# jstrom2002/ImageCodecs

Hardware: AMD Instinct MI355X
Metric: megapixels/s JPEG decode, 4096x4096 RGB batch (higher is better)
Workload: dtype u8

## Files before the change

imagecodecs_amd/__init__.py:

```python
from __future__ import annotations

import ctypes as C
import os
import subprocess

import numpy as np

__all__ = ["ICXError", "Context", "Batch", "HdrBatch", "Image", "lib", "build", "LIB_PATH",
           "OK", "NO_JPEG", "UNSUPPORTED", "OUT_OF_MEM", "INTERNAL_ERR", "SYNTAX_ERROR",
           "HDR_OK", "HDR_NOT_RADIANCE", "HDR_BAD_HEADER", "HDR_MALFORMED", "HDR_TRUNCATED",
           "HDR_TOO_LARGE", "HDR_INTERNAL_ERR", "hdr_probe", "exr_probe", "EXR_SUCCESS", "EXR_INVALID_DATA", "Multi", "RECORD_DTYPE", "records_device",
           "checksum64", "multi_shard"]

OK, NO_JPEG, UNSUPPORTED, OUT_OF_MEM, INTERNAL_ERR, SYNTAX_ERROR = range(6)
RESULT_NAMES = ["NJ_OK", "NJ_NO_JPEG", "NJ_UNSUPPORTED", "NJ_OUT_OF_MEM", "NJ_INTERNAL_ERR", "NJ_SYNTAX_ERROR"]

_HERE = os.path.dirname(os.path.abspath(__file__))
_DEFAULT_LIB = os.path.join(_HERE, "lib", "libicx.so")
LIB_PATH = os.environ.get("ICX_LIB") or _DEFAULT_LIB
_LIB = None


class ICXError(RuntimeError):
    pass


def build() -> str:
    subprocess.run(["make", "-s", "-C", _HERE], check=True)
    return LIB_PATH


_vp, _i32, _i64, _u64, _sz = C.c_void_p, C.c_int, C.c_int64, C.c_uint64, C.c_size_t
_SIGS = {
    "icx_version": (C.c_char_p, []),
    "icx_last_error": (C.c_char_p, [_vp]),
    "icx_create": (_vp, [_i32]),
    "icx_destroy": (None, [_vp]),
    "icx_free": (None, [_vp]),
    "icx_jpeg_probe": (_i32, [_vp, _sz, C.POINTER(_i32), C.POINTER(_i32), C.POINTER(_i32)]),
    "icx_nj_init": (None, [_vp]),
    "icx_nj_done": (None, [_vp]),
    "icx_nj_decode": (_i32, [_vp, _vp, _i32]),
    "icx_nj_get_width": (_i32, [_vp]),
    "icx_nj_get_height": (_i32, [_vp]),
    "icx_nj_is_color": (_i32, [_vp]),
    "icx_nj_get_image": (_vp, [_vp]),
    "icx_nj_get_image_size": (_i32, [_vp]),
    "icx_jpeg_decode": (_i32, [_vp, _vp, _sz, C.POINTER(_vp), C.POINTER(_i32), C.POINTER(_i32), C.POINTER(_i32)]),
    "icx_batch_create": (_vp, [_vp, _i32, _i32, _i32, _i32]),
    "icx_batch_destroy": (None, [_vp]),
    "icx_jpeg_batch_decode": (_i32, [_vp, _i32, _vp, _vp, _vp, _vp, _u64, _vp, _vp, _vp]),
    "icx_jpeg_batch_decode_host": (_i32, [_vp, _i32, _vp, _vp, _vp, _u64, _vp, _vp]),
    "icx_batch_stage_times": (_i32, [_vp, _vp, _vp, _i32]),
    "icx_batch_group": (_i32, [_vp]),
    "icx_batch_groups": (_i32, [_vp, _i32]),
    "icx_batch_path_stats": (_i32, [_vp, C.POINTER(_i32), C.POINTER(_i32), C.POINTER(_i32)]),
    "icx_tje_encode_with_func": (_i32, [_vp, _vp, _vp, _i32, _i32, _i32, _i32, _vp]),
    "icx_tje_encode_to_file_at_quality": (_i32, [_vp, C.c_char_p, _i32, _i32, _i32, _i32, _vp]),
    "icx_tje_encode_to_file": (_i32, [_vp, C.c_char_p, _i32, _i32, _i32, _vp]),
    "icx_jpeg_encode_with_func": (_i32, [_vp, _vp, _vp, _i32, _i32, _i32, _i32, _i32, _vp]),
    "icx_encoder_create": (_vp, [_vp]),
    "icx_encoder_destroy": (None, [_vp]),
    "icx_encoder_stage_times": (_i32, [_vp, _vp, _vp, _i32]),
    "icx_png_encode_with_func": (_i32, [_vp, _vp, _vp, _vp, _i32, _i32, _i32]),
    "icx_png_save_to_file": (_i32, [_vp, C.c_char_p, _vp, _i32, _i32, _i32]),
    "icx_png_encoder_create": (_vp, [_vp]),
    "icx_png_encoder_destroy": (None, [_vp]),
    "icx_png_encode_device": (_i32, [_vp, _i32, _i32, _i32, _vp, _vp, _u64, C.POINTER(_u64), _vp]),
    "icx_png_encode_device_batch": (_i32, [_vp, _i32, _i32, _i32, _i32, _vp, _vp, _u64, _vp, _vp, _vp]),
    "icx_png_encoder_stage_times": (_i32, [_vp, C.POINTER(C.c_char_p), C.POINTER(C.c_float), _i32]),
    "icx_jpeg_encode_device": (_i32, [_vp, _i32, _i32, _i32, _i32, _i32, _vp, _vp, _u64, C.POINTER(_u64), _vp]),
    "icx_jpeg_encode_device_batch": (_i32, [_vp, _i32, _i32, _i32, _i32, _i32, _i32, _vp, _vp, _u64, _vp, _vp, _vp]),
    "icx_hdr_probe": (_i32, [_vp, _sz, C.POINTER(_i32), C.POINTER(_i32)]),
    "icx_hdr_decode": (_i32, [_vp, _vp, _sz, C.POINTER(_vp), C.POINTER(_i32), C.POINTER(_i32), C.POINTER(_i32)]),
    "icx_hdr_batch_create": (_vp, [_vp, _i32, _i32, _i32]),
    "icx_hdr_batch_destroy": (None, [_vp]),
    "icx_hdr_batch_decode": (_i32, [_vp, _i32, _vp, _vp, _vp, _vp, _u64, _vp, _vp, _vp]),
    "icx_hdr_batch_stage_times": (_i32, [_vp, _vp, _vp, _i32]),
    "icx_jpeg_records": (_i32, [_vp, _i32, _vp, _u64, _vp, _vp, _i32, _i32, _vp, _vp]),
    "icx_checksum64": (_u64, [_vp, _sz]),
    "icx_ctx_device": (_i32, [_vp]),
    "icx_ctx_stream": (_vp, [_vp]),
    "icx_multi_create": (_vp, [_vp, _i32, _i32, _i32]),
    "icx_multi_destroy": (None, [_vp]),
    "icx_multi_decode_host": (_i32, [_vp, _i32, _vp, _vp, _vp, _u64, _vp, _vp]),
    "icx_multi_last_error": (C.c_char_p, [_vp]),
    "icx_multi_gather": (C.c_char_p, [_vp]),
    "icx_multi_shard": (_i32, [_vp, _i32, _i32, _vp]),
    "icx_exr_probe": (_i32, [_vp, _sz, C.POINTER(_i32), C.POINTER(_i32)]),
    "icx_exr_decode": (_i32, [_vp, _vp, _sz, C.POINTER(_vp), C.POINTER(_i32), C.POINTER(_i32)]),
    "icx_exr_decode_device": (_i32, [_vp, _vp, _vp, _sz, _vp, _sz, C.POINTER(_i32), C.POINTER(_i32)]),
    "icx_exr_decode_device_batch": (_i32, [_vp, _i32, _vp, _vp, _vp, _vp, _vp, _vp, _vp, _vp]),
}

RECORD_DTYPE = np.dtype([("status", "<i4"), ("width", "<i4"), ("height", "<i4"), ("ncomp", "<i4"),
                         ("checksum", "<u8")])

HDR_OK, HDR_NOT_RADIANCE, HDR_BAD_HEADER, HDR_MALFORMED, HDR_TRUNCATED, HDR_TOO_LARGE = range(6)
HDR_INTERNAL_ERR = -1

EXR_SUCCESS, EXR_INVALID_MAGIC_NUMBER, EXR_INVALID_EXR_VERSION, EXR_INVALID_ARGUMENT, EXR_INVALID_DATA = 0, -1, -2, -3, -4
EXR_UNSUPPORTED_FORMAT, EXR_INVALID_HEADER, EXR_UNSUPPORTED_FEATURE, EXR_INTERNAL_ERR = -8, -9, -10, -100

WRITE_FUNC = C.CFUNCTYPE(None, C.c_void_p, C.c_void_p, C.c_int)


def _share_hip_runtime_with_torch() -> None:
    import importlib.util
    spec = importlib.util.find_spec("torch")
    if spec is None or not spec.submodule_search_locations:
        return
    tlib = os.path.join(list(spec.submodule_search_locations)[0], "lib")
    for name in ("libhsa-runtime64.so", "libamdhip64.so"):
        path = os.path.join(tlib, name)
        if os.path.exists(path):
            C.CDLL(path, mode=C.RTLD_GLOBAL)


def lib():
    global _LIB
    if _LIB is None:
        if not os.path.exists(LIB_PATH):
            raise ICXError(f"{LIB_PATH} not built: run `make -C imagecodecs_amd` (hipcc, gfx950)")
        _share_hip_runtime_with_torch()
        L = C.CDLL(LIB_PATH)
        for name, (res, args) in _SIGS.items():
            try:
                fn = getattr(L, name)
            except AttributeError:
                if LIB_PATH != _DEFAULT_LIB:
                    continue
                raise
            fn.restype = res
            fn.argtypes = args
        _LIB = L
    return _LIB


def _err(ctx_ptr) -> str:
    msg = lib().icx_last_error(ctx_ptr)
    return msg.decode() if msg else ""


class Context:

    def __init__(self, device: int = 0):
        self._p = lib().icx_create(device)
        if not self._p:
            raise ICXError("icx_create failed: " + _err(None))
        self.device = device

    def close(self):
        if getattr(self, "_p", None):
            lib().icx_destroy(self._p)
            self._p = None

    def __del__(self):
        self.close()

    def __enter__(self):
        return self

    def __exit__(self, *a):
        self.close()

    @property
    def ptr(self):
        return self._p

    def nj_init(self):
        lib().icx_nj_init(self._p)

    def nj_done(self):
        lib().icx_nj_done(self._p)

    def nj_decode(self, jpeg: bytes) -> int:
        buf = C.create_string_buffer(bytes(jpeg), max(1, len(jpeg)))
        return lib().icx_nj_decode(self._p, buf, len(jpeg))

    def nj_get_width(self) -> int:
        return lib().icx_nj_get_width(self._p)

    def nj_get_height(self) -> int:
        return lib().icx_nj_get_height(self._p)

    def nj_is_color(self) -> int:
        return lib().icx_nj_is_color(self._p)

    def nj_get_image_size(self) -> int:
        return lib().icx_nj_get_image_size(self._p)

    def nj_get_image(self) -> bytes:
        p = lib().icx_nj_get_image(self._p)
        return C.string_at(p, self.nj_get_image_size()) if p else b""

    def decode(self, jpeg: bytes):
        buf = C.create_string_buffer(bytes(jpeg), max(1, len(jpeg)))
        out = C.c_void_p()
        w, h, n = C.c_int(), C.c_int(), C.c_int()
        code = lib().icx_jpeg_decode(self._p, buf, len(jpeg), C.byref(out), C.byref(w), C.byref(h), C.byref(n))
        pix = b""
        if out.value:
            pix = C.string_at(out.value, w.value * h.value * n.value)
            lib().icx_free(out)
        if code == INTERNAL_ERR and _err(self._p):
            raise ICXError(_err(self._p))
        return code, w.value, h.value, n.value, pix

    def tje_encode(self, quality: int, width: int, height: int, comps: int, src: bytes):
        chunks = []

        @WRITE_FUNC
        def sink(_ctx, data, size):
            chunks.append(C.string_at(data, size))

        buf = C.create_string_buffer(bytes(src), max(1, len(src)))
        ok = lib().icx_tje_encode_with_func(self._p, sink, None, quality, width, height, comps, buf)
        return b"".join(chunks) if ok == 1 else None

    def hdr_decode(self, data: bytes):
        buf = C.create_string_buffer(bytes(data), max(1, len(data)))
        out = C.c_void_p()
        w, h, rows = C.c_int(), C.c_int(), C.c_int()
        code = lib().icx_hdr_decode(self._p, buf, len(data), C.byref(out), C.byref(w), C.byref(h), C.byref(rows))
        if code == HDR_INTERNAL_ERR:
            raise ICXError("icx_hdr_decode: " + _err(self._p))
        arr = None
        if out.value:
            n = w.value * h.value * 4
            arr = np.frombuffer(C.string_at(out.value, n * 4), np.float32).reshape(h.value, w.value, 4).copy()
            lib().icx_free(out)
        return code, w.value, h.value, rows.value, arr

    def exr_decode(self, data: bytes):
        buf = C.create_string_buffer(bytes(data), max(1, len(data)))
        out = C.c_void_p()
        w, h = C.c_int(), C.c_int()
        code = lib().icx_exr_decode(self._p, buf, len(data), C.byref(out), C.byref(w), C.byref(h))
        if code == EXR_INTERNAL_ERR:
            raise ICXError("icx_exr_decode: " + _err(self._p))
        arr = None
        if out.value:
            n = w.value * h.value * 4
            arr = np.frombuffer(C.string_at(out.value, n * 4), np.float32).reshape(h.value, w.value, 4).copy()
            lib().icx_free(out)
        return code, w.value, h.value, arr

    def exr_decode_device(self, data: bytes, d_data: int, d_out: int, out_floats: int):
        buf = C.create_string_buffer(bytes(data), max(1, len(data)))
        w, h = C.c_int(), C.c_int()
        code = lib().icx_exr_decode_device(self._p, buf, C.c_void_p(d_data), len(data), C.c_void_p(d_out), out_floats,
                                           C.byref(w), C.byref(h))
        if code == EXR_INTERNAL_ERR:
            raise ICXError("icx_exr_decode_device: " + _err(self._p))
        return code, w.value, h.value

    def exr_decode_device_batch(self, datas, d_ptrs, d_outs, out_floats):
        n = len(datas)
        bufs = [C.create_string_buffer(bytes(d), max(1, len(d))) for d in datas]
        hp = (C.c_void_p * n)(*[C.cast(b, C.c_void_p) for b in bufs])
        dp = (C.c_void_p * n)(*d_ptrs)
        sz = (C.c_size_t * n)(*[len(d) for d in datas])
        op = (C.c_void_p * n)(*d_outs)
        of = (C.c_size_t * n)(*out_floats)
        codes = np.zeros(n, np.int32)
        ws = np.zeros(n, np.int32)
        hs = np.zeros(n, np.int32)
        rc = lib().icx_exr_decode_device_batch(self._p, n, hp, dp, sz, op, of, codes.ctypes.data, ws.ctypes.data,
                                               hs.ctypes.data)
        if rc == EXR_INTERNAL_ERR:
            raise ICXError("icx_exr_decode_device_batch: " + _err(self._p))
        if rc != 0:
            raise ICXError(f"icx_exr_decode_device_batch: code {rc}")
        return codes, ws, hs

    def png_encode(self, width: int, height: int, d: int, src: bytes):
        chunks = []

        @WRITE_FUNC
        def sink(_ctx, data, size):
            chunks.append(C.string_at(data, size))

        buf = C.create_string_buffer(bytes(src), max(1, len(src)))
        ok = lib().icx_png_encode_with_func(self._p, sink, None, buf, width, height, d)
        return b"".join(chunks) if ok == 1 else None

    def jpeg_encode(self, quality: int, subsampling: int, width: int, height: int, comps: int, src: bytes):
        chunks = []

        @WRITE_FUNC
        def sink(_ctx, data, size):
            chunks.append(C.string_at(data, size))

        buf = C.create_string_buffer(bytes(src), max(1, len(src)))
        ok = lib().icx_jpeg_encode_with_func(self._p, sink, None, quality, subsampling, width, height, comps, buf)
        return b"".join(chunks) if ok == 1 else None


class PngEncoder:

    def __init__(self, ctx: Context):
        self.ctx = ctx
        self._p = lib().icx_png_encoder_create(ctx.ptr)
        if not self._p:
            raise ICXError("icx_png_encoder_create failed: " + _err(ctx.ptr))

    def close(self):
        if getattr(self, "_p", None):
            lib().icx_png_encoder_destroy(self._p)
            self._p = None

    def __del__(self):
        self.close()

    def encode_device(self, width, height, d, d_src, d_out, out_cap, stream=0):
        n = C.c_uint64()
        rc = lib().icx_png_encode_device(self._p, width, height, d, d_src, d_out, out_cap, C.byref(n), stream or None)
        if rc not in (OK, OUT_OF_MEM):
            raise ICXError(f"icx_png_encode_device -> {rc}: {_err(self.ctx.ptr)}")
        return rc, int(n.value)

    def encode_device_batch(self, width, height, d, d_srcs, d_out, out_stride, stream=0):
        n = len(d_srcs)
        srcs = (C.c_void_p * max(1, n))(*d_srcs)
        sizes = np.zeros(max(1, n), np.uint64)
        status = np.zeros(max(1, n), np.int32)
        rc = lib().icx_png_encode_device_batch(self._p, n, width, height, d, srcs, d_out, out_stride,
                                               sizes.ctypes.data, status.ctypes.data, stream or None)
        if rc != OK:
            raise ICXError(f"icx_png_encode_device_batch -> {rc}: {_err(self.ctx.ptr)}")
        return status[:n], sizes[:n].astype(np.int64)

    def stage_times(self) -> dict:
        names = (C.c_char_p * 8)()
        ms = (C.c_float * 8)()
        k = lib().icx_png_encoder_stage_times(self._p, names, ms, 8)
        return {names[i].decode(): float(ms[i]) for i in range(k)}


class Encoder:

    def __init__(self, ctx: Context):
        self.ctx = ctx
        self._p = lib().icx_encoder_create(ctx.ptr)
        if not self._p:
            raise ICXError("icx_encoder_create failed: " + _err(ctx.ptr))

    def close(self):
        if getattr(self, "_p", None):
            lib().icx_encoder_destroy(self._p)
            self._p = None

    def __del__(self):
        self.close()

    def encode_device(self, quality, subsampling, width, height, comps, d_src, d_out, out_cap, stream=0):
        n = C.c_uint64()
        rc = lib().icx_jpeg_encode_device(self._p, quality, subsampling, width, height, comps, d_src, d_out,
                                          out_cap, C.byref(n), stream or None)
        if rc not in (OK, OUT_OF_MEM):
            raise ICXError(f"icx_jpeg_encode_device -> {rc}: {_err(self.ctx.ptr)}")
        return rc, int(n.value)

    def encode_device_batch(self, quality, subsampling, width, height, comps, d_srcs, d_out, out_stride, stream=0):
        n = len(d_srcs)
        srcs = (C.c_void_p * max(1, n))(*d_srcs)
        sizes = np.zeros(max(1, n), np.uint64)
        status = np.zeros(max(1, n), np.int32)
        rc = lib().icx_jpeg_encode_device_batch(self._p, n, quality, subsampling, width, height, comps, srcs, d_out,
                                                out_stride, sizes.ctypes.data, status.ctypes.data, stream or None)
        if rc != OK:
            raise ICXError(f"icx_jpeg_encode_device_batch -> {rc}: {_err(self.ctx.ptr)}")
        return status[:n], sizes[:n].astype(np.int64)

    def stage_times(self) -> dict:
        names = (C.c_char_p * 8)()
        ms = (C.c_float * 8)()
        k = lib().icx_encoder_stage_times(self._p, names, ms, 8)
        return {names[i].decode(): float(ms[i]) for i in range(k)}


def probe(jpeg: bytes):
    w, h, n = C.c_int(), C.c_int(), C.c_int()
    buf = C.create_string_buffer(bytes(jpeg), max(1, len(jpeg)))
    code = lib().icx_jpeg_probe(buf, len(jpeg), C.byref(w), C.byref(h), C.byref(n))
    return code, w.value, h.value, n.value


def records_device(ctx: "Context", n, d_out, out_stride, d_status, d_dims, max_width, max_height, d_records,
                   stream=0):
    rc = lib().icx_jpeg_records(ctx.ptr, n, d_out, out_stride, d_status, d_dims, max_width, max_height, d_records,
                                stream or None)
    if rc != OK:
        raise ICXError(f"icx_jpeg_records -> {rc}: {_err(ctx.ptr)}")


def checksum64(data: bytes) -> int:
    buf = C.create_string_buffer(bytes(data), max(1, len(data)))
    return int(lib().icx_checksum64(buf, len(data)))


def multi_shard(sizes, ndev: int) -> np.ndarray:
    n = len(sizes)
    sz = (C.c_size_t * max(1, n))(*[int(x) for x in sizes])
    out = np.zeros(max(1, n), np.int32)
    if lib().icx_multi_shard(sz, n, ndev, out.ctypes.data) != OK:
        raise ICXError("icx_multi_shard failed")
    return out[:n]


class Multi:

    def __init__(self, devices, max_width: int, max_height: int):
        devs = (C.c_int * len(devices))(*devices)
        self._p = lib().icx_multi_create(devs, len(devices), max_width, max_height)
        if not self._p:
            raise ICXError("icx_multi_create failed: " + _err(None))
        self.devices = list(devices)
        self.max_width, self.max_height = max_width, max_height

    @property
    def gather(self) -> str:
        return lib().icx_multi_gather(self._p).decode()

    def close(self):
        if getattr(self, "_p", None):
            lib().icx_multi_destroy(self._p)
            self._p = None

    def __del__(self):
        self.close()

    def decode_host(self, jpegs, want_pixels: bool = True):
        n = len(jpegs)
        stride = self.max_width * self.max_height * 3
        bufs = [C.create_string_buffer(bytes(j), max(1, len(j))) for j in jpegs]
        ptrs = (C.c_void_p * max(1, n))(*[C.cast(b, C.c_void_p) for b in bufs])
        sizes = (C.c_size_t * max(1, n))(*[len(j) for j in jpegs])
        outs_np = [np.empty(stride, np.uint8) for _ in range(n)] if want_pixels else None
        outs = (C.c_void_p * max(1, n))(*[o.ctypes.data for o in outs_np]) if want_pixels else None
        rec = np.zeros(max(1, n), RECORD_DTYPE)
        shard_of = np.zeros(max(1, n), np.int32)
        rc = lib().icx_multi_decode_host(self._p, n, ptrs, sizes, outs, stride, rec.ctypes.data, shard_of.ctypes.data)
        if rc != OK:
            msg = lib().icx_multi_last_error(self._p)
            raise ICXError(f"icx_multi_decode_host -> {rc}: {msg.decode() if msg else ''}")
        pix = None
        if want_pixels:
            pix = []
            for i in range(n):
                r = rec[i]
                nb = int(r["width"]) * int(r["height"]) * int(r["ncomp"])
                pix.append(outs_np[i][:nb] if r["status"] == OK else None)
        return rec[:n], shard_of[:n], pix


class Batch:

    def __init__(self, ctx: Context, max_images: int, max_width: int, max_height: int, group: int = 0):
        self.ctx = ctx
        self._p = lib().icx_batch_create(ctx.ptr, max_images, max_width, max_height, group)
        if not self._p:
            raise ICXError("icx_batch_create failed: " + _err(ctx.ptr))
        self.max_images, self.max_width, self.max_height = max_images, max_width, max_height

    def close(self):
        if getattr(self, "_p", None):
            lib().icx_batch_destroy(self._p)
            self._p = None

    def __del__(self):
        self.close()

    def decode_device(self, n, d_data, d_offsets, d_sizes, d_out, out_stride, d_status, d_dims, stream=0):
        rc = lib().icx_jpeg_batch_decode(self._p, n, d_data, d_offsets, d_sizes, d_out, out_stride,
                                         d_status, d_dims, stream or None)
        if rc != OK:
            raise ICXError(f"icx_jpeg_batch_decode -> {rc}: {_err(self.ctx.ptr)}")

    def decode_host(self, jpegs, out_stride=None):
        n = len(jpegs)
        out_stride = out_stride or self.max_width * self.max_height * 3
        bufs = [C.create_string_buffer(bytes(j), max(1, len(j))) for j in jpegs]
        ptrs = (C.c_void_p * n)(*[C.cast(b, C.c_void_p) for b in bufs])
        sizes = (C.c_size_t * n)(*[len(j) for j in jpegs])
        outs_np = [np.empty(out_stride, np.uint8) for _ in range(n)]
        outs = (C.c_void_p * n)(*[o.ctypes.data for o in outs_np])
        status = np.zeros(n, np.int32)
        dims = np.zeros((n, 3), np.int32)
        rc = lib().icx_jpeg_batch_decode_host(self._p, n, ptrs, sizes, outs, out_stride,
                                              status.ctypes.data, dims.ctypes.data)
        if rc != OK:
            raise ICXError(f"icx_jpeg_batch_decode_host -> {rc}: {_err(self.ctx.ptr)}")
        res = []
        for i in range(n):
            w, h, c = (int(x) for x in dims[i])
            pix = outs_np[i][: w * h * c].reshape(h, w, c) if status[i] == OK else None
            res.append((int(status[i]), w, h, c, pix))
        return res

    def path_stats(self) -> dict:
        a, b, c = C.c_int(), C.c_int(), C.c_int()
        lib().icx_batch_path_stats(self._p, C.byref(a), C.byref(b), C.byref(c))
        return {"parallel": a.value, "fallback": b.value, "sequential": c.value}

    @property
    def group(self) -> int:
        return int(lib().icx_batch_group(self._p))

    def groups_per_call(self, n: int) -> int:
        return int(lib().icx_batch_groups(self._p, n))

    def stage_times(self) -> dict:
        names = (C.c_char_p * 16)()
        ms = (C.c_float * 16)()
        k = lib().icx_batch_stage_times(self._p, names, ms, 16)
        return {names[i].decode(): float(ms[i]) for i in range(k)}


def hdr_probe(data: bytes):
    w, h = C.c_int(), C.c_int()
    buf = C.create_string_buffer(bytes(data), max(1, len(data)))
    code = lib().icx_hdr_probe(buf, len(data), C.byref(w), C.byref(h))
    return code, w.value, h.value


def exr_probe(data: bytes):
    w, h = C.c_int(), C.c_int()
    buf = C.create_string_buffer(bytes(data), max(1, len(data)))
    code = lib().icx_exr_probe(buf, len(data), C.byref(w), C.byref(h))
    return code, w.value, h.value


class HdrBatch:

    def __init__(self, ctx: Context, max_images: int, max_width: int, max_height: int):
        self.ctx = ctx
        self._p = lib().icx_hdr_batch_create(ctx.ptr, max_images, max_width, max_height)
        if not self._p:
            raise ICXError("icx_hdr_batch_create failed: " + _err(ctx.ptr))
        self.max_images, self.max_width, self.max_height = max_images, max_width, max_height

    def close(self):
        if getattr(self, "_p", None):
            lib().icx_hdr_batch_destroy(self._p)
            self._p = None

    def __del__(self):
        self.close()

    def decode_device(self, n, d_data, d_offsets, d_sizes, d_out, out_stride, d_status, d_dims, stream=0):
        rc = lib().icx_hdr_batch_decode(self._p, n, d_data, d_offsets, d_sizes, d_out, out_stride,
                                        d_status, d_dims, stream or None)
        if rc != HDR_OK:
            raise ICXError(f"icx_hdr_batch_decode -> {rc}: {_err(self.ctx.ptr)}")

    def stage_times(self) -> dict:
        names = (C.c_char_p * 8)()
        ms = (C.c_float * 8)()
        k = lib().icx_hdr_batch_stage_times(self._p, names, ms, 8)
        return {names[i].decode(): float(ms[i]) for i in range(k)}


class Image:

    UBYTE, USHORT, FLOAT = range(3)
    _ctx = None

    def __init__(self):
        self.h_ = self.w_ = self.d_ = 0
        self.pixels_ = None
        self.type_ = Image.UBYTE

    @classmethod
    def context(cls):
        if cls._ctx is None:
            cls._ctx = Context(0)
        return cls._ctx

    def read(self, filepath: str):
        ext = os.path.splitext(filepath)[1].lower()
        if ext == ".hdr":
            self._read_hdr(filepath)
            return
        if ext == ".exr":
            self._read_exr(filepath)
            return
        if ext not in (".jpg", ".jpeg"):
            raise ValueError("Cannot parse filetype")
        data = open(filepath, "rb").read()
        code, w, h, n, pix = self.context().decode(data)
        if code != OK:
            raise RuntimeError("Error decoding the input file.\n")
        self.w_, self.h_, self.d_ = w, h, n
        self.pixels_ = np.frombuffer(pix, np.uint8).copy()
        self.type_ = Image.UBYTE

    def _read_hdr(self, filepath: str):
        data = open(filepath, "rb").read()
        code, w, h, rows, px = self.context().hdr_decode(data)
        if code not in (HDR_OK, HDR_TRUNCATED):
            raise RuntimeError("Invalid file format")
        self.w_, self.h_, self.d_ = w, h, 4
        self.pixels_ = px.reshape(-1).view(np.uint8).copy()
        self.type_ = Image.FLOAT

    def _read_exr(self, filepath: str):
        data = open(filepath, "rb").read()
        code, w, h, px = self.context().exr_decode(data + b"\xff")
        if code != EXR_SUCCESS:
            raise RuntimeError("Could not load .exr")
        self.w_, self.h_, self.d_ = w, h, 4
        self.pixels_ = px.reshape(-1).view(np.uint8).copy()
        self.type_ = Image.FLOAT

    def write(self, filepath: str):
        ext = os.path.splitext(filepath)[1].lower()
        if ext == ".png":
            out = self.context().png_encode(self.w_, self.h_, self.d_, self.pixels_.tobytes())
        elif ext in (".jpg", ".jpeg"):
            out = self.context().tje_encode(3, self.w_, self.h_, self.d_, self.pixels_.tobytes())
        else:
            raise ValueError("Cannot parse filetype")
        with open(filepath, "wb") as f:
            if out is not None:
                f.write(out)

    def load(self, pixels, w: int, h: int, channels: int):
        self.pixels_ = np.ascontiguousarray(pixels, np.uint8).reshape(-1)
        self.w_, self.h_, self.d_ = w, h, channels
        self.type_ = Image.UBYTE

    def rows(self):
        return self.h_

    def cols(self):
        return self.w_

    def channels(self):
        return self.d_

    def empty(self):
        return self.h_ == 0 or self.w_ == 0 or self.d_ == 0 or self.pixels_ is None

    def byteSize(self):
        return 4 if self.type_ == Image.FLOAT else 2 if self.type_ == Image.USHORT else 1

    def type(self):
        return self.type_

    def totalBytes(self):
        return self.w_ * self.h_ * self.d_ * self.byteSize()

    def data(self):
        return self.pixels_
```

imagecodecs_amd/csrc/icx_api.cpp:

```cpp
#include <hip/hip_runtime.h>
#include <rocprofiler-sdk-roctx/roctx.h>

#include <algorithm>
#include <cstdio>
#include <cstdlib>
#include <cstring>
#include <exception>
#include <memory>
#include <string>
#include <vector>

#include "../../include/icx.h"
#include "icx_internal.h"
#include "icx_step.h"

using namespace icx;

struct icx_ctx {
    int device = 0;
    hipStream_t stream = nullptr;
    std::string err;
    std::vector<uint8_t> nj_image;
    int nj_w = 0, nj_h = 0, nj_color = 0, nj_size = 0;
    icx_batch* single = nullptr;
    uint8_t* d_in = nullptr;
    size_t d_in_cap = 0;
    ExrWs* exr = nullptr;
};

struct EventHook;

#ifndef ICX_MAX_PIPES
#define ICX_MAX_PIPES 2
#endif
constexpr int kMaxPipes = ICX_MAX_PIPES;
struct icx_batch {
    icx_ctx* ctx = nullptr;
    int max_images = 0;
    int pipes = 1;
    GroupWs ws[kMaxPipes];
    hipStream_t pst[kMaxPipes] = {};
    hipEvent_t fork = nullptr, join[kMaxPipes] = {};
    std::vector<hipEvent_t> front_done;
    int min_groups = 1;
    bool stagger = false;
    uint8_t* d_hin = nullptr;
    size_t d_hin_cap = 0;
    hipEvent_t done = nullptr;
    bool decoded = false;
    std::unique_ptr<EventHook> hook;
};

static std::string g_create_err;

static thread_local char g_msg[512];

#define ICX_HIP(ctx, call, ret)                                                             \
    do {                                                                                    \
        hipError_t e_ = (call);                                                             \
        if (e_ != hipSuccess) {                                                             \
            (void)hipGetLastError();  \
            std::snprintf(g_msg, sizeof g_msg, "%s failed: %s", #call, hipGetErrorString(e_)); \
            if (ctx) (ctx)->err = g_msg;                                                    \
            return ret;                                                                     \
        }                                                                                   \
    } while (0)

struct RoctxRange {
    explicit RoctxRange(const char* m) { (void)roctxRangePushA(m); }
    ~RoctxRange() { (void)roctxRangePop(); }
};
static const char* const kRangeNames[kStCount] = {"icx:parse", "icx:unstuff", "icx:entropy", "icx:write",
                                                  "icx:idct", "icx:upsample", "icx:convert"};
struct EventHook : StageHook {
    struct Rec { Stage s; hipEvent_t a, b; };
    std::vector<Rec> recs;
    std::vector<hipEvent_t> pool;
    size_t used = 0;
    hipEvent_t get() {
        if (used == pool.size()) {
            hipEvent_t e;
            if (hipEventCreate(&e) != hipSuccess) return nullptr;
            pool.push_back(e);
        }
        return pool[used++];
    }
    void reset() { recs.clear(); used = 0; }
    void begin(Stage s, hipStream_t st) override {
        (void)roctxRangePushA(kRangeNames[s]);
        hipEvent_t a = get(), b = get();
        if (!a || !b) return;
        (void)hipEventRecord(a, st);
        recs.push_back({s, a, b});
    }
    void end(Stage s, hipStream_t st) override {
        (void)roctxRangePop();
        for (auto it = recs.rbegin(); it != recs.rend(); ++it)
            if (it->s == s) { (void)hipEventRecord(it->b, st); return; }
    }
    ~EventHook() override {
        for (auto e : pool) (void)hipEventDestroy(e);
    }
};

extern "C" {

const char* icx_version(void) { return "icx 0.1.0 gfx950"; }

const char* icx_last_error(const icx_ctx* ctx) { return ctx ? ctx->err.c_str() : g_create_err.c_str(); }

icx_ctx* icx_create(int device) {
    int n = 0;
    if (hipGetDeviceCount(&n) != hipSuccess || n <= 0) {
        g_create_err = "no HIP device available (libicx has no CPU decode path)";
        return nullptr;
    }
    if (device < 0 || device >= n) {
        g_create_err = "device ordinal out of range";
        return nullptr;
    }
    if (hipSetDevice(device) != hipSuccess) {
        g_create_err = "hipSetDevice failed";
        return nullptr;
    }
    auto* c = new icx_ctx();
    c->device = device;
    if (hipStreamCreateWithFlags(&c->stream, hipStreamNonBlocking) != hipSuccess) {
        g_create_err = "hipStreamCreate failed";
        delete c;
        return nullptr;
    }
    return c;
}

void icx_batch_destroy(icx_batch* b);

void icx_destroy(icx_ctx* c) {
    if (!c) return;
    (void)hipSetDevice(c->device);
    if (c->single) icx_batch_destroy(c->single);
    if (c->d_in) (void)hipFree(c->d_in);
    if (c->exr) exr_ws_destroy(c->exr);
    if (c->stream) (void)hipStreamDestroy(c->stream);
    delete c;
}

void icx_free(void* p) { std::free(p); }
int icx_ctx_device(const icx_ctx* c) { return c ? c->device : -1; }
void* icx_ctx_stream(const icx_ctx* c) { return c ? (void*)c->stream : nullptr; }

int icx_jpeg_probe(const uint8_t* jpeg, size_t size, int* w, int* h, int* ncomp) {
    if (w) *w = 0;
    if (h) *h = 0;
    if (ncomp) *ncomp = 0;
    if (!jpeg) return ICX_NO_JPEG;
    auto d = std::make_unique<Desc>();
    int st = parse_headers(jpeg, (int64_t)std::min<size_t>(size, 0x7FFFFFFF), *d);
    if (st != kPending) return st;
    if (w) *w = d->W;
    if (h) *h = d->H;
    if (ncomp) *ncomp = d->nc == 1 ? 1 : 3;
    return ICX_OK;
}

static int64_t ws_per_slot(GroupWs& ws, int max_w, int max_h) {
    ws.max_w = max_w;
    ws.max_h = max_h;
    ws.coef_cap = ws_coef_cap(max_w, max_h);
    ws.plane_cap = ws_plane_cap(max_w, max_h);
    ws.tmp_cap = ws_tmp_cap(max_w, max_h);
    const int bpp = std::getenv("ICX_UPOOL_BPP") ? std::max(1, std::min(16, std::atoi(std::getenv("ICX_UPOOL_BPP")))) : 2;
    ws.ucap = ((int64_t)max_w * max_h * bpp + 4095) / 4096 * 4096;
    ws.rst_cap = ((int64_t)max_w / 8 + 1) * ((int64_t)max_h / 8 + 1);
    const int64_t tiles_per_slot = ws.ucap / kTileBytes + 2;
    const int64_t lanes_per_slot = ((ws.ucap + kSubBytesSmall - 1) / kSubBytesSmall + kLanes - 1) / kLanes * kLanes + kLanes;
    return ws.coef_cap * kPoolPerSlotX4 / 4 * (64 * 2 + 4 + 8) + ws.plane_cap + (int64_t)sizeof(Desc) + ws.ucap +
           (int64_t)sizeof(StepSet) +
           tiles_per_slot * 28 + ws.rst_cap * 8 +
           lanes_per_slot * (8 + 8 + 20 + 24 + 4 + 16 + (int64_t)sizeof(RecState) * kRec + (int64_t)sizeof(GwOut) +
                             (int64_t)sizeof(GcRec) + 8) + kMaxRepair * 4;
}

static void ws_free(GroupWs& ws) {
    if (ws.tmp_own && ws.tmp) (void)hipFree(ws.tmp);
    for (void* p : {(void*)ws.desc, (void*)ws.ac, (void*)ws.dc, (void*)ws.planes, (void*)ws.spec,
                    (void*)ws.tilepre, (void*)ws.wgpre, (void*)ws.wg2pre, (void*)ws.totals, (void*)ws.tiles,
                    (void*)ws.tile_obase, (void*)ws.U, (void*)ws.X, (void*)ws.sub, (void*)ws.rst, (void*)ws.tile_rbase,
                    (void*)ws.ent, (void*)ws.stats, (void*)ws.Y, (void*)ws.rec, (void*)ws.nrec, (void*)ws.guess_cnt,
                    (void*)ws.repair, (void*)ws.steps, (void*)ws.map, (void*)ws.chunk_next, (void*)ws.pool_next,
                    (void*)ws.gw, (void*)ws.crec, (void*)ws.clist})
        if (p) (void)hipFree(p);
    if (ws.h_defer) (void)hipHostFree(ws.h_defer);
    if (ws.h_layout) (void)hipHostFree(ws.h_layout);
    if (ws.ev_defer) (void)hipEventDestroy(ws.ev_defer);
    ws = GroupWs{};
}

static bool ws_alloc_all(icx_ctx* ctx, GroupWs& ws, int group, int max_w, int max_h);
static bool ws_alloc(icx_ctx* ctx, GroupWs& ws, int group, int max_w, int max_h) {
    if (ws_alloc_all(ctx, ws, group, max_w, max_h)) return true;
    ws_free(ws);
    return false;
}

static bool ws_alloc_all(icx_ctx* ctx, GroupWs& ws, int group, int max_w, int max_h) {
    (void)ws_per_slot(ws, max_w, max_h);
    const int64_t tiles_per_slot = ws.ucap / kTileBytes + 2;
    const int64_t lanes_per_slot = ((ws.ucap + kSubBytesSmall - 1) / kSubBytesSmall + kLanes - 1) / kLanes * kLanes + kLanes;
    ws.slots = group;
    ws.upool = (int64_t)(group + 2) * ws.ucap;
    ICX_HIP(ctx, hipMalloc(&ws.desc, sizeof(Desc) * group), false);
    ws.pool_cap = (int64_t)(group + 2) * ws.coef_cap * kPoolPerSlotX4 / 4;
    ICX_HIP(ctx, hipMalloc(&ws.ac, (size_t)(ws.pool_cap + kGwChunk) * 64 * 2), false);
    ICX_HIP(ctx, hipMalloc(&ws.dc, (size_t)(ws.pool_cap + kGwChunk) * 4), false);
    ICX_HIP(ctx, hipMalloc(&ws.map, (size_t)ws.pool_cap * sizeof(uint2)), false);
    ICX_HIP(ctx, hipMalloc(&ws.chunk_next, (size_t)(ws.pool_cap / kGwChunk + 2) * 4), false);
    ICX_HIP(ctx, hipMalloc(&ws.pool_next, sizeof(unsigned long long)), false);
    ICX_HIP(ctx, hipMalloc(&ws.planes, (size_t)ws.plane_cap * group), false);
    if ((int64_t)(ws.pool_cap + kGwChunk) * 64 * 2 >= ws.tmp_cap * 6 * group) {
        ws.tmp = reinterpret_cast<uint8_t*>(ws.ac);
    } else {
        ICX_HIP(ctx, hipMalloc(&ws.tmp, (size_t)ws.tmp_cap * 6 * group), false);
        ws.tmp_own = true;
    }
    ws.tiles_cap = tiles_per_slot * (group + 2);
    ws.lanes_cap = lanes_per_slot * (group + 2);
    ICX_HIP(ctx, hipMalloc(&ws.spec, sizeof(SpecImg) * group), false);
    ICX_HIP(ctx, hipMalloc(&ws.tilepre, sizeof(int32_t) * (group + 1)), false);
    ICX_HIP(ctx, hipMalloc(&ws.wgpre, sizeof(int32_t) * (group + 1)), false);
    ICX_HIP(ctx, hipMalloc(&ws.wg2pre, sizeof(int32_t) * (group + 1)), false);
    ICX_HIP(ctx, hipMalloc(&ws.totals, sizeof(int32_t) * 4), false);
    ICX_HIP(ctx, hipMalloc(&ws.tiles, sizeof(TileRec) * ws.tiles_cap), false);
    ICX_HIP(ctx, hipMalloc(&ws.tile_obase, sizeof(int32_t) * ws.tiles_cap), false);
    ICX_HIP(ctx, hipMalloc(&ws.U, (size_t)ws.upool + 256), false);
    ICX_HIP(ctx, hipMalloc(&ws.X, sizeof(uint64_t) * ws.lanes_cap), false);
    ICX_HIP(ctx, hipMalloc(&ws.sub, sizeof(SubRec) * ws.lanes_cap), false);
    ICX_HIP(ctx, hipMalloc(&ws.rst, sizeof(int64_t) * ws.rst_cap * group), false);
    ICX_HIP(ctx, hipMalloc(&ws.tile_rbase, sizeof(int32_t) * ws.tiles_cap), false);
    ICX_HIP(ctx, hipMalloc(&ws.ent, sizeof(LaneEntry) * ws.lanes_cap), false);
    ICX_HIP(ctx, hipMalloc(&ws.stats, sizeof(int32_t) * 4), false);
    ICX_HIP(ctx, hipMalloc(&ws.Y, sizeof(uint64_t) * ws.lanes_cap), false);
    ICX_HIP(ctx, hipMalloc(&ws.rec, sizeof(RecState) * kRec * ws.lanes_cap), false);
    ICX_HIP(ctx, hipMalloc(&ws.nrec, sizeof(int32_t) * ws.lanes_cap), false);
    ICX_HIP(ctx, hipMalloc(&ws.guess_cnt, sizeof(int32_t) * 4 * ws.lanes_cap), false);
    ICX_HIP(ctx, hipMalloc(&ws.repair, sizeof(int32_t) * kMaxRepair * group), false);
    ICX_HIP(ctx, hipMalloc(&ws.steps, sizeof(StepSet) * group), false);
    ICX_HIP(ctx, hipMalloc(&ws.gw, sizeof(GwOut) * ws.lanes_cap), false);
    ICX_HIP(ctx, hipMalloc(&ws.crec, sizeof(GcRec) * ws.lanes_cap), false);
    ICX_HIP(ctx, hipMalloc(&ws.clist, sizeof(int2) * ws.lanes_cap), false);
    ICX_HIP(ctx, hipHostMalloc(&ws.h_defer, 3 * sizeof(int32_t), hipHostMallocDefault), false);
    ws.h_defer[0] = ws.h_defer[1] = ws.h_defer[2] = 0;
    ICX_HIP(ctx, hipHostMalloc(&ws.h_layout, sizeof(int32_t), hipHostMallocDefault), false);
    *ws.h_layout = 1;
    ICX_HIP(ctx, hipEventCreateWithFlags(&ws.ev_defer, hipEventDisableTiming), false);
    return true;
}

icx_batch* icx_batch_create(icx_ctx* ctx, int max_images, int max_w, int max_h, int group) {
    if (!ctx || max_images <= 0 || max_w <= 0 || max_h <= 0 || max_w > 65535 || max_h > 65535) {
        if (ctx) ctx->err = "icx_batch_create: bad arguments";
        return nullptr;
    }
    ICX_HIP(ctx, hipSetDevice(ctx->device), nullptr);
    std::unique_ptr<icx_batch, void (*)(icx_batch*)> b(new icx_batch(), icx_batch_destroy);
    b->ctx = ctx;
    b->max_images = max_images;
    int pipes = kMaxPipes;
    if (const char* e = std::getenv("ICX_PIPES")) pipes = std::max(1, std::min(kMaxPipes, std::atoi(e)));
    if (max_images < 2) pipes = 1;
    GroupWs probe;
    const int64_t per_slot = ws_per_slot(probe, max_w, max_h);
    if (group <= 0) {
        size_t free_b = 0, total_b = 0;
        ICX_HIP(ctx, hipMemGetInfo(&free_b, &total_b), nullptr);
        const int64_t budget = (int64_t)(0.8 * (double)free_b);
        group = (int)std::max<int64_t>(1, std::min<int64_t>(max_images, budget / per_slot));
    }
    group = std::min(group, max_images);
    if (group < 2) pipes = 1;
    b->pipes = pipes;
    if (const char* e = std::getenv("ICX_GROUPS")) b->min_groups = std::max(1, std::atoi(e));
    if (const char* e = std::getenv("ICX_STAGGER")) b->stagger = std::atoi(e) != 0;
    for (int p = 0; p < pipes; ++p) {
        const int slots = (group + pipes - 1) / pipes;
        if (!ws_alloc(ctx, b->ws[p], slots, max_w, max_h)) return nullptr;
        if (p > 0) ICX_HIP(ctx, hipStreamCreateWithFlags(&b->pst[p], hipStreamNonBlocking), nullptr);
        ICX_HIP(ctx, hipEventCreateWithFlags(&b->join[p], hipEventDisableTiming), nullptr);
    }
    ICX_HIP(ctx, hipEventCreateWithFlags(&b->fork, hipEventDisableTiming), nullptr);
    ICX_HIP(ctx, hipEventCreateWithFlags(&b->done, hipEventDisableTiming), nullptr);
    b->hook = std::make_unique<EventHook>();
    return b.release();
}

void icx_batch_destroy(icx_batch* b) {
    if (!b) return;
    (void)hipSetDevice(b->ctx->device);
    for (int p = 0; p < kMaxPipes; ++p) {
        ws_free(b->ws[p]);
        if (b->pst[p]) (void)hipStreamDestroy(b->pst[p]);
        if (b->join[p]) (void)hipEventDestroy(b->join[p]);
    }
    if (b->fork) (void)hipEventDestroy(b->fork);
    if (b->done) (void)hipEventDestroy(b->done);
    for (auto e : b->front_done) (void)hipEventDestroy(e);
    if (b->d_hin) (void)hipFree(b->d_hin);
    delete b;
}

static int batch_split(const icx_batch* b, int n, int* per_out) {
    const int slots = b->ws[0].slots;
    const int want = std::min(n, std::max((n + slots - 1) / slots, b->min_groups));
    int per = (n + want - 1) / want;
    int ng = (n + per - 1) / per;
    if (b->pipes > 1 && ng > 1 && ng % b->pipes) {
        const int up = (ng + b->pipes - 1) / b->pipes * b->pipes;
        if (up <= n) {
            const int per2 = (n + up - 1) / up;
            const int ng2 = (n + per2 - 1) / per2;
            if (ng2 % b->pipes == 0) {
                per = per2;
                ng = ng2;
            }
        }
    }
    *per_out = per;
    return ng;
}

int icx_batch_groups(const icx_batch* b, int n) {
    int per = 0;
    return b && n > 0 ? batch_split(b, n, &per) : 0;
}

int icx_jpeg_batch_decode(icx_batch* b, int n, const uint8_t* d_data, const uint64_t* d_off, const uint64_t* d_size,
                          uint8_t* d_out, uint64_t out_stride, int32_t* d_status, int32_t* d_dims, void* stream) {
    if (!b) return ICX_INTERNAL_ERR;
    icx_ctx* ctx = b->ctx;
    if (n < 0 || n > b->max_images) { ctx->err = "icx_jpeg_batch_decode: n exceeds batch capacity"; return ICX_INTERNAL_ERR; }
    if (n == 0) return ICX_OK;
    if (!d_data || !d_off || !d_size || !d_out || !d_status || !d_dims) { ctx->err = "null pointer"; return ICX_INTERNAL_ERR; }
    ICX_HIP(ctx, hipSetDevice(ctx->device), ICX_INTERNAL_ERR);
    hipStream_t st = stream ? (hipStream_t)stream : ctx->stream;
    const RoctxRange range("icx_jpeg_batch_decode");
    b->hook->reset();
    for (int p = 0; p < b->pipes; ++p)
        ICX_HIP(ctx, hipMemsetAsync(b->ws[p].stats, 0, sizeof(int32_t) * 4, st), ICX_INTERNAL_ERR);
    int per = 0;
    const int ng = batch_split(b, n, &per);
    const int used = std::min(b->pipes, ng);
    if (used > 1) {
        ICX_HIP(ctx, hipEventRecord(b->fork, st), ICX_INTERNAL_ERR);
        for (int p = 1; p < used; ++p) ICX_HIP(ctx, hipStreamWaitEvent(b->pst[p], b->fork, 0), ICX_INTERNAL_ERR);
    }
    const bool stagger = b->stagger && used > 1;
    hipStreamCaptureStatus cap = hipStreamCaptureStatusNone;
    ICX_HIP(ctx, hipStreamIsCapturing(st, &cap), ICX_INTERNAL_ERR);
    const char* hw = std::getenv("ICX_HOST_WAIT");
    const bool no_wait_env = hw && std::atoi(hw) == 0;
    const bool host_wait = !stagger && cap == hipStreamCaptureStatusNone && !no_wait_env;
    while (stagger && (int)b->front_done.size() < ng) {
        hipEvent_t e;
        ICX_HIP(ctx, hipEventCreateWithFlags(&e, hipEventDisableTiming), ICX_INTERNAL_ERR);
        b->front_done.push_back(e);
    }
    auto front0 = [&](int g) {
        const int g0 = g * per, p = g % used;
        launch_decode_front(b->ws[p], std::min(per, n - g0), d_data, d_off + g0, d_size + g0, out_stride,
                            p == 0 ? st : b->pst[p], b->hook.get(), host_wait ? kFrontFirst : kFrontAll);
    };
    for (int g = 0; g < std::min(used, ng); ++g) {
        if (stagger && g > 0) ICX_HIP(ctx, hipStreamWaitEvent(b->pst[g % used], b->front_done[g - 1], 0), ICX_INTERNAL_ERR);
        front0(g);
        if (stagger) ICX_HIP(ctx, hipEventRecord(b->front_done[g], g % used == 0 ? st : b->pst[g % used]), ICX_INTERNAL_ERR);
    }
    for (int g = 0; g < ng; ++g) {
        const int g0 = g * per, gn = std::min(per, n - g0), p = g % used;
        hipStream_t ps = p == 0 ? st : b->pst[p];
        if (host_wait) launch_decode_front(b->ws[p], gn, d_data, d_off + g0, d_size + g0, out_stride, ps, b->hook.get(),
                                           kFrontRest);
        launch_decode_back(b->ws[p], gn, d_out + (uint64_t)g0 * out_stride, out_stride, d_status + g0, d_dims + 3 * g0,
                           ps, b->hook.get(), host_wait);
        const int gnext = g + used;
        if (gnext < ng) {
            hipStream_t pn = gnext % used == 0 ? st : b->pst[gnext % used];
            if (stagger) ICX_HIP(ctx, hipStreamWaitEvent(pn, b->front_done[gnext - 1], 0), ICX_INTERNAL_ERR);
            front0(gnext);
            if (stagger) ICX_HIP(ctx, hipEventRecord(b->front_done[gnext], pn), ICX_INTERNAL_ERR);
        }
    }
    for (int p = 1; p < used; ++p) {
        ICX_HIP(ctx, hipEventRecord(b->join[p], b->pst[p]), ICX_INTERNAL_ERR);
        ICX_HIP(ctx, hipStreamWaitEvent(st, b->join[p], 0), ICX_INTERNAL_ERR);
    }
    ICX_HIP(ctx, hipEventRecord(b->done, st), ICX_INTERNAL_ERR);
    b->decoded = true;
    ICX_HIP(ctx, hipGetLastError(), ICX_INTERNAL_ERR);
    return ICX_OK;
}

int icx_batch_path_stats(const icx_batch* b, int32_t* parallel, int32_t* fallback, int32_t* sequential) {
    if (!b) return ICX_INTERNAL_ERR;
    int32_t h[4] = {0, 0, 0, 0};
    ICX_HIP(b->ctx, hipSetDevice(b->ctx->device), ICX_INTERNAL_ERR);
    if (b->decoded) ICX_HIP(b->ctx, hipEventSynchronize(b->done), ICX_INTERNAL_ERR);
    for (int p = 0; p < b->pipes; ++p) {
        int32_t q[4];
        ICX_HIP(b->ctx, hipMemcpy(q, b->ws[p].stats, sizeof q, hipMemcpyDeviceToHost), ICX_INTERNAL_ERR);
        for (int k = 0; k < 4; ++k) h[k] += q[k];
    }
    if (parallel) *parallel = h[0];
    if (fallback) *fallback = h[1];
    if (sequential) *sequential = h[2];
    return ICX_OK;
}

int icx_batch_group(const icx_batch* b) { return b ? b->ws[0].slots : 0; }

int icx_batch_stage_times(const icx_batch* b, const char** names, float* ms, int cap) {
    if (!b) return 0;
    float acc[kStCount] = {0};
    for (auto& r : b->hook->recs) {
        float t = 0;
        if (hipEventSynchronize(r.b) == hipSuccess && hipEventElapsedTime(&t, r.a, r.b) == hipSuccess) acc[r.s] += t;
        else (void)hipGetLastError();
    }
    int k = 0;
    for (int s = 0; s < kStCount && k < cap; ++s, ++k) {
        if (names) names[k] = kStageNames[s];
        if (ms) ms[k] = acc[s];
    }
    return kStCount;
}

int icx_jpeg_batch_decode_host(icx_batch* b, int n, const uint8_t* const* jpegs, const size_t* sizes,
                               uint8_t* const* outs, uint64_t out_stride, int32_t* status, int32_t* dims) {
    if (!b) return ICX_INTERNAL_ERR;
    icx_ctx* ctx = b->ctx;
    if (n <= 0) return n == 0 ? ICX_OK : ICX_INTERNAL_ERR;
    ICX_HIP(ctx, hipSetDevice(ctx->device), ICX_INTERNAL_ERR);
    std::vector<uint64_t> off(n), sz(n);
    uint64_t total = 0;
    for (int i = 0; i < n; ++i) { off[i] = total; sz[i] = sizes[i]; total += (sizes[i] + 15) & ~uint64_t(15); }
    const size_t meta = (size_t)n * (8 + 8 + 4 + 12);
    const size_t need = total + meta + (size_t)n * out_stride + 256;
    if (need > b->d_hin_cap) {
        if (b->d_hin) (void)hipFree(b->d_hin);
        b->d_hin = nullptr;
        b->d_hin_cap = 0;
        ICX_HIP(ctx, hipMalloc(&b->d_hin, need), ICX_OUT_OF_MEM);
        b->d_hin_cap = need;
    }
    uint8_t* base = b->d_hin;
    uint8_t* d_data = base;
    uint64_t* d_off = reinterpret_cast<uint64_t*>(base + ((total + 15) & ~uint64_t(15)));
    uint64_t* d_sz = d_off + n;
    int32_t* d_st = reinterpret_cast<int32_t*>(d_sz + n);
    int32_t* d_dm = d_st + n;
    uint8_t* d_out = reinterpret_cast<uint8_t*>(((uintptr_t)(d_dm + 3 * n) + 255) & ~uintptr_t(255));
    hipStream_t st = ctx->stream;
    for (int i = 0; i < n; ++i)
        if (sz[i]) ICX_HIP(ctx, hipMemcpyAsync(d_data + off[i], jpegs[i], sz[i], hipMemcpyHostToDevice, st), ICX_INTERNAL_ERR);
    ICX_HIP(ctx, hipMemcpyAsync(d_off, off.data(), 8 * n, hipMemcpyHostToDevice, st), ICX_INTERNAL_ERR);
    ICX_HIP(ctx, hipMemcpyAsync(d_sz, sz.data(), 8 * n, hipMemcpyHostToDevice, st), ICX_INTERNAL_ERR);
    int rc = icx_jpeg_batch_decode(b, n, d_data, d_off, d_sz, d_out, out_stride, d_st, d_dm, st);
    if (rc) return rc;
    ICX_HIP(ctx, hipMemcpyAsync(status, d_st, 4 * n, hipMemcpyDeviceToHost, st), ICX_INTERNAL_ERR);
    ICX_HIP(ctx, hipMemcpyAsync(dims, d_dm, 12 * n, hipMemcpyDeviceToHost, st), ICX_INTERNAL_ERR);
    ICX_HIP(ctx, hipStreamSynchronize(st), ICX_INTERNAL_ERR);
    for (int i = 0; i < n; ++i) {
        const size_t bytes = (size_t)dims[3 * i] * dims[3 * i + 1] * dims[3 * i + 2];
        if (status[i] == ICX_OK && bytes)
            ICX_HIP(ctx, hipMemcpyAsync(outs[i], d_out + (uint64_t)i * out_stride, bytes, hipMemcpyDeviceToHost, st),
                    ICX_INTERNAL_ERR);
    }
    ICX_HIP(ctx, hipStreamSynchronize(st), ICX_INTERNAL_ERR);
    return ICX_OK;
}

static int decode_one(icx_ctx* ctx, const uint8_t* jpeg, size_t size, std::vector<uint8_t>& out, int& w, int& h,
                      int& color) {
    w = h = color = 0;
    out.clear();
    if (!ctx) return ICX_INTERNAL_ERR;
    int pw = 0, ph = 0, pc = 0;
    const int probe = icx_jpeg_probe(jpeg, size, &pw, &ph, &pc);
    if (probe != ICX_OK) return probe;
    if (!ctx->single || ctx->single->ws[0].max_w < pw || ctx->single->ws[0].max_h < ph) {
        if (ctx->single) icx_batch_destroy(ctx->single);
        ctx->single = icx_batch_create(ctx, 1, std::max(pw, 1), std::max(ph, 1), 1);
        if (!ctx->single) return ICX_OUT_OF_MEM;
    }
    const uint8_t* in[1] = {jpeg};
    size_t sizes[1] = {std::min<size_t>(size, 0x7FFFFFFF)};
    out.resize(std::max<size_t>((size_t)pw * ph * 3, 1));
    uint8_t* outs[1] = {out.data()};
    int32_t st = 0, dims[3] = {0, 0, 0};
    int rc = icx_jpeg_batch_decode_host(ctx->single, 1, in, sizes, outs, out.size(), &st, dims);
    if (rc) return rc;
    if (st != ICX_OK) { out.clear(); return st; }
    w = dims[0];
    h = dims[1];
    color = dims[2] == 3;
    out.resize((size_t)w * h * dims[2]);
    return ICX_OK;
}

int icx_jpeg_decode(icx_ctx* ctx, const uint8_t* jpeg, size_t size, uint8_t** out, int* w, int* h, int* ncomp) {
    if (out) *out = nullptr;
    std::vector<uint8_t> buf;
    int W = 0, H = 0, color = 0;
    int rc = decode_one(ctx, jpeg, size, buf, W, H, color);
    if (w) *w = W;
    if (h) *h = H;
    if (ncomp) *ncomp = rc == ICX_OK ? (color ? 3 : 1) : 0;
    if (rc == ICX_OK && out && !buf.empty()) {
        *out = static_cast<uint8_t*>(std::malloc(buf.size()));
        if (!*out) return ICX_OUT_OF_MEM;
        std::memcpy(*out, buf.data(), buf.size());
    }
    return rc;
}

void icx_nj_init(icx_ctx* ctx) {
    if (!ctx) return;
    ctx->nj_image.clear();
    ctx->nj_w = ctx->nj_h = ctx->nj_color = ctx->nj_size = 0;
}
void icx_nj_done(icx_ctx* ctx) { icx_nj_init(ctx); }

int icx_nj_decode(icx_ctx* ctx, const void* jpeg, int size) {
    if (!ctx) return ICX_INTERNAL_ERR;
    icx_nj_init(ctx);
    int W = 0, H = 0, color = 0;
    int rc = decode_one(ctx, static_cast<const uint8_t*>(jpeg), (size_t)(size & 0x7FFFFFFF), ctx->nj_image, W, H, color);
    if (rc == ICX_OK) {
        ctx->nj_w = W;
        ctx->nj_h = H;
        ctx->nj_color = color;
        ctx->nj_size = (int)ctx->nj_image.size();
    }
    return rc;
}
int icx_nj_get_width(const icx_ctx* ctx) { return ctx ? ctx->nj_w : 0; }
int icx_nj_get_height(const icx_ctx* ctx) { return ctx ? ctx->nj_h : 0; }
int icx_nj_is_color(const icx_ctx* ctx) { return ctx ? ctx->nj_color : 0; }
unsigned char* icx_nj_get_image(icx_ctx* ctx) {
    return (ctx && !ctx->nj_image.empty()) ? ctx->nj_image.data() : nullptr;
}
int icx_nj_get_image_size(const icx_ctx* ctx) { return ctx ? ctx->nj_size : 0; }

int icx_tje_encode_with_func(icx_ctx* ctx, icx_write_func* func, void* context, int quality, int width, int height,
                             int num_components, const unsigned char* src) {
    if (!ctx || !func) return 0;
    if (quality < 1 || quality > 3) { ctx->err = "quality must be 1, 2 or 3"; return 0; }
    if (num_components != 3 && num_components != 4) { ctx->err = "num_components must be 3 or 4"; return 0; }
    if (width > 0xFFFF || height > 0xFFFF || width < 0 || height < 0) { ctx->err = "image too large"; return 0; }
    if ((int64_t)width * height > 0 && !src) { ctx->err = "null source"; return 0; }
    ICX_HIP(ctx, hipSetDevice(ctx->device), 0);
    std::vector<uint8_t> file;
    if (!tje_encode_gpu(ctx->stream, quality, width, height, num_components, src, file)) {
        ctx->err = "HIP failure in tje_encode_gpu";
        return 0;
    }
    for (size_t o = 0; o < file.size(); o += 1023)
        func(context, file.data() + o, (int)std::min<size_t>(1023, file.size() - o));
    return 1;
}

static void file_sink(void* ctx, void* data, int size) { std::fwrite(data, (size_t)size, 1, (FILE*)ctx); }

int icx_tje_encode_to_file_at_quality(icx_ctx* ctx, const char* dest_path, int quality, int width, int height,
                                      int num_components, const unsigned char* src) {
    FILE* fd = std::fopen(dest_path, "wb");
    if (!fd) { if (ctx) ctx->err = "could not open file for writing"; return 0; }
    int result = icx_tje_encode_with_func(ctx, file_sink, fd, quality, width, height, num_components, src);
    result |= 0 == std::fclose(fd);
    return result;
}

int icx_tje_encode_to_file(icx_ctx* ctx, const char* dest_path, int width, int height, int num_components,
                           const unsigned char* src) {
    return icx_tje_encode_to_file_at_quality(ctx, dest_path, 3, width, height, num_components, src);
}

static const char* enc_args_bad(int quality, int subsampling, int width, int height, int comps) {
    if (quality < 1 || quality > 100) return "quality must be 1..100";
    if (subsampling != 444 && subsampling != 420) return "subsampling must be 444 or 420";
    if (comps != 3 && comps != 4) return "num_components must be 3 or 4";
    if (width > 0xFFFF || height > 0xFFFF || width < 0 || height < 0) return "image too large";
    return nullptr;
}

int icx_jpeg_encode_with_func(icx_ctx* ctx, icx_write_func* func, void* context, int quality, int subsampling,
                              int width, int height, int num_components, const unsigned char* src) {
    if (!ctx || !func) return 0;
    if (const char* e = enc_args_bad(quality, subsampling, width, height, num_components)) { ctx->err = e; return 0; }
    if ((int64_t)width * height > 0 && !src) { ctx->err = "null source"; return 0; }
    ICX_HIP(ctx, hipSetDevice(ctx->device), 0);
    std::vector<uint8_t> file;
    if (!jpeg_encode_gpu(ctx->stream, quality, subsampling, width, height, num_components, src, file)) {
        ctx->err = "HIP failure in jpeg_encode_gpu";
        return 0;
    }
    for (size_t o = 0; o < file.size(); o += 1023)
        func(context, file.data() + o, (int)std::min<size_t>(1023, file.size() - o));
    return 1;
}

struct icx_encoder {
    icx_ctx* ctx = nullptr;
    EncWs* ws = nullptr;
};

icx_encoder* icx_encoder_create(icx_ctx* ctx) {
    if (!ctx) return nullptr;
    icx_encoder* e = new icx_encoder();
    e->ctx = ctx;
    e->ws = enc_ws_create();
    return e;
}

void icx_encoder_destroy(icx_encoder* enc) {
    if (!enc) return;
    (void)hipSetDevice(enc->ctx->device);
    enc_ws_destroy(enc->ws);
    delete enc;
}

int icx_encoder_stage_times(icx_encoder* enc, const char** names, float* ms, int cap) {
    if (!enc || cap <= 0) return 0;
    return enc_ws_stage_times(enc->ws, names, ms, cap);
}

int icx_jpeg_encode_device(icx_encoder* enc, int quality, int subsampling, int width, int height,
                           int num_components, const uint8_t* d_src, uint8_t* d_out, uint64_t out_cap,
                           uint64_t* out_size, void* hip_stream) {
    if (!enc || !out_size) return ICX_UNSUPPORTED;
    icx_ctx* ctx = enc->ctx;
    if (const char* e = enc_args_bad(quality, subsampling, width, height, num_components)) {
        ctx->err = e;
        return ICX_UNSUPPORTED;
    }
    if (((int64_t)width * height > 0 && !d_src) || (out_cap && !d_out)) { ctx->err = "null buffer"; return ICX_UNSUPPORTED; }
    ICX_HIP(ctx, hipSetDevice(ctx->device), ICX_INTERNAL_ERR);
    hipStream_t st = hip_stream ? (hipStream_t)hip_stream : ctx->stream;
    const int rc = jpeg_encode_device(st, enc->ws, quality, subsampling, width, height, num_components, d_src, d_out,
                                      out_cap, out_size);
    if (rc < 0) { ctx->err = "HIP failure in jpeg_encode_device"; return ICX_INTERNAL_ERR; }
    return rc == 0 ? ICX_OK : ICX_OUT_OF_MEM;
}

int icx_jpeg_encode_device_batch(icx_encoder* enc, int n, int quality, int subsampling, int width, int height,
                                 int num_components, const uint8_t* const* d_srcs, uint8_t* d_out, uint64_t out_stride,
                                 uint64_t* out_sizes, int32_t* status, void* hip_stream) {
    if (!enc || n < 0 || (n > 0 && (!d_srcs || !out_sizes || !status))) return ICX_UNSUPPORTED;
    icx_ctx* ctx = enc->ctx;
    if (const char* e = enc_args_bad(quality, subsampling, width, height, num_components)) {
        ctx->err = e;
        return ICX_UNSUPPORTED;
    }
    for (int i = 0; i < n; ++i)
        if ((int64_t)width * height > 0 && !d_srcs[i]) { ctx->err = "null buffer"; return ICX_UNSUPPORTED; }
    if (n > 0 && out_stride && !d_out) { ctx->err = "null buffer"; return ICX_UNSUPPORTED; }
    ICX_HIP(ctx, hipSetDevice(ctx->device), ICX_INTERNAL_ERR);
    hipStream_t st = hip_stream ? (hipStream_t)hip_stream : ctx->stream;
    std::vector<int32_t> rc(n > 0 ? n : 1);
    if (jpeg_encode_device_batch(st, enc->ws, n, quality, subsampling, width, height, num_components, d_srcs, d_out,
                                 out_stride, out_sizes, rc.data()) < 0) {
        ctx->err = "HIP failure in jpeg_encode_device_batch";
        return ICX_INTERNAL_ERR;
    }
    for (int i = 0; i < n; ++i) status[i] = rc[i] == 0 ? ICX_OK : ICX_OUT_OF_MEM;
    return ICX_OK;
}

static const char* png_args_bad(int w, int h, int d) {
    if (d != 3 && d != 4) return "d must be 3 or 4";
    if (w <= 0 || h <= 0) return "empty image";
    if ((int64_t)w * h > (int64_t)1 << 31) return "image too large";
    return nullptr;
}

int icx_png_encode_with_func(icx_ctx* ctx, icx_write_func* func, void* context, const unsigned char* pixels, int width,
                             int height, int d) {
    if (!ctx || !func) return 0;
    if (const char* e = png_args_bad(width, height, d)) { ctx->err = e; return 0; }
    if (!pixels) { ctx->err = "null source"; return 0; }
    ICX_HIP(ctx, hipSetDevice(ctx->device), 0);
    std::vector<uint8_t> file;
    if (!png_encode_gpu(ctx->stream, width, height, d, pixels, file)) {
        ctx->err = "HIP failure in png_encode_gpu";
        return 0;
    }
    for (size_t o = 0; o < file.size(); o += 1023)
        func(context, file.data() + o, (int)std::min<size_t>(1023, file.size() - o));
    return 1;
}

int icx_png_save_to_file(icx_ctx* ctx, const char* path, const unsigned char* pixels, int width, int height, int d) {
    if (!ctx || !path) return ICX_UNSUPPORTED;
    FILE* fd = std::fopen(path, "wb");
    if (!fd) { ctx->err = "could not open file for writing"; return ICX_INTERNAL_ERR; }
    const int ok = icx_png_encode_with_func(ctx, file_sink, fd, pixels, width, height, d);
    const bool closed = std::fclose(fd) == 0;
    if (!ok) return png_args_bad(width, height, d) || !pixels ? ICX_UNSUPPORTED : ICX_INTERNAL_ERR;
    return closed ? ICX_OK : ICX_INTERNAL_ERR;
}

constexpr int kPngInflightMax = 8;
struct icx_png_encoder {
    icx_ctx* ctx = nullptr;
    PngWs* ws = nullptr;
    PngWs* wsx[kPngInflightMax] = {};
    hipStream_t stx[kPngInflightMax] = {};
    hipEvent_t fork = nullptr;
// ... 313 lines not shown
```

imagecodecs_amd/csrc/icx_decode.hip:

```cpp
#include <hip/hip_runtime.h>

#include <algorithm>
#include <cstdlib>

#include "icx_internal.h"

namespace icx {

const char* const kStageNames[kStCount] = {"parse", "unstuff", "entropy", "write", "idct", "upsample", "convert"};

int64_t ws_coef_cap(int w, int h) {
    int64_t wp = ((int64_t)w + 63) / 64 * 64, hp = ((int64_t)h + 63) / 64 * 64;
    return 3 * (wp / 8) * (hp / 8);
}
int64_t ws_plane_cap(int w, int h) { return ws_coef_cap(w, h) * 64; }
int64_t ws_tmp_cap(int w, int h) { return ((int64_t)w + 8) * ((int64_t)h + 8); }

__device__ __forceinline__ bool fused420_shape(const Desc& d);
__global__ __launch_bounds__(64) void k_parse(int n, const uint8_t* __restrict__ data, const uint64_t* __restrict__ off,
                                              const uint64_t* __restrict__ size, Desc* __restrict__ desc, int max_w,
                                              int max_h, uint64_t out_stride, int32_t* __restrict__ layout) {
    const int i = blockIdx.x;
    if (i >= n) return;
    Desc& d = desc[i];
// ... 1187 lines not shown
    hi = max(hi, R[0][0]);
    lo = min(lo, R[0][0]);
    const bool fast = __all(hi < (1 << 14) && lo > -(1 << 14));
    if (fast) {
#pragma unroll
        for (int i = 0; i < 4; ++i) idct_row_full(R[i]);
    } else {
#pragma unroll
        for (int i = 0; i < 4; ++i) idct_row<false>(R[i]);
    }
    int32_t C[8][4];
#pragma unroll
    for (int i = 0; i < 4; ++i) {
#pragma unroll
        for (int jj = 0; jj < 4; ++jj) {
            const int32_t keep = h ? R[i][4 + jj] : R[i][jj];
            const int32_t got = pair_swap(h ? R[i][jj] : R[i][4 + jj]);
            C[i][jj] = h ? got : keep;
            C[4 + i][jj] = h ? keep : got;
        }
    }
    if (fast) {
        int32_t o[4][8];
#pragma unroll
        for (int jj = 0; jj < 4; ++jj) {
            int32_t col[8];
#pragma unroll
            for (int r = 0; r < 8; ++r) col[r] = C[r][jj];
            idct_col_raw(col, o[jj]);
        }
#pragma unroll
        for (int r = 0; r < 8; ++r) rowd[r] = sat4<14>(o[0][r], o[1][r], o[2][r], o[3][r]);
        return;
    }
#pragma unroll
    for (int r = 0; r < 8; ++r) rowd[r] = 0;
#pragma unroll
    for (int jj = 0; jj < 4; ++jj) {
        int32_t col[8];
#pragma unroll
        for (int r = 0; r < 8; ++r) col[r] = C[r][jj];
        uint8_t o[8];
        idct_col<false>(col, o);
#pragma unroll
        for (int r = 0; r < 8; ++r) rowd[r] |= (uint32_t)o[r] << (8 * jj);
    }
}
__device__ __forceinline__ void load_qw_g(const uint8_t* q, uint32_t (&qw)[16]) {
    const uint32_t* p = reinterpret_cast<const uint32_t*>(q);
#pragma unroll
    for (int k = 0; k < 16; ++k) qw[k] = p[k];
}
__device__ __forceinline__ void load_qw(const uint8_t* qz, uint32_t (&qw)[16]) {
    const uint4* qs = reinterpret_cast<const uint4*>(qz);
#pragma unroll
    for (int k = 0; k < 4; ++k) {
        const uint4 w = qs[k];
        qw[4 * k] = w.x; qw[4 * k + 1] = w.y; qw[4 * k + 2] = w.z; qw[4 * k + 3] = w.w;
    }
}
__device__ __forceinline__ void load_block(const int16_t* ac, int64_t blk, int h, int4 (&c)[8]) {
    const int4* src = reinterpret_cast<const int4*>(ac + blk * 64);
    c[0] = nt_ld(src + (h ? 4 : 0));
    c[1] = nt_ld(src + 1);
    c[2] = nt_ld(src + 2);
    c[3] = nt_ld(src + (h ? 7 : 3));
    c[5] = nt_ld(src + 5);
    c[6] = nt_ld(src + 6);
    c[4] = c[0];
    c[7] = c[3];
}

template <class PendF, class UnitF>
__device__ __forceinline__ void idct_units(const int16_t* ac, const Desc& d, int h, uint32_t wid, uint32_t nw,
                                           uint32_t nunits, PendF pendf, UnitF unit) {
    if (wid >= nunits) return;
    auto at = [&](uint32_t u) { return pendf(min(u, nunits - 1)); };
    int4 ca[8], cb[8];
    BlkLoc la = blk_resolve(d, at(wid)), lb;
    load_block(ac, la.blk, h, ca);
    BlkPend pa, pb = at(wid + nw);
    auto step = [&](uint32_t u, const int4 (&D)[8], const BlkLoc& lD, int4 (&Dn)[8], BlkLoc& lDn, const BlkPend& Pn,
                    BlkPend& Pa) {
        lDn = blk_resolve(d, Pn);
        load_block(ac, lDn.blk, h, Dn);
        Pa = at(u + 2 * nw);
        unit(u, D, lD);
    };
    for (uint32_t u = wid;;) {
        step(u, ca, la, cb, lb, pb, pa);
        if ((u += nw) >= nunits) break;
        step(u, cb, lb, ca, la, pa, pb);
        if ((u += nw) >= nunits) break;
    }
}

#ifndef ICX_IDCT_Y_MINW
#define ICX_IDCT_Y_MINW 4
#endif
#ifndef ICX_IDCT_C_MINW
#define ICX_IDCT_C_MINW 1
#endif

__global__ __launch_bounds__(256, ICX_IDCT_C_MINW) void k_idct420c(const Desc* __restrict__ desc, const int16_t* __restrict__ ac,
                                                  const int32_t* __restrict__ dcv, const uint2* __restrict__ map,
                                                  uint8_t* __restrict__ planes, int64_t plane_cap) {
    const int img = blockIdx.y;
    const Desc& d = desc[img];
    if (!fused420(d)) return;
    const int t = threadIdx.x;
    const int wave = __builtin_amdgcn_readfirstlane(t >> 6), lane = t & 63, q = lane >> 1, h = lane & 1, cc = q >> 4, mq = q & 15;
    uint32_t qw[16], qb[16];
    load_qw_g(d.q[d.c[1].tq], qw);
    load_qw_g(d.q[d.c[2].tq], qb);
#pragma unroll
    for (int k = 0; k < 16; ++k) qw[k] = cc ? qb[k] : qw[k];
    const int mbw = d.mbw, stride = d.c[1].stride;
    uint8_t* Pc = planes + (int64_t)img * plane_cap + comp_plane_off(d, 1);
    const uint32_t ccoff = cc ? (uint32_t)(comp_plane_off(d, 2) - comp_plane_off(d, 1)) : 0u;
    const uint32_t ucols = (uint32_t)((mbw + 15) >> 4), nunits = ucols * (uint32_t)d.mbh;
    const uint32_t chunk0 = (gridDim.x & 7) ? blockIdx.x : (blockIdx.x & 7) * (gridDim.x >> 3) + (blockIdx.x >> 3);
    const uint32_t wid = chunk0 * 4 + wave, nw = gridDim.x * 4;
    auto pendf = [&](uint32_t u) {
        const uint32_t mby = u / ucols;
        const int mx = (int)((u - mby * ucols) << 4) + mq;
        return blk_pend(d, map, ((int64_t)mby * mbw + min(mx, mbw - 1)) * 6 + 4 + cc);
    };
    auto unit = [&](uint32_t u, const int4 (&c)[8], const BlkLoc& l) {
        const uint32_t mby = u / ucols;
        const int mx = min((int)((u - mby * ucols) << 4) + mq, mbw - 1);
        uint32_t rowd[8];
        pair_idct(c, qw, h, dcv, l, rowd);
        uint8_t* const rowp = Pc + (int64_t)mby * 8 * stride;
        const uint32_t lo = ccoff + (uint32_t)(mx * 8 + 4 * h);
#pragma unroll
        for (int r = 0; r < 8; ++r) nt_st(rowd[r], reinterpret_cast<uint32_t*>(rowp + (lo + (uint32_t)(r * stride))));
    };
    idct_units(ac, d, h, wid, nw, nunits, pendf, unit);
}

__global__ __launch_bounds__(256, ICX_IDCT_Y_MINW) void k_idct420y(const Desc* __restrict__ desc, const int16_t* __restrict__ ac,
                                                  const int32_t* __restrict__ dcv, const uint2* __restrict__ map,
                                                  uint8_t* __restrict__ planes, int64_t plane_cap) {
    const int img = blockIdx.y;
    const Desc& d = desc[img];
    if (!fused420(d)) return;
    const int t = threadIdx.x;
    const int wave = __builtin_amdgcn_readfirstlane(t >> 6), lane = t & 63, q = lane >> 1, h = lane & 1, mq = q >> 2, k = q & 3;
    int sbx, sby;
    (void)mcu_block_comp(d, k, sbx, sby);
    uint32_t qw[16];
    load_qw_g(d.q[d.c[0].tq], qw);
    const int mbw = d.mbw, stride = d.c[0].stride;
    uint8_t* Py = planes + (int64_t)img * plane_cap;
    const uint32_t ucols = (uint32_t)((mbw + 7) >> 3), nunits = ucols * (uint32_t)d.mbh;
    const uint32_t chunk0 = (gridDim.x & 7) ? blockIdx.x : (blockIdx.x & 7) * (gridDim.x >> 3) + (blockIdx.x >> 3);
    const uint32_t wid = chunk0 * 4 + wave, nw = gridDim.x * 4;
    auto pendf = [&](uint32_t u) {
        const uint32_t mby = u / ucols;
        const int mx = (int)((u - mby * ucols) << 3) + mq;
        return blk_pend(d, map, ((int64_t)mby * mbw + min(mx, mbw - 1)) * 6 + k);
    };
    auto unit = [&](uint32_t u, const int4 (&c)[8], const BlkLoc& l) {
        const uint32_t mby = u / ucols;
        const int mx = min((int)((u - mby * ucols) << 3) + mq, mbw - 1);
        uint32_t rowd[8];
        pair_idct(c, qw, h, dcv, l, rowd);
        uint8_t* const rowp = Py + (int64_t)mby * 16 * stride;
        const uint32_t lo = (uint32_t)(sby * 8 * stride + mx * 16 + sbx * 8 + 4 * h);
#pragma unroll
        for (int r = 0; r < 8; ++r) nt_st(rowd[r], reinterpret_cast<uint32_t*>(rowp + (lo + (uint32_t)(r * stride))));
    };
    idct_units(ac, d, h, wid, nw, nunits, pendf, unit);
}

#ifndef ICX_IDCT1_MINW
#define ICX_IDCT1_MINW 4
#endif
#ifndef ICX_IDCT1_PF
#define ICX_IDCT1_PF 0
#endif
__device__ __forceinline__ void load_block8(const int16_t* ac, int64_t blk, int4 (&c)[8]) {
    const int4* src = reinterpret_cast<const int4*>(ac + blk * 64);
#pragma unroll
    for (int k = 0; k < 8; ++k) c[k] = nt_ld(src + k);
}
__device__ __forceinline__ void block_dequant(const int4 (&c)[8], const uint32_t (&qw)[16], const int32_t* dcv,
                                              const BlkLoc& loc, int32_t (&R)[8][8], int32_t& hi, int32_t& lo) {
    auto qt = [&](int z) { return (int32_t)((qw[z >> 2] >> (8 * (z & 3))) & 0xFFu); };
    auto coef = [&](int z) {
        const int4& w = c[z >> 3];
        const int e = z & 7;
        const uint32_t d32 = (uint32_t)(e < 2 ? w.x : e < 4 ? w.y : e < 6 ? w.z : w.w);
        return (int32_t)(int16_t)(d32 >> (16 * (e & 1)));
    };
    hi = 0;
    lo = 0;
#pragma unroll
    for (int n = 1; n < 64; ++n) {
        const int z = kZigOfNatC[n];
        R[n >> 3][n & 7] = m24(coef(z), qt(z));
        hi = max(hi, R[n >> 3][n & 7]);
        lo = min(lo, R[n >> 3][n & 7]);
    }
    R[0][0] = wmul(blk_dc((int16_t)c[0].x, dcv, loc), qt(0));
    hi = max(hi, R[0][0]);
    lo = min(lo, R[0][0]);
}
__device__ __forceinline__ void block_transform(int32_t (&R)[8][8], int32_t hi, int32_t lo, uint32_t (&rowd)[16]) {
    if (hi < (1 << 14) && lo > -(1 << 14)) {
#pragma unroll
        for (int i = 0; i < 8; ++i) idct_row_full(R[i]);
#pragma unroll
        for (int half = 0; half < 2; ++half) {
            int32_t o[4][8];
#pragma unroll
            for (int jj = 0; jj < 4; ++jj) {
                int32_t col[8];
#pragma unroll
                for (int r = 0; r < 8; ++r) col[r] = R[r][4 * half + jj];
                idct_col_raw(col, o[jj]);
            }
#pragma unroll
            for (int r = 0; r < 8; ++r) rowd[2 * r + half] = sat4<14>(o[0][r], o[1][r], o[2][r], o[3][r]);
        }
    } else {
#pragma unroll
        for (int i = 0; i < 8; ++i) idct_row<false>(R[i]);
#pragma unroll
        for (int r = 0; r < 16; ++r) rowd[r] = 0;
#pragma unroll
        for (int j = 0; j < 8; ++j) {
            int32_t col[8];
#pragma unroll
            for (int r = 0; r < 8; ++r) col[r] = R[r][j];
            uint8_t ob[8];
            idct_col<false>(col, ob);
#pragma unroll
            for (int r = 0; r < 8; ++r) rowd[2 * r + (j >> 2)] |= (uint32_t)ob[r] << (8 * (j & 3));
        }
    }
}
__device__ __forceinline__ void block_idct(const int4 (&c)[8], const uint32_t (&qw)[16], const int32_t* dcv,
                                           const BlkLoc& loc, uint32_t (&rowd)[16]) {
    int32_t R[8][8], hi, lo;
    block_dequant(c, qw, dcv, loc, R, hi, lo);
    block_transform(R, hi, lo, rowd);
}
template <class BlkN>
__device__ __forceinline__ void plane_units(const Desc& d, const int16_t* ac, const int32_t* dcv, const uint2* map,
                                            const uint32_t (&qw)[16], uint8_t* P, int stride, uint32_t nbx,
                                            uint32_t nby, uint32_t wid, uint32_t nw, BlkN blkn) {
    const uint32_t lane = threadIdx.x & 63;
    const uint32_t ucols = (nbx + 63) >> 6, nunits = ucols * nby;
    if (wid >= nunits) return;
    auto pend = [&](uint32_t u) {
        u = min(u, nunits - 1);
        const uint32_t by = u / ucols;
        const uint32_t bx = min(((u - by * ucols) << 6) + lane, nbx - 1);
        return blk_pend(d, map, blkn(bx, by));
    };
    auto unit = [&](uint32_t u, const int4 (&c)[8], const BlkLoc& l) {
        const uint32_t by = u / ucols, bx0 = (u - by * ucols) << 6;
        const uint32_t bx = min(bx0 + lane, nbx - 1);
        uint32_t rowd[16];
        block_idct(c, qw, dcv, l, rowd);
        uint8_t* const rowp = P + (int64_t)by * 8 * stride + (int64_t)bx0 * 8;
        const uint32_t lo = (bx - bx0) * 8;
#pragma unroll
        for (int r = 0; r < 8; ++r) {
            const uint2 v = make_uint2(rowd[2 * r], rowd[2 * r + 1]);
            nt_st(v, reinterpret_cast<uint2*>(rowp + (lo + (uint32_t)(r * stride))));
        }
    };
#if ICX_IDCT1_PF
    int4 ca[8], cb[8];
    BlkLoc la = blk_resolve(d, pend(wid)), lb;
    load_block8(ac, la.blk, ca);
    BlkPend pa, pb = pend(wid + nw);
    auto step = [&](uint32_t u, const int4 (&D)[8], const BlkLoc& lD, int4 (&Dn)[8], BlkLoc& lDn, const BlkPend& Pn,
                    BlkPend& Pa) {
        lDn = blk_resolve(d, Pn);
        load_block8(ac, lDn.blk, Dn);
        Pa = pend(u + 2 * nw);
        unit(u, D, lD);
    };
    for (uint32_t u = wid;;) {
        step(u, ca, la, cb, lb, pb, pa);
        if ((u += nw) >= nunits) break;
        step(u, cb, lb, ca, la, pa, pb);
        if ((u += nw) >= nunits) break;
    }
#else
    BlkPend p = pend(wid);
    for (uint32_t u = wid; u < nunits; u += nw) {
        const BlkLoc l = blk_resolve(d, p);
        int4 c[8];
        load_block8(ac, l.blk, c);
        p = pend(u + nw);
        unit(u, c, l);
    }
#endif
}
__global__ __launch_bounds__(256, ICX_IDCT1_MINW) void k_idct420s(const Desc* __restrict__ desc, const int16_t* __restrict__ ac,
                                                                   const int32_t* __restrict__ dcv, const uint2* __restrict__ map,
                                                                   uint8_t* __restrict__ planes, int64_t plane_cap, int luma) {
    const int img = blockIdx.y;
    const Desc& d = desc[img];
    if (!fused420(d)) return;
    const uint32_t wave = (uint32_t)wave_index();
    const uint32_t chunk0 = (gridDim.x & 7) ? blockIdx.x : (blockIdx.x & 7) * (gridDim.x >> 3) + (blockIdx.x >> 3);
    const uint32_t wid = chunk0 * 4 + wave, nw = gridDim.x * 4;
    const uint32_t mbw = (uint32_t)d.mbw, mbh = (uint32_t)d.mbh;
    uint8_t* const slot = planes + (int64_t)img * plane_cap;
    const uint32_t ynbx = 2 * mbw, yunits = luma ? ((ynbx + 63) >> 6) * (2 * mbh) : 0u;
    const uint32_t cnbx = mbw, cunits = ((cnbx + 63) >> 6) * mbh;
    auto first = [&](uint32_t base) { return wid >= base ? wid - base : (base - wid + nw - 1) / nw * nw + wid - base; };
    uint32_t qw[16];
    auto uniform_q = [&]() {
#pragma unroll
        for (int k = 0; k < 16; ++k) qw[k] = __builtin_amdgcn_readfirstlane(qw[k]);
    };
    if (wid < yunits) {
        load_qw_g(d.q[d.c[0].tq], qw);
        uniform_q();
        plane_units(d, ac, dcv, map, qw, slot, d.c[0].stride, ynbx, 2 * mbh, wid, nw, [&](uint32_t bx, uint32_t by) {
            return (int64_t)(((by >> 1) * mbw + (bx >> 1)) * 6 + ((by & 1) << 1) + (bx & 1));
        });
    }
#pragma unroll
    for (uint32_t cc = 0; cc < 2; ++cc) {
        const uint32_t f = first(yunits + cc * cunits);
        if (f >= cunits) continue;
        load_qw_g(d.q[d.c[1 + cc].tq], qw);
        uniform_q();
        plane_units(d, ac, dcv, map, qw, slot + comp_plane_off(d, 1 + cc), d.c[1 + cc].stride, cnbx, mbh, f, nw,
                    [&](uint32_t bx, uint32_t by) { return (int64_t)((by * mbw + bx) * 6 + 4 + cc); });
    }
}

__device__ __forceinline__ void lds_barrier() { asm volatile("s_waitcnt lgkmcnt(0)\n\ts_barrier" ::: "memory"); }

constexpr int kFB = 4;
__global__ __launch_bounds__(256) void k_fused420(const Desc* __restrict__ desc, const int16_t* __restrict__ ac,
                                                  const int32_t* __restrict__ dcv, const uint2* __restrict__ map,
                                                  const uint8_t* __restrict__ planes, int64_t plane_cap, uint8_t* __restrict__ out,
                                                  uint64_t out_stride) {
    const int img = blockIdx.y;
    const Desc& d = desc[img];
    if (!fused420(d)) return;
    __shared__ uint32_t Yl_all[4][16][64];
    __shared__ __attribute__((aligned(16))) uint8_t qz[64];
    const int t = threadIdx.x;
    if (t < 64) qz[t] = d.q[d.c[0].tq][t];
    __syncthreads();
    const int wave = __builtin_amdgcn_readfirstlane(t >> 6), lane = t & 63, h = lane & 1, k = (lane >> 1) & 3;
    uint32_t (*Yl)[64] = Yl_all[wave];
    int sbx, sby;
    (void)mcu_block_comp(d, k, sbx, sby);
    uint32_t qw[16];
    load_qw(qz, qw);
    const int W = d.W, H = d.H, mbw = d.mbw, mbh = d.mbh;
    const uint8_t* pslot = planes + (int64_t)img * plane_cap;
    const CPl c1{pslot + comp_plane_off(d, 1), d.c[1].w, d.c[1].h, d.c[1].stride};
    const CPl c2{pslot + comp_plane_off(d, 2), d.c[2].w, d.c[2].h, d.c[2].stride};
    uint8_t* o = out + (int64_t)img * out_stride;
    const StreamOut so{o, W, ((reinterpret_cast<uintptr_t>(o) & 3) == 0) && (W & 3) == 0};
    const int nsx = (mbw + 15) >> 4, nsy = (mbh + kFB - 1) / kFB, nstrip = nsx * nsy;
    for (int strip = blockIdx.x * 4 + wave; strip < nstrip; strip += gridDim.x * 4) {
        const int sy = strip / nsx, sx = strip - sy * nsx;
        const int mx0 = sx << 4, mb0 = sy * kFB, mb1 = min(mbh, mb0 + kFB);
        const int x0 = 256 * sx + 4 * lane, M = x0 >> 2;
        const bool xl = x0 < W;
        const int nb = min(4, W - x0) * 3;
        const bool f1 = M >= 1 && x0 + 3 <= 2 * c1.w - 4 && 2 * M + 5 < c1.s;
        const bool f2 = M >= 1 && x0 + 3 <= 2 * c2.w - 4 && 2 * M + 5 < c2.s;
        KvWin w;
        kv_init<true>(w, c1, c2, M, f1, f2, 8 * mb0);
        for (int mby = mb0; mby < mb1; ++mby) {
#pragma unroll
            for (int r2 = 0; r2 < 2; ++r2) {
                const int mq = (lane >> 3) + 8 * r2, mx = mx0 + mq;
                const bool live = mx < mbw;
                const int64_t n = ((int64_t)mby * mbw + (live ? mx : mbw - 1)) * 6 + k;
                int4 c[8];
                const BlkLoc l = blk_loc(d, map, n);
                load_block(ac, l.blk, h, c);
                uint32_t rowd[8];
                pair_idct(c, qw, h, dcv, l, rowd);
                if (live) {
                    const int lc = mq * 4 + sbx * 2 + h;
#pragma unroll
                    for (int r = 0; r < 8; ++r) Yl[sby * 8 + r][lc] = rowd[r];
                }
            }
            asm volatile("" ::: "memory");
            const int Y0 = 16 * mby, Y1 = min(H, Y0 + 16);
            if (xl) {
                auto luma = [&](int y) { return Yl[y - Y0][lane]; };
                auto emit = [&](int y, uint32_t yv, uint32_t cb, uint32_t cr) {
                    uint32_t w[3];
                    ycc4_to_rgb(yv, cb, cr, w);
                    so.put3(y, x0, w, nb);
                };
                kv_rows<true>(w, c1, c2, M, f1, f2, Y0, Y1, luma, emit);
            }
            asm volatile("" ::: "memory");
        }
    }
}

#ifndef ICX_FB5
#define ICX_FB5 4
#endif
#ifndef ICX_FUSED5_MINW
#define ICX_FUSED5_MINW 3
#endif
#ifndef ICX_F5_CARRY
#define ICX_F5_CARRY 1
#endif
#ifndef ICX_F5_PF
#define ICX_F5_PF 1
#endif
#ifndef ICX_F5_QV
#define ICX_F5_QV 0
#endif
#ifndef ICX_F5_QL
#define ICX_F5_QL 1
#endif
constexpr int kFB5 = ICX_FB5;
__global__ __launch_bounds__(256, ICX_FUSED5_MINW) void k_fused420s(const Desc* __restrict__ desc, const int16_t* __restrict__ ac,
                                                   const int32_t* __restrict__ dcv, const uint2* __restrict__ map,
                                                   const uint8_t* __restrict__ planes, int64_t plane_cap,
                                                   uint8_t* __restrict__ out, uint64_t out_stride) {
    const int img = blockIdx.y;
    const Desc& d = desc[img];
    if (!fused420(d)) return;
    __shared__ __attribute__((aligned(16))) uint32_t Yl_all[4][16][64];
    const int wave = wave_index(), lane = threadIdx.x & 63, mq = lane >> 2, k = lane & 3, sbx = k & 1, sby = k >> 1;
    uint32_t (*Yl)[64] = Yl_all[wave];
    uint32_t qw[16];
#if ICX_F5_QL
    __shared__ __attribute__((aligned(16))) uint32_t qlds[16];
    if (threadIdx.x < 16) qlds[threadIdx.x] = reinterpret_cast<const uint32_t*>(d.q[d.c[0].tq])[threadIdx.x];
    __syncthreads();
#endif
    load_qw_g(d.q[d.c[0].tq], qw);
#if ICX_F5_QV
#pragma unroll
    for (int k2 = 0; k2 < 16; ++k2) asm volatile("" : "+v"(qw[k2]));
#elif ICX_F5_QL
#else
#pragma unroll
    for (int k2 = 0; k2 < 16; ++k2) qw[k2] = __builtin_amdgcn_readfirstlane(qw[k2]);
#endif
    const int W = d.W, H = d.H, mbw = d.mbw, mbh = d.mbh;
    const uint8_t* pslot = planes + (int64_t)img * plane_cap;
    const CPl c1{pslot + comp_plane_off(d, 1), d.c[1].w, d.c[1].h, d.c[1].stride};
    const CPl c2{pslot + comp_plane_off(d, 2), d.c[2].w, d.c[2].h, d.c[2].stride};
    uint8_t* o = out + (int64_t)img * out_stride;
    const StreamOut so{o, W, ((reinterpret_cast<uintptr_t>(o) & 3) == 0) && (W & 3) == 0};
    const int nsx = (mbw + 15) >> 4, nsy = (mbh + kFB5 - 1) / kFB5, nstrip = nsx * nsy;
    uint8_t* const P0 = const_cast<uint8_t*>(pslot);
    const int s0 = d.c[0].stride;
    const int ef = edge_from(c1, c2, W);
    const bool conv = ef > 1;
    const uint32_t chunk0 = (gridDim.x & 7) ? blockIdx.x : (blockIdx.x & 7) * (gridDim.x >> 3) + (blockIdx.x >> 3);
    for (int strip = chunk0 * 4 + wave; strip < nstrip; strip += gridDim.x * 4) {
        const int sy = strip / nsx, sx = strip - sy * nsx;
        const int mx0 = sx << 4, mb0 = sy * kFB5, mb1 = min(mbh, mb0 + kFB5);
        const int M = 64 * sx + lane, x0 = 4 * M;
        const bool live = M >= 1 && M < ef;
        const bool border = x0 < W && !live;
        const int Mc = min(max(M, 1), max(ef - 1, 1));
        const int nb = live ? min(4, W - x0) * 3 : 0;
        const int mxl = min(mx0 + mq, mbw - 1);
        auto nblk = [&](int mby) { return ((int64_t)min(mby, mb1 - 1) * mbw + mxl) * 6 + k; };
        BlkPend p = blk_pend(d, map, nblk(mb0));
#if ICX_F5_CARRY
        KvWin w;
        if (conv) kv_init<true>(w, c1, c2, Mc, true, true, 8 * mb0);
#endif
#if ICX_F5_PF
        BlkLoc l = blk_resolve(d, p);
        int4 c[8];
        load_block8(ac, l.blk, c);
        p = blk_pend(d, map, nblk(mb0 + 1));
#endif
        for (int mby = mb0; mby < mb1; ++mby) {
            {
#if !ICX_F5_PF
                const BlkLoc l = blk_resolve(d, p);
                int4 c[8];
                load_block8(ac, l.blk, c);
                p = blk_pend(d, map, nblk(mby + 1));
#endif
                uint32_t rowd[16];
#if ICX_F5_QL
                {
                    asm volatile("" ::: "memory");
                    uint32_t qv[16];
#pragma unroll
                    for (int q4 = 0; q4 < 4; ++q4) {
                        const uint4 t4 = reinterpret_cast<const uint4*>(qlds)[q4];
                        qv[4 * q4] = t4.x;
                        qv[4 * q4 + 1] = t4.y;
                        qv[4 * q4 + 2] = t4.z;
                        qv[4 * q4 + 3] = t4.w;
                    }
                    block_idct(c, qv, dcv, l, rowd);
                }
#else
                block_idct(c, qw, dcv, l, rowd);
#endif
                uint2* dst = reinterpret_cast<uint2*>(&Yl[sby * 8][mq * 4 + sbx * 2]);
#pragma unroll
                for (int r = 0; r < 8; ++r) dst[r * 32] = make_uint2(rowd[2 * r], rowd[2 * r + 1]);
            }
#if ICX_F5_PF
            l = blk_resolve(d, p);
            load_block8(ac, l.blk, c);
            p = blk_pend(d, map, nblk(mby + 2));
#endif
            asm volatile("" ::: "memory");
            const int Y0 = 16 * mby, Y1 = min(H, Y0 + 16);
            if (border) {
                for (int y = Y0; y < Y1; ++y)
                    *reinterpret_cast<uint32_t*>(P0 + (int64_t)y * s0 + x0) = Yl[y - Y0][lane];
            }
            if (conv) {
                auto luma = [&](int y) { return Yl[y - Y0][lane]; };
                auto emit = [&](int y, uint32_t yv, uint32_t cb, uint32_t cr) {
                    uint32_t wo[3];
                    ycc4_to_rgb(yv, cb, cr, wo);
                    so.put3(y, 4 * Mc, wo, nb);
                };
#if !ICX_F5_CARRY
                KvWin w;
                kv_init<true>(w, c1, c2, Mc, true, true, Y0 >> 1);
#endif
                kv_rows<true>(w, c1, c2, Mc, true, true, Y0, Y1, luma, emit);
            }
            asm volatile("" ::: "memory");
        }
    }
}

#ifndef ICX_BACK_PP
#define ICX_BACK_PP 0
#endif
#ifndef ICX_BACK_MINW
#define ICX_BACK_MINW 4
#endif
constexpr int kBW = 16;
constexpr int kBRaw = 36;
struct BackLds {
    uint32_t y[3][16][64];
    uint32_t raw[2][2][8][kBRaw];
    uint32_t dbl[4][2][8][64];
    uint32_t q[3][16];
};
__global__ __launch_bounds__(256, ICX_BACK_MINW) void k_back420(const Desc* __restrict__ desc, const int16_t* __restrict__ ac,
                                                 const int32_t* __restrict__ dcv, const uint2* __restrict__ map,
                                                 uint8_t* __restrict__ out, uint64_t out_stride, int seg) {
    const int img = blockIdx.y;
    const Desc& d = desc[img];
    if (!fused420(d)) return;
    __shared__ __attribute__((aligned(16))) BackLds L;
    const int t = threadIdx.x;
    const int wave = __builtin_amdgcn_readfirstlane(t >> 6), lane = t & 63, p = t >> 1, h = t & 1;
    const int W = d.W, H = d.H, mbw = d.mbw, mbh = d.mbh;
    const int cw = d.c[1].w, chh = d.c[1].h, cs = d.c[1].stride;
    if (t < 48) L.q[t >> 4][t & 15] = reinterpret_cast<const uint32_t*>(d.q[d.c[t >> 4].tq])[t & 15];
    const int kb = p < 64 ? (p & 3) : (p < 96 ? 4 + ((p - 64) >> 4) : 4 + (p & 1));
    const int dmx = p < 64 ? (p >> 2) : (p < 96 ? (p & 15) : (p < 98 ? -1 : kBW));
    int sbx = 0, sby = 0;
    if (kb < 4) (void)mcu_block_comp(d, kb, sbx, sby);
    const uint8_t* qz = reinterpret_cast<const uint8_t*>(L.q[kb < 4 ? 0 : kb - 3]);
    uint8_t* o = out + (int64_t)img * out_stride;
    const StreamOut so{o, W, ((reinterpret_cast<uintptr_t>(o) & 3) == 0) && (W & 3) == 0};
    const int nsx = (mbw + kBW - 1) / kBW, nseg = (mbh + seg - 1) / seg, items = nsx * nseg;
    for (int it = blockIdx.x; it < items; it += gridDim.x) {
        const int sg = it / nsx, sx = it - sg * nsx;
        const int mx0 = sx * kBW, r0 = sg * seg, r1 = min(mbh, r0 + seg);
        const int lo = max(r0 - 1, 0), hi = min(r1, mbh - 1);
        const int M = 64 * sx + lane, x0 = 4 * M;
#ifdef ICX_EXP_BACK_NOSTORE
        uint32_t sink = 0;
#endif
        auto live_at = [&](int tr) {
            const int row = kb < 4 ? tr + 1 : tr + 2, mx = mx0 + dmx;
            return (kb < 4 ? row >= r0 && row < r1 : row >= lo && row <= hi) && p < 100 && mx >= 0 && mx < mbw;
        };
        auto pend_at = [&](int tr) {
            const int row = kb < 4 ? tr + 1 : tr + 2;
            const int mxc = min(max(mx0 + dmx, 0), mbw - 1), rowc = min(max(row, 0), mbh - 1);
#ifdef ICX_EXP_BACK_NOMAP
            return BlkPend{make_uint2(0, 0), d.acbase + ((int64_t)rowc * mbw + mxc) * 6 + kb};
#else
            return blk_pend(d, map, ((int64_t)rowc * mbw + mxc) * 6 + kb);
#endif
        };
        auto step = [&](int tr, const int4 (&D)[8], const BlkLoc& lD, int4 (&Dn)[8], BlkLoc& lDn, const BlkPend& Pn,
                        BlkPend& Pa) {
            const int ry = tr + 1, rc = tr + 2;
            const bool live = live_at(tr);
            if (__any(live)) {
                uint32_t qw[16];
                load_qw(qz, qw);
                uint32_t rowd[8];
                pair_idct(D, qw, h, dcv, lD, rowd);
                if (live) {
                    if (kb < 4) {
                        uint32_t* dst = &L.y[ry % 3][sby * 8][dmx * 4 + sbx * 2 + h];
#pragma unroll
                        for (int r = 0; r < 8; ++r) dst[r * 64] = rowd[r];
                    } else {
                        uint32_t* dst = &L.raw[rc & 1][kb - 4][0][(dmx + 1) * 2 + h];
#pragma unroll
                        for (int r = 0; r < 8; ++r) dst[r * kBRaw] = rowd[r];
                    }
                }
            }
            lDn = blk_resolve(d, Pn);
#ifndef ICX_EXP_BACK_NOLOAD
            load_block(ac, lDn.blk, h, Dn);
#endif
            Pa = pend_at(tr + 2);
            const int rd = tr + 1;
            if (rd >= lo && rd <= hi) {
                const bool interior = M >= 1 && x0 + 3 <= 2 * cw - 4;
#pragma unroll
                for (int j = 0; j < 4; ++j) {
                    const int task = wave * 4 + j, cc = task >> 3, r = task & 7;
                    const uint32_t* rw = L.raw[rd & 1][cc][r];
                    uint32_t v;
                    if (interior) {
                        const int b0 = ((2 * lane + 6) >> 2);
                        const uint64_t w = ((uint64_t)rw[b0] | ((uint64_t)rw[b0 + 1] << 32)) ^ 0x8080808080808080ull;
                        const uint64_t b = w >> ((lane & 1) ? 0 : 16);
                        const uint32_t w0 = (uint32_t)b, w1 = (uint32_t)(b >> 8), w2 = (uint32_t)(b >> 16);
                        v = pack4(dtap(w0, kTapRev), dtap(w1, kTapFwd), dtap(w1, kTapRev), dtap(w2, kTapFwd));
                    } else {
                        const uint8_t* rb = reinterpret_cast<const uint8_t*>(rw);
                        const int sh = 8 * mx0 - 8;
                        auto at = [&](int g) { return (int)rb[min(max(g - sh, 0), 4 * kBRaw - 1)]; };
                        v = pmap([&](int i) {
                            const int x = x0 + i;
                            if (x >= 2 * cw) return 0;
                            return (int)double_tap(x, cw, at, [&](int jj) { return at(cs - jj); });
                        });
                    }
                    L.dbl[rd & 3][cc][r][lane] = v;
                }
            }
#ifndef ICX_EXP_BACK_NOBAR
            lds_barrier();
#endif
            const int y0 = 16 * tr + 4 * wave;
            if (tr >= r0 && y0 < H) {
                const int k0 = y0 >> 1;
                const int nb = x0 < W ? min(4, W - x0) * 3 : 0;
                uint32_t A[2][6];
#pragma unroll
                for (int cc = 0; cc < 2; ++cc)
#pragma unroll
                    for (int i = 0; i < 6; ++i) {
                        const int r = min(max(k0 - 2 + i, 0), chh - 1);
                        A[cc][i] = L.dbl[(r >> 3) & 3][cc][r & 7][lane];
                    }
#pragma unroll
                for (int u = 0; u < 2; ++u) {
                    const int k = k0 + u, y = 2 * k;
                    if (y >= H) break;
                    uint32_t ev[2], od[2];
#pragma unroll
                    for (int cc = 0; cc < 2; ++cc) {
                        const uint32_t w0 = A[cc][u], w1 = A[cc][u + 1], w2 = A[cc][u + 2], w3 = A[cc][u + 3],
                                       w4 = A[cc][u + 4];
                        if (k >= 2 && k <= chh - 3) {
                            uint32_t e[4], f[4];
#pragma unroll
                            for (int i = 0; i < 4; ++i) {
                                e[i] = dtap(kv_column(w0, w1, w2, w3, i) ^ kBias8, kTapRev);
                                f[i] = dtap(kv_column(w1, w2, w3, w4, i) ^ kBias8, kTapFwd);
                            }
                            ev[cc] = pack4(e[0], e[1], e[2], e[3]);
                            od[cc] = pack4(f[0], f[1], f[2], f[3]);
                        } else {
                            ev[cc] = vtap_even(k, chh, w0, w1, w2, w3);
                            od[cc] = vtap_odd(k, chh, w1, w2, w3, w4);
                        }
                    }
                    const uint32_t(*Y)[64] = L.y[tr % 3];
                    uint32_t wv[3];
                    ycc4_to_rgb(Y[y - 16 * tr][lane], ev[0], ev[1], wv);
#ifdef ICX_EXP_BACK_NOSTORE
                    sink ^= wv[0] ^ wv[1] ^ wv[2];
#else
                    so.put3(y, x0, wv, nb);
#endif
                    if (y + 1 < H) {
                        ycc4_to_rgb(Y[y + 1 - 16 * tr][lane], od[0], od[1], wv);
#ifdef ICX_EXP_BACK_NOSTORE
                        sink ^= wv[0] ^ wv[1] ^ wv[2];
#else
                        so.put3(y + 1, x0, wv, nb);
#endif
                    }
                }
            }
        };
        lds_barrier();
#if ICX_BACK_PP
        int4 ca[8], cb[8];
        BlkLoc la = blk_resolve(d, pend_at(lo - 2)), lb;
        BlkPend pa, pb = pend_at(lo - 1);
        load_block(ac, la.blk, h, ca);
        for (int tr = lo - 2;;) {
            step(tr, ca, la, cb, lb, pb, pa);
            if (++tr >= r1) break;
            step(tr, cb, lb, ca, la, pa, pb);
            if (++tr >= r1) break;
        }
#else
        int4 ca[8];
        BlkLoc la = blk_resolve(d, pend_at(lo - 2));
        BlkPend pa = pend_at(lo - 1);
        load_block(ac, la.blk, h, ca);
        for (int tr = lo - 2; tr < r1; ++tr) step(tr, ca, la, ca, la, pa, pa);
#endif
#ifdef ICX_EXP_BACK_NOSTORE
        if (sink == 0x12345678u) o[lane] = 1;
#endif
    }
}

__global__ void k_finalize(int n, const Desc* __restrict__ desc, int32_t* __restrict__ status,
                           int32_t* __restrict__ dims) {
    const int i = blockIdx.x * blockDim.x + threadIdx.x;
    if (i >= n) return;
    const Desc& d = desc[i];
    const int st = d.status == kPending ? kInternalErr : d.status;
    status[i] = st;
    dims[3 * i + 0] = st == kOk ? d.W : 0;
    dims[3 * i + 1] = st == kOk ? d.H : 0;
    dims[3 * i + 2] = st == kOk ? (d.nc == 1 ? 1 : 3) : 0;
}

void launch_decode_front(const GroupWs& ws, int n, const uint8_t* d_data, const uint64_t* d_off,
                         const uint64_t* d_size, uint64_t out_stride, hipStream_t st, StageHook* hook, int part) {
    if (n <= 0) return;
    auto B = [&](Stage s) { if (hook) hook->begin(s, st); };
    auto E = [&](Stage s) { if (hook) hook->end(s, st); };
    if (part != kFrontRest) {
        B(kStParse);
        *ws.h_layout = 0;
        hipLaunchKernelGGL(k_parse, dim3(n), dim3(64), 0, st, n, d_data, d_off, d_size, ws.desc, ws.max_w, ws.max_h,
                           out_stride, ws.h_layout);
        E(kStParse);
    }
    launch_spec_entropy(ws, n, d_data, d_off, st, hook, part);
    if (part == kFrontFirst) return;
    B(kStEntropy);
    hipLaunchKernelGGL(k_entropy_seq, dim3(n), dim3(64), 0, st, n, d_data, d_off, ws.desc, ws.ac, ws.dc);
    E(kStEntropy);
}

void launch_decode_back(const GroupWs& ws, int n, uint8_t* d_out, uint64_t out_stride, int32_t* d_status,
                        int32_t* d_dims, hipStream_t st, StageHook* hook, bool known_layout) {
    if (n <= 0) return;
    const bool other = !known_layout || hipEventSynchronize(ws.ev_defer) != hipSuccess || *ws.h_layout != 0;
    auto B = [&](Stage s) { if (hook) hook->begin(s, st); };
    auto E = [&](Stage s) { if (hook) hook->end(s, st); };
    const int tb = 64, nb = (n + tb - 1) / tb;
    B(kStIdct);
    const int64_t maxblk = ws.coef_cap;
    static const int gwg = std::getenv("ICX_GENERIC_WG") ? std::max(8, std::atoi(std::getenv("ICX_GENERIC_WG"))) : kGenericWG;
    int gx = (int)std::max<int64_t>(1, std::min<int64_t>((maxblk + 32 * kIdctU - 1) / (32 * kIdctU), gwg / n));
    if (gx >= 8) gx &= ~7;
    const int fuse = [] {
        const int v = std::getenv("ICX_FUSE420") ? std::atoi(std::getenv("ICX_FUSE420")) : 5;
        return (v >= 0 && v <= 5) ? v : 5;
    }();
    if (other || fuse == 0) {
        hipLaunchKernelGGL(k_idct, dim3(gx, n), dim3(256), 0, st, ws.desc, ws.ac, ws.dc, ws.map, ws.planes, ws.plane_cap,
                           fuse);
        hipLaunchKernelGGL(k_idct_any, dim3(gx, n), dim3(256), 0, st, ws.desc, ws.ac, ws.dc, ws.map, ws.planes,
                           ws.plane_cap);
    }
    if (fuse == 4 || fuse == 5) {
        static const int upw = std::getenv("ICX_IDCT1_UPW") ? std::max(1, std::atoi(std::getenv("ICX_IDCT1_UPW"))) : 1;
        const int64_t units = (maxblk / 6) * (fuse == 4 ? 6 : 2) / 64 + 3;
        const int sgx = (int)std::max<int64_t>(1, std::min<int64_t>((units + 4 * upw - 1) / (4 * upw), 16384 / n)) & ~7;
        hipLaunchKernelGGL(k_idct420s, dim3(std::max(sgx, 8), n), dim3(256), 0, st, ws.desc, ws.ac, ws.dc, ws.map,
                           ws.planes, ws.plane_cap, fuse == 4 ? 1 : 0);
    }
    if (fuse == 1 || fuse == 2) {
        const int cgx = (int)std::max<int64_t>(1, std::min<int64_t>((maxblk / 6 / 16 + 31) / 32, 16384 / n)) & ~7;
        hipLaunchKernelGGL(k_idct420c, dim3(std::max(cgx, 8), n), dim3(256), 0, st, ws.desc, ws.ac, ws.dc, ws.map,
                           ws.planes, ws.plane_cap);
        if (fuse == 2) {
            const int ygx = (int)std::max<int64_t>(1, std::min<int64_t>((maxblk / 6 / 8 + 31) / 32, 16384 / n)) & ~7;
            hipLaunchKernelGGL(k_idct420y, dim3(std::max(ygx, 8), n), dim3(256), 0, st, ws.desc, ws.ac, ws.dc, ws.map,
                               ws.planes, ws.plane_cap);
        }
    }
    E(kStIdct);
    B(kStConvert);
    const int fgx = (int)std::max<int64_t>(1, std::min<int64_t>((((int64_t)(ws.max_w + 255) / 256) *
                                                                  ((ws.max_h + 16 * kFB - 1) / (16 * kFB)) + 3) / 4,
                                                                 16384 / n));
    if (fuse == 3) {
        const int seg = std::getenv("ICX_BSEG")
             ? std::max(1, std::atoi(std::getenv("ICX_BSEG"))) : 32;
        const int64_t items = (int64_t)((ws.max_w + 16 * kBW - 1) / (16 * kBW)) * (((ws.max_h + 15) / 16 + seg - 1) / seg);
        const int bgx = (int)std::max<int64_t>(1, std::min<int64_t>(items, 16384 / n));
        hipLaunchKernelGGL(k_back420, dim3(bgx, n), dim3(256), 0, st, ws.desc, ws.ac, ws.dc, ws.map, d_out, out_stride,
                           seg);
    }
    if (fuse == 1)
        hipLaunchKernelGGL(k_fused420, dim3(fgx, n), dim3(256), 0, st, ws.desc, ws.ac, ws.dc, ws.map, ws.planes,
                           ws.plane_cap, d_out, out_stride);
    if (fuse == 5) {
        const int64_t fs = ((int64_t)(ws.max_w + 255) / 256) * ((ws.max_h + 16 * kFB5 - 1) / (16 * kFB5));
        static const int spw = std::getenv("ICX_F5_SPW") ? std::max(1, std::atoi(std::getenv("ICX_F5_SPW"))) : 1;
        int f5 = (int)std::max<int64_t>(1, std::min<int64_t>((fs + 4 * spw - 1) / (4 * spw), 16384 / n));
        if (f5 >= 8) f5 &= ~7;
        hipLaunchKernelGGL(k_fused420s, dim3(f5, n), dim3(256), 0, st, ws.desc, ws.ac, ws.dc, ws.map, ws.planes,
                           ws.plane_cap, d_out, out_stride);
    }
    E(kStConvert);
    B(kStUpsample);
    const int ux = (int)std::max<int64_t>(1, std::min<int64_t>((ws.tmp_cap + 255) / 256, gwg / (3 * n)));
    for (int p = 0; p < 6 && other; ++p)
        hipLaunchKernelGGL(k_upsample, dim3(ux, n * 3), dim3(256), 0, st, ws.desc, ws.planes, ws.tmp, ws.plane_cap,
                           ws.tmp_cap, p);
    E(kStUpsample);
    B(kStConvert);
    const int cx = (int)std::max<int64_t>(1, std::min<int64_t>(((int64_t)ws.max_w * ws.max_h + 255) / 256, gwg / n));
    const int64_t sxw = ((int64_t)(ws.max_w + 255) / 256) * ((ws.max_h + kSH - 1) / kSH) / 4 + 1;
    const int sxg = (int)std::max<int64_t>(1, std::min<int64_t>(sxw, 16384 / n));
    const int sxo = (int)std::max<int64_t>(1, std::min<int64_t>(sxw, gwg / n));
    hipLaunchKernelGGL(k_convert_stream<3>, dim3(sxg, n), dim3(256), 0, st, ws.desc, ws.planes, ws.plane_cap, d_out,
                       out_stride, fuse);
    if (other) {
        hipLaunchKernelGGL(k_convert_stream<0>, dim3(sxo, n), dim3(256), 0, st, ws.desc, ws.planes, ws.plane_cap, d_out,
                           out_stride, fuse);
        hipLaunchKernelGGL(k_convert_stream<1>, dim3(sxo, n), dim3(256), 0, st, ws.desc, ws.planes, ws.plane_cap, d_out,
                           out_stride, fuse);
        hipLaunchKernelGGL(k_convert_stream<2>, dim3(sxo, n), dim3(256), 0, st, ws.desc, ws.planes, ws.plane_cap, d_out,
                           out_stride, fuse);
        hipLaunchKernelGGL(k_convert_stream<4>, dim3(sxo, n), dim3(256), 0, st, ws.desc, ws.planes, ws.plane_cap, d_out,
                           out_stride, fuse);
    }
    const int64_t egw = (4 * ((ws.max_h + kSHE - 1) / kSHE) + 255) / 256;
    const int egx = (int)std::max<int64_t>(1, std::min<int64_t>(egw, 16384 / n));
    const int ego = (int)std::max<int64_t>(1, std::min<int64_t>(egw, gwg / n));
    hipLaunchKernelGGL(k_convert_edge<3>, dim3(egx, n), dim3(256), 0, st, ws.desc, ws.planes, ws.plane_cap, d_out,
                       out_stride, fuse);
    if (other) {
        hipLaunchKernelGGL(k_convert_edge<1>, dim3(ego, n), dim3(256), 0, st, ws.desc, ws.planes, ws.plane_cap, d_out,
                           out_stride, fuse);
        hipLaunchKernelGGL(k_convert_fused, dim3(cx, n), dim3(256), 0, st, ws.desc, ws.planes, ws.plane_cap, d_out,
                           out_stride);
        hipLaunchKernelGGL(k_convert, dim3(cx, n), dim3(256), 0, st, ws.desc, ws.planes, ws.tmp, ws.plane_cap,
                           ws.tmp_cap, d_out, out_stride);
    }
    hipLaunchKernelGGL(k_finalize, dim3(nb), dim3(tb), 0, st, n, ws.desc, d_status, d_dims);
    E(kStConvert);
}

void launch_decode_group(const GroupWs& ws, int n, const uint8_t* d_data, const uint64_t* d_off,
                         const uint64_t* d_size, uint8_t* d_out, uint64_t out_stride, int32_t* d_status,
                         int32_t* d_dims, hipStream_t st, StageHook* hook) {
    launch_decode_front(ws, n, d_data, d_off, d_size, out_stride, st, hook);
    launch_decode_back(ws, n, d_out, out_stride, d_status, d_dims, st, hook, false);
}

}
```

imagecodecs_amd/csrc/icx_internal.h:

```cpp
#pragma once
#include <hip/hip_runtime.h>
#include <stdint.h>

#include <string>
#include <vector>

#include "icx_jpeg.h"

namespace icx {

constexpr int kTileBytes = 4096;
constexpr int kSubBytes = 2560;
constexpr int kMaxRounds = 8;
constexpr int kPoolPerSlotX4 = 10;
constexpr int kSubBytesSmall = 512;
constexpr int kRec = 16;
constexpr int kGenericWG = 4096;
constexpr int kGuessLead = 4096;
constexpr int kMaxRepair = 1024;
constexpr int kLanes = 256;
constexpr int kWriteLanesBig = 512;
constexpr int kSpecMaxBpm = 16;
enum : int32_t { kSpecSyntax = 1, kSpecGiveUp = 2 };

struct SpecImg {
    int32_t mode;
    int32_t err;
    int32_t ntiles, tile_base;
    int32_t nwg, wg_base;
    int32_t nsub, nrepair;
    int32_t nint, nrst;
    int32_t sub_bytes;
    int32_t gw_S;
    int64_t scan_len;
    int64_t ulen;
    int64_t errpos;
    int64_t total_blocks;
    int64_t uoff;
    int32_t ncount;
    int32_t dri_first;
    int64_t tail_G, tail_n;
    int32_t tail_p[3];
    int32_t kint;
};
struct TileRec { int32_t kept, end_err; int64_t end_at; int32_t nrst, pad_; };
struct SubRec { int32_t cnt, ds0, ds1, ds2; int32_t mism; };
struct RecState { uint32_t rel; int32_t b, cnt; int32_t ds[3]; };
struct LaneEntry { int64_t G; int32_t p0, p1, p2, pad; };

constexpr int kGwChunk = 32;
constexpr int kRecGw = kRec;
constexpr int64_t kGwMinPixels = 2048 * 2048;
constexpr int kGwMaxWalk = 64;
constexpr int kDriGwMin = 4096;
struct GwOut {
    uint64_t g0;
    int32_t k;
    int32_t ds[3];
    int32_t err;
    int32_t chunk0;
    int32_t nrec;
    int32_t over;
};
struct GcRec {
    int32_t chunk0;
    int32_t pad_;
    int32_t c;
    int32_t m;
    int32_t cds[3];
    int32_t err;
};

constexpr int16_t kDcEscape = INT16_MIN;
__host__ __device__ inline int16_t dc_cell(int32_t dc) {
    return (dc > -32768 && dc <= 32767) ? (int16_t)dc : kDcEscape;
}

struct GroupWs {
    int slots = 0;
    int max_w = 0, max_h = 0;
    int64_t coef_cap = 0;
    int64_t plane_cap = 0;
    int64_t tmp_cap = 0;
    Desc* desc = nullptr;
    int16_t* ac = nullptr;
    int32_t* dc = nullptr;
    uint8_t* planes = nullptr;
    uint8_t* tmp = nullptr;
    bool tmp_own = false;
    int64_t ucap = 0;
    int64_t upool = 0;
    int64_t tiles_cap = 0;
    int64_t lanes_cap = 0;
    SpecImg* spec = nullptr;
    int32_t* tilepre = nullptr;
    int32_t* wgpre = nullptr;
    int32_t* wg2pre = nullptr;
    int32_t* totals = nullptr;
    TileRec* tiles = nullptr;
    int32_t* tile_obase = nullptr;
    uint8_t* U = nullptr;
    uint64_t* X = nullptr;
    uint64_t* Y = nullptr;
    RecState* rec = nullptr;
    int32_t* nrec = nullptr;
    int32_t* guess_cnt = nullptr;
    int32_t* repair = nullptr;
    SubRec* sub = nullptr;
    int64_t rst_cap = 0;
    int64_t* rst = nullptr;
    int32_t* tile_rbase = nullptr;
    LaneEntry* ent = nullptr;
    struct StepSet* steps = nullptr;
    int32_t* stats = nullptr;
    int64_t pool_cap = 0;
    uint2* map = nullptr;
    int32_t* chunk_next = nullptr;
    unsigned long long* pool_next = nullptr;
    GwOut* gw = nullptr;
    GcRec* crec = nullptr;
    int2* clist = nullptr;
    int32_t* h_defer = nullptr;
    int32_t* h_layout = nullptr;
    hipEvent_t ev_defer = nullptr;
};

struct BlkLoc {
    int64_t blk;
    int32_t dcoff;
};
__device__ __forceinline__ BlkLoc blk_loc(const Desc& d, const uint2* map, int64_t n) {
    if (!d.mapped) return BlkLoc{d.acbase + n, 0};
    const uint2 e = map[d.acbase + n];
    return BlkLoc{(int64_t)e.x, (int32_t)e.y};
}
__device__ __forceinline__ int32_t blk_dc(int16_t cell, const int32_t* dcv, const BlkLoc& l) {
    int32_t v = cell;
    if (__any(cell == kDcEscape)) {
        const int32_t e = dcv[l.blk];
        v = cell == kDcEscape ? e : v;
    }
    return wadd(v, l.dcoff);
}
struct BlkPend {
    uint2 e;
    int64_t n;
};
__device__ __forceinline__ BlkPend blk_pend(const Desc& d, const uint2* map, int64_t n) {
    return BlkPend{map[d.acbase + n], d.acbase + n};
}
__device__ __forceinline__ BlkLoc blk_resolve(const Desc& d, const BlkPend& q) {
#ifdef ICX_EXP_BACK_NOMAP
    return BlkLoc{q.n, 0};
#else
    return d.mapped ? BlkLoc{(int64_t)q.e.x, (int32_t)q.e.y} : BlkLoc{q.n, 0};
#endif
}


int64_t ws_coef_cap(int w, int h);
int64_t ws_plane_cap(int w, int h);
int64_t ws_tmp_cap(int w, int h);

enum Stage { kStParse = 0, kStUnstuff, kStEntropy, kStWrite, kStIdct, kStUpsample, kStConvert, kStCount };
extern const char* const kStageNames[kStCount];
struct StageHook {
    virtual void begin(Stage s, hipStream_t st) = 0;
    virtual void end(Stage s, hipStream_t st) = 0;
    virtual ~StageHook() = default;
};

void launch_decode_group(const GroupWs& ws, int n, const uint8_t* d_data, const uint64_t* d_off,
                         const uint64_t* d_size, uint8_t* d_out, uint64_t out_stride, int32_t* d_status,
                         int32_t* d_dims, hipStream_t st, StageHook* hook);
enum { kFrontAll = 0, kFrontFirst = 1, kFrontRest = 2 };
void launch_decode_front(const GroupWs& ws, int n, const uint8_t* d_data, const uint64_t* d_off,
                         const uint64_t* d_size, uint64_t out_stride, hipStream_t st, StageHook* hook,
                         int part = kFrontAll);
void launch_decode_back(const GroupWs& ws, int n, uint8_t* d_out, uint64_t out_stride, int32_t* d_status,
                        int32_t* d_dims, hipStream_t st, StageHook* hook, bool known_layout = false);
void launch_spec_entropy(const GroupWs& ws, int n, const uint8_t* d_data, const uint64_t* d_off, hipStream_t st,
                         StageHook* hook, int part = kFrontAll);
enum { kRoundAll = 0, kRoundHead = 1, kRoundTail = 2, kRoundTailNoDri = 3, kRoundTailGw = 4 };
void launch_spec_round(const GroupWs& ws, int n, const uint8_t* d_data, const uint64_t* d_off, hipStream_t st,
                       StageHook* hook, int round, int last, int piece = kRoundAll);

struct Record {
    int32_t status, w, h, c;
    uint64_t checksum;
};
static_assert(sizeof(Record) == 24, "icx_record layout");
void launch_records(int n, const uint8_t* d_out, uint64_t out_stride, const int32_t* d_status, const int32_t* d_dims,
                    Record* d_rec, int max_w, int max_h, hipStream_t st);

bool tje_encode_gpu(hipStream_t st, int quality, int w, int h, int comps, const uint8_t* src,
                    std::vector<uint8_t>& out);
struct EncWs;
EncWs* enc_ws_create();
void enc_ws_destroy(EncWs* ws);
int enc_ws_stage_times(EncWs* ws, const char** names, float* ms, int cap);
bool jpeg_encode_gpu(hipStream_t st, int quality, int subsampling, int w, int h, int comps, const uint8_t* src,
                     std::vector<uint8_t>& out);
int jpeg_encode_device(hipStream_t st, EncWs* ws, int quality, int subsampling, int w, int h, int comps,
                       const uint8_t* d_src, uint8_t* d_out, uint64_t cap, uint64_t* size);
int jpeg_encode_device_batch(hipStream_t st, EncWs* ws, int n, int quality, int subsampling, int w, int h, int comps,
                             const uint8_t* const* d_srcs, uint8_t* d_out, uint64_t stride, uint64_t* sizes,
                             int32_t* status);

struct PngWs;
PngWs* png_ws_create();
void png_ws_destroy(PngWs* ws);
int png_ws_stage_times(PngWs* ws, const char** names, float* ms, int cap);
int png_encode_device_batch(int k, hipStream_t* sts, PngWs** wss, int n, int w, int h, int d,
                            const uint8_t* const* d_srcs, uint8_t* d_out, uint64_t stride, uint64_t* sizes,
                            int32_t* status);
int png_encode_device(hipStream_t st, PngWs* ws, int w, int h, int d, const uint8_t* d_src, uint8_t* d_out,
                      uint64_t cap, uint64_t* size);
bool png_encode_gpu(hipStream_t st, int w, int h, int d, const uint8_t* src, std::vector<uint8_t>& out);

enum : int32_t {
    kHdrOk = 0, kHdrNotRadiance = 1, kHdrBadHeader = 2, kHdrMalformed = 3, kHdrTruncated = 4, kHdrTooLarge = 5,
    kHdrPending = 6
};
struct HdrDesc {
    int32_t status, w, h, rows;
    int64_t ds, size;
    int32_t has_marker;
    int32_t not_flat;
    int32_t ncand, new_ok;
    int32_t mode;
    int32_t pad_;
};
struct HdrWs {
    int max_images = 0, max_w = 0, max_h = 0;
    HdrDesc* desc = nullptr;
    int32_t* cq = nullptr;
    int32_t* ce = nullptr;
    int64_t* start = nullptr;
    uint8_t* kind = nullptr;
    uint8_t* planes = nullptr;
};
int hdr_probe(const uint8_t* data, int64_t size, int* w, int* h);
int64_t hdr_ws_bytes(int max_images, int max_w, int max_h);
bool hdr_ws_alloc(HdrWs& ws, int max_images, int max_w, int max_h);
void hdr_ws_free(HdrWs& ws);
void launch_hdr_decode(const HdrWs& ws, int n, const uint8_t* d_data, const uint64_t* d_off, const uint64_t* d_size,
                       float* d_out, uint64_t out_stride, int32_t* d_status, int32_t* d_dims, hipStream_t st,
                       StageHook* hook);

struct ExrWs;
ExrWs* exr_ws_create();
void exr_ws_destroy(ExrWs* w);
int exr_decode(hipStream_t st, ExrWs& ws, const uint8_t* data, size_t size, const uint8_t* d_file, float* d_out,
               size_t out_floats, float** out_rgba, int* width, int* height, std::string& err);
int exr_decode_batch(hipStream_t st, ExrWs& ws, int n, const uint8_t* const* data, const uint8_t* const* d_data,
                     const size_t* sizes, float* const* d_out, const size_t* out_floats, int32_t* codes, int32_t* widths,
                     int32_t* heights, std::string& err);
int exr_probe(const uint8_t* data, size_t size, int* width, int* height);

}
```

imagecodecs_amd/csrc/icx_spec.hip:

```cpp
#include <hip/hip_runtime.h>
#include <rocprim/warp/warp_scan.hpp>

#include <algorithm>
#include <cstdlib>
#include <type_traits>

#include "icx_spec_core.h"

namespace icx {

__device__ int block_exclusive_scan(int v, int* sh) {
    const int t = threadIdx.x;
    sh[t] = v;
    __syncthreads();
    for (int o = 1; o < (int)blockDim.x; o <<= 1) {
        const int x = t >= o ? sh[t - o] : 0;
        __syncthreads();
        sh[t] += x;
        __syncthreads();
    }
    const int incl = sh[t];
    __syncthreads();
    return incl - v;
}

__global__ __launch_bounds__(1024) void k_spec_plan(int n, const uint8_t* __restrict__ data, const uint64_t* __restrict__ off,
                                                    Desc* __restrict__ desc, SpecImg* __restrict__ spec,
                                                    int32_t* __restrict__ tilepre, int32_t* __restrict__ wgpre,
                                                    int32_t* __restrict__ wg2pre, int32_t* __restrict__ totals,
                                                    int64_t upool, int64_t lanes_cap, int sub_bytes, int64_t pool_cap,
                                                    unsigned long long* __restrict__ pool_next, int gw, int round,
                                                    int last_round, int32_t* __restrict__ defer_out, int dri_min) {
    __shared__ int sh[1024];
    __shared__ int last[7];
    if (round > 0) {
        int any = 0;
        for (int i = threadIdx.x; i < n; i += blockDim.x) any |= spec[i].mode == 4;
        if (!__syncthreads_or(any)) {
            if (threadIdx.x == 0) {
                totals[0] = totals[1] = totals[2] = 0;
                tilepre[n] = wgpre[n] = wg2pre[n] = 0;
                if (defer_out) defer_out[0] = defer_out[1] = defer_out[2] = 0;
            }
            return;
        }
    }
    int carry_t = 0, carry_w = 0, carry_w2 = 0, carry_u = 0, carry_c = 0, carry_r = 0, carry_a = 0, carry_d = 0, carry_i = 0, carry_k = 0;
    const int64_t pool_units = upool >> 12, wg_cap = lanes_cap / kLanes;
    for (int i0 = 0; i0 < n; i0 += blockDim.x) {
        const int i = i0 + threadIdx.x;
        const int64_t scan_len = i < n ? desc[i].size - desc[i].scan_off : 0;
        const bool mine = i < n && (round == 0 || spec[i].mode == 4);
        const bool cand = mine && desc[i].status == kPending && desc[i].nc >= 1 && desc[i].bpm <= kSpecMaxBpm &&
                          scan_len > 0 && scan_len < ((int64_t)1 << 40);
        int nt = 0, nw = 0, nw2 = 0, nu = 0, kint = 0;
        int64_t sb = kSubBytes, nsub = 0, nlanes = 0;
        if (cand) {
            const Desc& d = desc[i];
            nu = (int)min<int64_t>((scan_len + 64 + 4095) >> 12, INT32_MAX / 4);
            nt = (int)ustf_ntiles(scan_len, ustf_align(data + off[i] + d.scan_off));
            const int64_t nmcu = (int64_t)d.mbw * d.mbh;
            sb = sub_bytes;
            if (sb <= 0) {
                const int64_t smax = sub_bytes < 0 ? -(int64_t)sub_bytes : kSubBytes;
                const int64_t full = (int64_t)kWriteLanesBig * smax;
                const int64_t nwg = (scan_len + full - 1) / full;
                sb = (scan_len + nwg * kWriteLanesBig - 1) / (nwg * kWriteLanesBig);
                sb = min<int64_t>(smax, max<int64_t>(kSubBytesSmall, (sb + 15) & ~15));
            }
            nsub = d.restart == 0 ? (scan_len + sb - 1) / sb : (nmcu + d.restart - 1) / d.restart;
            if (d.restart != 0 && gw && dri_min > 0 && scan_len / nsub >= dri_min && min_mcu_bits(d) >= 8) {
                const int64_t avg = scan_len / nsub;
                kint = (int)min<int64_t>(64, max<int64_t>(2, (avg + kSubBytes - 1) / kSubBytes));
                sb = (avg + kint - 1) / kint;
            }
            nlanes = kint ? nsub * kint : nsub;
            nw = (int)min<int64_t>((nlanes + kLanes - 1) / kLanes, INT32_MAX / 4);
            nw2 = (int)((nlanes + kWriteLanesBig - 1) / kWriteLanesBig);
        }
        const int nwc = cand && (desc[i].restart == 0 || kint) ? nw : 0;
        const int eu = block_exclusive_scan(nu, sh);
        const int ec = block_exclusive_scan(nwc, sh);
        const bool ok = cand && (int64_t)carry_u + eu + nu <= pool_units && (int64_t)carry_c + ec + nwc <= wg_cap;
        if (threadIdx.x == blockDim.x - 1) { last[3] = eu + nu; last[4] = ec + nwc; }
        if (!ok) nt = nw = nw2 = 0;
        const int nwr = ok ? nwc : 0;
        const int er = block_exclusive_scan(nwr, sh);
        if (threadIdx.x == blockDim.x - 1) last[5] = er + nwr;
        const int64_t tb = i < n && desc[i].status == kPending ? (int64_t)desc[i].mbw * desc[i].mbh * desc[i].bpm : 0;
        const bool gwr = gw && cand && (desc[i].restart == 0 || kint), gwi = gwr && ok;
        const int32_t gS = gwr ? (int32_t)((tb * 11 / 10 + nlanes - 1) / nlanes + 1) : 0;
        const int64_t region = gwr ? nlanes * gS : tb;
        const int na = round ? 0 : (int)min<int64_t>((region + kGwChunk - 1) / kGwChunk, INT32_MAX / 4);
        const int ea = block_exclusive_scan(na, sh);
        if (threadIdx.x == blockDim.x - 1) last[6] = ea + na;
        if (mine) {
            const Desc& d = desc[i];
            SpecImg& s = spec[i];
            s.mode = ok ? (d.restart == 0 || kint ? 1 : 3) : (cand && !last_round ? 4 : 0);
            s.err = 0;
            s.nrepair = 0;
            s.ncount = 0;
            s.dri_first = INT32_MAX;
            s.nrst = 0;
            s.sub_bytes = ok ? (int32_t)sb : kSubBytes;
            s.uoff = ((int64_t)carry_u + eu) << 12;
            s.ulen = 0;
            s.scan_len = ok ? scan_len : 0;
            s.total_blocks = ok ? (int64_t)d.mbw * d.mbh * d.bpm : 0;
            s.nint = ok && (s.mode == 3 || kint) ? (int32_t)nsub : 0;
            s.kint = ok ? kint : 0;
            s.ntiles = nt;
            s.nwg = nw;
            s.gw_S = gS;
            Desc& dd = desc[i];
            if (round == 0) dd.acbase = ((int64_t)carry_a + ea) * kGwChunk;
            dd.mapped = gwi;
            if (round == 0 && dd.acbase + region > pool_cap && dd.status == kPending) {
                dd.status = kOutOfMem;
                s.mode = 0;
                dd.mapped = 0;
            }
        }
        carry_d += __syncthreads_count(mine && !ok && cand && !last_round);
        carry_i += __syncthreads_count(ok && desc[i].restart != 0 && !kint);
        carry_k += __syncthreads_count(ok && kint);
        const int et = block_exclusive_scan(nt, sh);
        const int ew = block_exclusive_scan(nw, sh);
        const int ew2 = block_exclusive_scan(nw2, sh);
        if (i < n) {
            tilepre[i] = carry_t + et;
            wgpre[i] = carry_w + ew;
            wg2pre[i] = carry_w2 + ew2;
            spec[i].tile_base = carry_t + et;
            spec[i].wg_base = carry_r + er;
        }
        if (threadIdx.x == blockDim.x - 1) { last[0] = et + nt; last[1] = ew + nw; last[2] = ew2 + nw2; }
        __syncthreads();
        carry_t += last[0];
        carry_w += last[1];
        carry_w2 += last[2];
        carry_u = min(carry_u + last[3], INT32_MAX / 4);
        carry_c = min(carry_c + last[4], INT32_MAX / 4);
        carry_r += last[5];
        carry_a = min(carry_a + last[6], INT32_MAX / 4);
        __syncthreads();
    }
    if (threadIdx.x == 0) {
        tilepre[n] = carry_t;
        wgpre[n] = carry_w;
        wg2pre[n] = carry_w2;
        totals[0] = carry_t;
        totals[1] = carry_w;
        totals[2] = carry_w2;
        if (round == 0) *pool_next = (unsigned long long)carry_a * kGwChunk;
        if (defer_out) {
            defer_out[0] = carry_d;
            defer_out[1] = carry_i;
            defer_out[2] = carry_k;
        }
    }
}

__device__ __forceinline__ int find_image(const int32_t* pre, int n, int x) {
    int lo = 0, hi = n - 1;
    while (lo < hi) {
        const int mid = (lo + hi + 1) >> 1;
        if (pre[mid] <= x) lo = mid; else hi = mid - 1;
    }
    return lo;
}

__device__ __forceinline__ int wave_incl_scan(int v) {
    using WScan = rocprim::warp_scan<int, 64>;
    typename WScan::storage_type st;
    int r;
    WScan().inclusive_scan(v, r, st);
    return r;
}
__device__ __forceinline__ long long wave_min_ll(long long v) {
#pragma unroll
    for (int o = 32; o > 0; o >>= 1) v = min(v, __shfl_xor(v, o));
    return v;
}

struct TileRange {
    int t, t1, i;
};
__device__ __forceinline__ TileRange wave_tiles(const int32_t* tilepre, int n, int total) {
    const int nw = gridDim.x * (blockDim.x >> 6),
              w = __builtin_amdgcn_readfirstlane((int)(blockIdx.x * (blockDim.x >> 6) + (threadIdx.x >> 6)));
    const int per = (total + nw - 1) / nw;
    TileRange r;
    r.t = min(total, w * per);
    r.t1 = min(total, r.t + per);
    r.i = r.t < r.t1 ? find_image(tilepre, n, r.t) : 0;
    return r;
}

struct ChunkIn {
    uint32_t D[4];
    int nx;
    int prun;
};
struct TileChunks {
    uint4 V0, V1, V2, V3;
    uint32_t pw, nx3;
    int r;
    __device__ __forceinline__ void load(const uint8_t* R, int64_t L, int64_t t0, int lane) {
        static_assert(kTileBytes == 4096, "four 1 KiB rounds");
        const int64_t alast = ((int64_t)(ustf_align(R) + L - 1) & ~(int64_t)15) - ustf_align(R);
        auto ld = [&](int64_t a) {
            const uint4 v = gload16(R + (a < L ? a : alast));
            return a < L ? v : make_uint4(0u, 0u, 0u, 0u);
        };
        const int64_t a0 = t0 + lane * 16;
        V0 = ld(a0); V1 = ld(a0 + 1024); V2 = ld(a0 + 2048); V3 = ld(a0 + 3072);
        const uint32_t p = gload4(R + t0 - 4);
        pw = t0 >= 1 ? p : 0u;
        const int64_t an = t0 + kTileBytes;
        const uint32_t q = gload4(R + (an < L ? an : alast));
        nx3 = an < L ? q : 0u;
        r = 0;
    }
    __device__ __forceinline__ ChunkIn next(int64_t a, int lane) {
        ChunkIn c;
        c.D[0] = V0.x; c.D[1] = V0.y; c.D[2] = V0.z; c.D[3] = V0.w;
        uint32_t p = __shfl_up(V0.w, 1);
        if (lane == 0) p = pw;
        uint32_t nw = __shfl_down(V0.x, 1);
        const uint32_t q = __shfl(V1.x, 0);
        if (lane == 63) nw = r == 3 ? nx3 : q;
        pw = __shfl(V0.w, 63);
        V0 = V1; V1 = V2; V2 = V3;
        ++r;
        c.nx = (int)(nw & 0xFFu);
        c.prun = ff_run4(p, a);
        return c;
    }
};
__device__ __forceinline__ int wave_sum(int v) { return __shfl(wave_incl_scan(v), 63); }

struct TileImg {
    int i, t_first, t_end;
    const uint8_t* R;
    int64_t L;
    __device__ __forceinline__ void set(int img, const uint8_t* data, const uint64_t* off, const Desc* desc,
                                        const SpecImg* spec, const int32_t* tilepre) {
        i = __builtin_amdgcn_readfirstlane(img);
        t_first = __builtin_amdgcn_readfirstlane(tilepre[i]);
        t_end = __builtin_amdgcn_readfirstlane(tilepre[i + 1]);
        R = data + off[i] + desc[i].scan_off;
        L = spec[i].scan_len;
    }
    __device__ __forceinline__ int64_t t0(int t) const {
        return (int64_t)(t - t_first) * kTileBytes - ustf_align(R);
    }
};

__global__ __launch_bounds__(256) void k_ustf_count(int n, const uint8_t* __restrict__ data,
                                                    const uint64_t* __restrict__ off, const Desc* __restrict__ desc,
                                                    SpecImg* __restrict__ spec, const int32_t* __restrict__ tilepre,
                                                    const int32_t* __restrict__ totals, TileRec* __restrict__ tiles) {
    const int lane = threadIdx.x & 63;
    const TileRange tr = wave_tiles(tilepre, n, totals[0]);
    TileImg im, imn;
    TileChunks tc, tn;
    if (tr.t < tr.t1) {
        im.set(tr.i, data, off, desc, spec, tilepre);
        tc.load(im.R, im.L, im.t0(tr.t), lane);
    }
    imn = im;
    for (int t = tr.t; t < tr.t1; ++t) {
        if (t + 1 < tr.t1) {
            while (t + 1 >= imn.t_end) imn.set(imn.i + 1, data, off, desc, spec, tilepre);
            tn.load(imn.R, imn.L, imn.t0(t + 1), lane);
        }
        const int i = im.i;
        const uint8_t* R = im.R;
        const int64_t L = im.L;
        const int64_t t0 = im.t0(t);
        int32_t giveup = 0;
        int kept = 0, nrst = 0, err = 0;
        long long tend = LLONG_MAX;
        for (int r = 0; r < kTileBytes / 1024 && t0 + r * 1024 < L; ++r) {
            const int64_t a = t0 + r * 1024 + lane * 16;
            RstSink rs{0, 0, nullptr, 0, 0};
            const ChunkIn c = tc.next(a, lane);
            const Ustf16 u = ustf16<false>(R, L, a, c.D, c.nx, c.prun, &giveup, &rs);
            if (__any(u.end_at >= 0)) {
                const long long e = wave_min_ll(u.end_at >= 0 ? (long long)u.end_at : LLONG_MAX);
                const bool before = u.end_at >= 0 ? u.end_at <= e : a < e;
                kept += before ? u.kept : 0;
                nrst += before ? rs.n : 0;
                const uint64_t owner = __ballot(u.end_at >= 0 && u.end_at == e);
                err = __shfl(u.end_err, __ffsll((long long)owner) - 1);
                tend = e;
                break;
            }
            kept += u.kept;
            nrst += rs.n;
        }
        kept = wave_sum(kept);
        nrst = __any(nrst) ? wave_sum(nrst) : 0;
        if (__any(giveup) && lane == 0) atomicOr(&spec[i].err, kSpecGiveUp);
        if (lane == 0) {
            TileRec rec;
            rec.kept = kept;
            rec.end_at = tend == LLONG_MAX ? -1 : tend;
            rec.end_err = tend == LLONG_MAX ? 0 : err;
            rec.nrst = nrst;
            rec.pad_ = 0;
            tiles[t] = rec;
        }
        tc = tn;
        im = imn;
    }
}

__global__ __launch_bounds__(256) void k_ustf_scan(int n, SpecImg* __restrict__ spec, TileRec* __restrict__ tiles,
                                                   int32_t* __restrict__ tile_obase, int32_t* __restrict__ tile_rbase,
                                                   uint8_t* __restrict__ U) {
    __shared__ int sh[256];
    __shared__ int s_first_end;
    const int i = blockIdx.x;
    if (i >= n) return;
    SpecImg& s = spec[i];
    if (s.mode != 1 && s.mode != 3) return;
    if (threadIdx.x == 0) s_first_end = INT32_MAX;
    __syncthreads();
    for (int t = threadIdx.x; t < s.ntiles; t += blockDim.x)
        if (tiles[s.tile_base + t].end_at >= 0) atomicMin(&s_first_end, t);
    __syncthreads();
    const int fe = s_first_end;
    int64_t carry = 0;
    int32_t rcarry = 0;
    for (int t0 = 0; t0 < s.ntiles; t0 += blockDim.x) {
        const int t = t0 + threadIdx.x;
        const bool in = t < s.ntiles && t <= fe;
        const int k = in ? tiles[s.tile_base + t].kept : 0;
        const int nr = in ? tiles[s.tile_base + t].nrst : 0;
        const int ex = block_exclusive_scan(k, sh);
        const int rex = block_exclusive_scan(nr, sh);
        if (t < s.ntiles) {
            tile_obase[s.tile_base + t] = (int32_t)(carry + ex);
            tile_rbase[s.tile_base + t] = rcarry + rex;
        }
        __shared__ int s_sum, s_rsum;
        if (threadIdx.x == blockDim.x - 1) { s_sum = ex + k; s_rsum = rex + nr; }
        __syncthreads();
        carry += s_sum;
        rcarry += s_rsum;
        __syncthreads();
    }
    {
        uint8_t* u = U + s.uoff;
        for (int64_t p = carry + threadIdx.x; p < u_pad_end(carry); p += blockDim.x) u[p] = 0xFF;
    }
    if (threadIdx.x == 0) {
        s.ulen = carry;
        s.nrst = rcarry;
        s.errpos = (fe != INT32_MAX && tiles[s.tile_base + fe].end_err) ? carry : INT64_MAX;
        const int64_t nsub = carry > 0 ? (carry + s.sub_bytes - 1) / s.sub_bytes : 1;
        s.nsub = s.mode == 3 ? s.nint : (s.kint > 0 ? s.nint * s.kint : (int32_t)nsub);
    }
}

__global__ __launch_bounds__(256) void k_ustf_write(int n, const uint8_t* __restrict__ data,
                                                    const uint64_t* __restrict__ off, const Desc* __restrict__ desc,
                                                    const SpecImg* __restrict__ spec, const int32_t* __restrict__ tilepre,
                                                    const int32_t* __restrict__ totals, const TileRec* __restrict__ tiles,
                                                    const int32_t* __restrict__ tile_obase,
                                                    const int32_t* __restrict__ tile_rbase, uint8_t* __restrict__ U,
                                                    int64_t* __restrict__ rst, int64_t rst_cap) {
    constexpr int kBufW = kTileBytes / 4 + 8;
    __shared__ uint32_t sbuf_all[4][kBufW];
    const int lane = threadIdx.x & 63;
    uint32_t* sbuf = sbuf_all[threadIdx.x >> 6];
    const uint8_t* sb = reinterpret_cast<const uint8_t*>(sbuf);
    const TileRange tr = wave_tiles(tilepre, n, totals[0]);
    TileImg im, imn;
    TileChunks tc, tn;
    int64_t ulen = 0;
    int32_t obv = 0;
    if (tr.t < tr.t1) {
        im.set(tr.i, data, off, desc, spec, tilepre);
        tc.load(im.R, im.L, im.t0(tr.t), lane);
    }
    imn = im;
    for (int t = tr.t; t < tr.t1; ++t) {
        if (t + 1 < tr.t1) {
            while (t + 1 >= imn.t_end) imn.set(imn.i + 1, data, off, desc, spec, tilepre);
            tn.load(imn.R, imn.L, imn.t0(t + 1), lane);
        }
        ulen = spec[im.i].ulen;
        if (spec[im.i].mode != 1 && spec[im.i].mode != 3) ulen = 0;
        if (t == tr.t || ((t - tr.t) & 63) == 0) obv = tr.t + ((t - tr.t) & ~63) + lane < tr.t1 ? tile_obase[t + lane] : 0;
        const int i = im.i;
        const int64_t obase = __shfl(obv, (t - tr.t) & 63);
        if (obase >= 0 && obase < ulen) {
        const uint8_t* R = im.R;
        const int64_t L = im.L;
        const int64_t t0 = im.t0(t);
        for (int k = lane; k < kBufW / 4; k += 64) reinterpret_cast<uint4*>(sbuf)[k] = make_uint4(0u, 0u, 0u, 0u);
        __builtin_amdgcn_wave_barrier();
        int32_t giveup = 0;
        int kept = 0, nrst = 0;
        for (int r = 0; r < kTileBytes / 1024 && t0 + r * 1024 < L; ++r) {
            const int64_t a = t0 + r * 1024 + lane * 16;
            RstSink rs0{0, 0, nullptr, 0, 0};
            const ChunkIn c = tc.next(a, lane);
            const Ustf16 u = ustf16<true>(R, L, a, c.D, c.nx, c.prun, &giveup, &rs0);
            const long long e = __any(u.end_at >= 0) ? wave_min_ll(u.end_at >= 0 ? (long long)u.end_at : LLONG_MAX)
                                                     : LLONG_MAX;
            const bool before = u.end_at >= 0 ? u.end_at <= e : a < e;
            const int k = before ? u.kept : 0;
            const int incl = wave_incl_scan(k);
            const int nr = before ? rs0.n : 0;
            if (__any(nr)) {
                const int rincl = wave_incl_scan(nr);
                if (nr) {
                    RstSink rs{0, obase + kept + (incl - k), rst + (int64_t)i * rst_cap, tile_rbase[t] + nrst + rincl - nr,
                               (int32_t)min<int64_t>(rst_cap, INT32_MAX)};
                    (void)ustf16<false>(R, L, a, c.D, c.nx, c.prun, &giveup, &rs);
                }
                nrst += __shfl(rincl, 63);
            }
            if (k) {
                const int ob = kept + incl - k, q = ob >> 2, sft = ob & 3;
                const uint32_t* d = u.out;
                if (k == 16 && (ob & 15) == 0) {
                    reinterpret_cast<uint4*>(sbuf)[q >> 2] = make_uint4(d[0], d[1], d[2], d[3]);
                } else if (sft == 0) {
#pragma unroll
                    for (int j = 0; j < 4; ++j) atomicOr(&sbuf[q + j], d[j]);
                } else {
                    atomicOr(&sbuf[q], d[0] << (8 * sft));
#pragma unroll
                    for (int j = 1; j < 4; ++j) atomicOr(&sbuf[q + j], __builtin_amdgcn_alignbyte(d[j], d[j - 1], 4 - sft));
                    atomicOr(&sbuf[q + 4], d[3] >> (32 - 8 * sft));
                }
            }
            kept += __shfl(incl, 63);
            if (e != LLONG_MAX) break;
        }
        __builtin_amdgcn_wave_barrier();
        const int64_t nout = min<int64_t>(kept, ulen - obase);
        uint8_t* dst = U + spec[i].uoff + obase;
        const int head = (int)min<int64_t>(nout, (16 - (obase & 15)) & 15);
        const int nunit = (int)((nout - head) >> 4);
        const int tail0 = head + nunit * 16;
        if (lane < head) dst[lane] = sb[lane];
        if (lane < nout - tail0) dst[tail0 + lane] = sb[tail0 + lane];
        for (int u = lane; u < nunit; u += 64) {
            const int b0 = head + 16 * u, shb = (b0 & 3) * 8;
            const uint32_t* q = sbuf + (b0 >> 2);
            uint32_t v[4];
#pragma unroll
            for (int j = 0; j < 4; ++j) v[j] = (uint32_t)((((uint64_t)q[j + 1] << 32) | q[j]) >> shb);
            *reinterpret_cast<uint4*>(dst + b0) = make_uint4(v[0], v[1], v[2], v[3]);
        }
        __builtin_amdgcn_wave_barrier();
        }
        tc = tn;
        im = imn;
    }
}

constexpr uint64_t kTsAgg = 1, kTsInc = 2;
constexpr int kTsRstBits = 21;
__device__ __forceinline__ uint64_t ts_pack(uint64_t flag, bool end, int64_t nrst, int64_t kept) {
    return flag << 62 | (uint64_t)end << 61 | (uint64_t)nrst << 40 | (uint64_t)kept;
}
__device__ __forceinline__ int64_t ts_kept(uint64_t v) { return (int64_t)(v & (((uint64_t)1 << 40) - 1)); }
__device__ __forceinline__ int64_t ts_rst(uint64_t v) { return (int64_t)((v >> 40) & ((1u << kTsRstBits) - 1)); }
__device__ __forceinline__ bool ts_end(uint64_t v) { return (v >> 61) & 1; }
__device__ __forceinline__ long long wave_sum_ll(long long v) {
#pragma unroll
    for (int o = 32; o > 0; o >>= 1) v += __shfl_xor(v, o);
    return v;
}
__device__ __forceinline__ int find_image_wave(const int32_t* pre, int n, int t, int lane) {
    if (n > 4096) return find_image(pre, n, t);
    const int step = (n + 63) >> 6;
    const int k = lane * step;
    const uint64_t m = __ballot(k < n && pre[min(k, n - 1)] <= t);
    const int base = (63 - __clzll((long long)m)) * step;
    const int k2 = base + lane;
    const uint64_t m2 = __ballot(lane < step && k2 < n && pre[min(k2, n - 1)] <= t);
    return base + 63 - __clzll((long long)m2);
}
constexpr int kTsSpinMax = 1 << 22;

__global__ __launch_bounds__(256) void k_ustf_one(int n, const uint8_t* __restrict__ data, const uint64_t* __restrict__ off,
                                                  const Desc* __restrict__ desc, SpecImg* __restrict__ spec,
                                                  const int32_t* __restrict__ tilepre, const int32_t* __restrict__ totals,
                                                  uint64_t* __restrict__ tstate, uint8_t* __restrict__ U,
                                                  int64_t* __restrict__ rst, int64_t rst_cap) {
    constexpr int kBufW = kTileBytes / 4 + 8;
    __shared__ uint32_t sbuf_all[4][kBufW];
    const int lane = threadIdx.x & 63;
    uint32_t* sbuf = sbuf_all[threadIdx.x >> 6];
    const uint8_t* sb = reinterpret_cast<const uint8_t*>(sbuf);
    const int total = totals[0];
    unsigned int* ticket = reinterpret_cast<unsigned int*>(tstate + total);
    auto take = [&]() {
        int v = 0;
        if (lane == 0) v = (int)atomicAdd(ticket, 1u);
        return __builtin_amdgcn_readfirstlane(__shfl(v, 0));
    };
    auto ts_load = [&](int q) { return __hip_atomic_load(tstate + q, __ATOMIC_RELAXED, __HIP_MEMORY_SCOPE_AGENT); };
    auto ts_store = [&](int q, uint64_t v) {
        if (lane == 0) __hip_atomic_store(tstate + q, v, __ATOMIC_RELAXED, __HIP_MEMORY_SCOPE_AGENT);
    };
    TileImg im, imn;
    TileChunks tc, tn;
    int t = take();
    if (t < total) {
        im.set(find_image_wave(tilepre, n, t, lane), data, off, desc, spec, tilepre);
        tc.load(im.R, im.L, im.t0(t), lane);
    }
    while (t < total) {
        const int i = im.i;
        SpecImg& s = spec[i];
        const bool on = s.mode == 1 || s.mode == 3;
        const uint8_t* R = im.R;
        const int64_t L = im.L;
        const int64_t t0 = im.t0(t);
        for (int k = lane; k < kBufW / 4; k += 64) reinterpret_cast<uint4*>(sbuf)[k] = make_uint4(0u, 0u, 0u, 0u);
        __builtin_amdgcn_wave_barrier();
        int32_t giveup = 0;
        int kept = 0, nrst = 0, end_err = 0;
        bool own_end = false;
        for (int r = 0; on && r < kTileBytes / 1024 && t0 + r * 1024 < L; ++r) {
            const int64_t a = t0 + r * 1024 + lane * 16;
            RstSink rs0{0, 0, nullptr, 0, 0};
            const ChunkIn c = tc.next(a, lane);
            const Ustf16 u = ustf16<true>(R, L, a, c.D, c.nx, c.prun, &giveup, &rs0);
            const long long e = __any(u.end_at >= 0) ? wave_min_ll(u.end_at >= 0 ? (long long)u.end_at : LLONG_MAX)
                                                     : LLONG_MAX;
            const bool before = u.end_at >= 0 ? u.end_at <= e : a < e;
            const int k = before ? u.kept : 0;
            const int incl = wave_incl_scan(k);
            nrst += before ? rs0.n : 0;
            if (k) {
                const int ob = kept + incl - k, q = ob >> 2, sft = ob & 3;
                const uint32_t* d = u.out;
                if (k == 16 && (ob & 15) == 0) {
                    reinterpret_cast<uint4*>(sbuf)[q >> 2] = make_uint4(d[0], d[1], d[2], d[3]);
                } else if (sft == 0) {
#pragma unroll
                    for (int j = 0; j < 4; ++j) atomicOr(&sbuf[q + j], d[j]);
                } else {
                    atomicOr(&sbuf[q], d[0] << (8 * sft));
#pragma unroll
                    for (int j = 1; j < 4; ++j) atomicOr(&sbuf[q + j], __builtin_amdgcn_alignbyte(d[j], d[j - 1], 4 - sft));
                    atomicOr(&sbuf[q + 4], d[3] >> (32 - 8 * sft));
                }
            }
            kept += __shfl(incl, 63);
            if (e != LLONG_MAX) {
                const uint64_t owner = __ballot(u.end_at >= 0 && u.end_at == e);
                end_err = __shfl(u.end_err, __ffsll((long long)owner) - 1);
                own_end = true;
                break;
            }
        }
        nrst = __any(nrst) ? wave_sum(nrst) : 0;
        if (__any(giveup) && lane == 0) atomicOr(&s.err, kSpecGiveUp);
        ts_store(t, ts_pack(kTsAgg, own_end, min(nrst, (1 << kTsRstBits) - 1), kept));
        const int tnx = take();
        if (tnx < total) {
            imn.set(find_image_wave(tilepre, n, tnx, lane), data, off, desc, spec, tilepre);
            tn.load(imn.R, imn.L, imn.t0(tnx), lane);
        }
        int64_t pk = 0, pr = 0, ak = 0, ar = 0;
        bool pe = false, ae = false, stuck = false;
        for (int p = t - 1;; p -= 64) {
            const int q = p - lane;
            uint64_t v = ts_pack(kTsInc, false, 0, 0);
            if (q >= im.t_first) {
                int spins = 0;
                for (v = ts_load(q); (v >> 62) == 0 && spins < kTsSpinMax; ++spins) {
                    __builtin_amdgcn_s_sleep(1);
                    v = ts_load(q);
                }
                if ((v >> 62) == 0) {
                    stuck = true;
                    v = ts_pack(kTsInc, false, 0, 0);
                }
            }
            const uint64_t mi = __ballot((v >> 62) == kTsInc);
            const int m = mi ? __ffsll((long long)mi) - 1 : 64;
            const uint64_t vm = __shfl(v, m & 63);
            if (m < 64 && ts_end(vm)) {
                pk = ts_kept(vm);
                pr = ts_rst(vm);
                pe = true;
                break;
            }
            const uint64_t me = __ballot(lane < m && ts_end(v));
            const int e = me ? 63 - __clzll((long long)me) : -1;
            const bool in = lane < m && lane >= (e < 0 ? 0 : e);
            const int64_t wk = wave_sum_ll(in ? ts_kept(v) : 0), wr = wave_sum_ll(in ? ts_rst(v) : 0);
            if (e >= 0) { ak = wk; ar = wr; ae = true; }
            else { ak += wk; ar += wr; }
            if (m < 64) {
                pk = ts_kept(vm) + ak;
                pr = ts_rst(vm) + ar;
                pe = ae;
                break;
            }
        }
        if (__any(stuck) && lane == 0) atomicOr(&s.err, kSpecGiveUp);
        const int64_t ik = pe ? pk : pk + kept, ir = pe ? pr : pr + nrst;
        if (ir >= (1 << kTsRstBits) && lane == 0) atomicOr(&s.err, kSpecGiveUp);
        ts_store(t, ts_pack(kTsInc, pe || own_end, min<int64_t>(ir, (1 << kTsRstBits) - 1), ik));
        __builtin_amdgcn_wave_barrier();
        if (on && !pe) {
            const int64_t obase = pk;
            if (nrst) {
                TileChunks t2;
                t2.load(R, L, t0, lane);
                int kk = 0, nr_done = 0;
                int32_t gdummy = 0;
                for (int r = 0; r < kTileBytes / 1024 && t0 + r * 1024 < L; ++r) {
                    const int64_t a = t0 + r * 1024 + lane * 16;
                    RstSink rs0{0, 0, nullptr, 0, 0};
                    const ChunkIn c = t2.next(a, lane);
                    const Ustf16 u = ustf16<false>(R, L, a, c.D, c.nx, c.prun, &gdummy, &rs0);
                    const long long e = __any(u.end_at >= 0) ? wave_min_ll(u.end_at >= 0 ? (long long)u.end_at : LLONG_MAX)
                                                             : LLONG_MAX;
                    const bool before = u.end_at >= 0 ? u.end_at <= e : a < e;
                    const int k = before ? u.kept : 0;
                    const int incl = wave_incl_scan(k);
                    const int nr = before ? rs0.n : 0;
                    if (__any(nr)) {
                        const int rincl = wave_incl_scan(nr);
                        if (nr) {
                            RstSink rs{0, obase + kk + (incl - k), rst + (int64_t)i * rst_cap, (int32_t)(pr + nr_done + rincl - nr),
                                       (int32_t)min<int64_t>(rst_cap, INT32_MAX)};
                            (void)ustf16<false>(R, L, a, c.D, c.nx, c.prun, &gdummy, &rs);
                        }
                        nr_done += __shfl(rincl, 63);
                    }
                    kk += __shfl(incl, 63);
                    if (e != LLONG_MAX) break;
                }
            }
            const int64_t nout = kept;
            uint8_t* dst = U + s.uoff + obase;
            const int head = (int)min<int64_t>(nout, (16 - (obase & 15)) & 15);
            const int nunit = (int)((nout - head) >> 4);
            const int tail0 = head + nunit * 16;
            if (lane < head) dst[lane] = sb[lane];
            if (lane < nout - tail0) dst[tail0 + lane] = sb[tail0 + lane];
            for (int u = lane; u < nunit; u += 64) {
                const int b0 = head + 16 * u, shb = (b0 & 3) * 8;
                const uint32_t* q = sbuf + (b0 >> 2);
                uint32_t v[4];
#pragma unroll
                for (int j = 0; j < 4; ++j) v[j] = (uint32_t)((((uint64_t)q[j + 1] << 32) | q[j]) >> shb);
                *reinterpret_cast<uint4*>(dst + b0) = make_uint4(v[0], v[1], v[2], v[3]);
            }
            if (own_end || t == im.t_end - 1) {
// ... 718 lines not shown
    if (i >= n) return;
    SpecImg& s = spec[i];
    if (s.mode != 1 || s.ncount == 0) return;
    stage_tab(SS.scan, steps[i].scan);
    stage_tab(SS.write, steps[i].write);
    __syncthreads();
    const int64_t base = (int64_t)s.wg_base * kLanes;
    for (int q = threadIdx.x; q < s.ncount; q += blockDim.x) {
        const int64_t j = clist[base + q].y;
        const int64_t f = base + j;
        uint64_t ex = 0;
        int32_t give_up = 0;
        gw_count_lane(desc[i], s, SS, U, j, f, X[f - 1], gwo[f], rec + f * kRec, ac, dcv, chunk_next, pool_next, pool_cap,
                      crec, &ex, &give_up, rst + (int64_t)i * rst_cap, min<int64_t>(s.nrst, rst_cap));
        if (give_up) atomicOr(&s.err, kSpecGiveUp);
        Y[f] = ex;
        if (crec[f].m < 0 && j + 1 < s.nsub && ex != X[f] && !(s.kint > 0 && (j + 1) % s.kint == 0)) {
            const int r = atomicAdd(&s.nrepair, 1);
            if (r < kMaxRepair) repair[(int64_t)i * kMaxRepair + r] = (int32_t)j;
        }
    }
}

__global__ __launch_bounds__(64) void k_gw_repair(int n, const Desc* __restrict__ desc, SpecImg* __restrict__ spec,
                                                  const StepSet* __restrict__ steps, const uint8_t* __restrict__ U,
                                                  uint64_t* __restrict__ X, const uint64_t* __restrict__ Y,
                                                  const GwOut* __restrict__ gwo, const RecState* __restrict__ rec,
                                                  int16_t* __restrict__ ac, int32_t* __restrict__ dcv,
                                                  int32_t* __restrict__ chunk_next, unsigned long long* __restrict__ pool_next,
                                                  int64_t pool_cap, GcRec* __restrict__ crec, int32_t* __restrict__ repair,
                                                  const int64_t* __restrict__ rst, int64_t rst_cap) {
    const int i = blockIdx.x;
    if (i >= n || threadIdx.x != 0) return;
    SpecImg& s = spec[i];
    if (s.mode != 1 || s.nrepair == 0) return;
    const int64_t* RS = rst + (int64_t)i * rst_cap;
    const int64_t nrst = min<int64_t>(s.nrst, rst_cap);
    auto give_up_walk = [&] {
        if (s.kint > 0) dri_gw_fallback(s);
        else s.mode = 2;
    };
    if (s.nrepair > kMaxRepair) { give_up_walk(); return; }
    int32_t* q = repair + (int64_t)i * kMaxRepair;
    const int nq = s.nrepair;
    for (int a = 1; a < nq; ++a) {
        const int32_t v = q[a];
        int c = a - 1;
        while (c >= 0 && q[c] > v) { q[c + 1] = q[c]; --c; }
        q[c + 1] = v;
    }
    const int64_t base = (int64_t)s.wg_base * kLanes;
    int64_t done = -1;
    for (int a = 0; a < nq; ++a) {
        const int64_t j = q[a];
        if (j <= done) continue;
        X[base + j] = Y[base + j];
        int64_t k = j + 1;
        for (int steps_ = 0; k < s.nsub; ++k, ++steps_) {
            if (s.kint > 0 && k % s.kint == 0) break;
            if (steps_ >= kGwMaxWalk) { give_up_walk(); return; }
            const int64_t f = base + k;
            if (gwo[f].g0 == X[f - 1]) {
                GcRec c;
                c.chunk0 = -1; c.pad_ = 0; c.c = 0; c.m = -2; c.cds[0] = c.cds[1] = c.cds[2] = 0; c.err = INT32_MAX;
                crec[f] = c;
                break;
            }
            uint64_t ex = 0;
            int32_t give_up = 0;
            gw_count_lane(desc[i], s, steps[i], U, k, f, X[f - 1], gwo[f], rec + f * kRec, ac, dcv, chunk_next, pool_next,
                          pool_cap, crec, &ex, &give_up, RS, nrst);
            if (give_up) { give_up_walk(); return; }
            if (crec[f].m >= 0 || k + 1 == s.nsub || ex == X[f]) break;
            X[f] = ex;
        }
        done = k;
    }
}

__global__ __launch_bounds__(256) void k_gw_scan(int n, Desc* __restrict__ desc, SpecImg* __restrict__ spec,
                                                 const GwOut* __restrict__ gwo, const GcRec* __restrict__ crec,
                                                 const RecState* __restrict__ rec, LaneEntry* __restrict__ ent,
                                                 const uint64_t* __restrict__ X, const uint64_t* __restrict__ Y,
                                                 const uint8_t* __restrict__ U, const int64_t* __restrict__ rst,
                                                 int64_t rst_cap) {
    __shared__ int sh[256];
    __shared__ int s_cnt, s_d0, s_d1, s_d2;
    __shared__ int s_bad;
    const int i = blockIdx.x;
    if (i >= n) return;
    SpecImg& s = spec[i];
    if (s.mode != 1) return;
    if (s.kint > 0) {
        const int64_t K = s.kint, nint = s.nint, base = (int64_t)s.wg_base * kLanes;
        const int64_t iblk = (int64_t)desc[i].restart * desc[i].bpm;
        const int64_t* RS = rst + (int64_t)i * rst_cap;
        const int64_t nrst = min<int64_t>(s.nrst, rst_cap);
        if (threadIdx.x == 0) s_bad = (s.err & kSpecGiveUp) != 0 || nrst < nint - 1;
        __syncthreads();
        const bool give_up = s_bad != 0;
        for (int64_t m = threadIdx.x; m < nint && !give_up; m += blockDim.x) {
            const int64_t G0 = m * iblk;
            int32_t cnt = 0, p0 = 0, p1 = 0, p2 = 0;
            bool bad = false;
            for (int64_t ii = 0; ii < K; ++ii) {
                const int64_t f = base + m * K + ii;
                const GwOut g = gwo[f];
                const GcRec c = crec[f];
                int32_t d[3];
                const int32_t nb = gw_lane_total(g, c, rec + f * kRec, d);
                const int32_t e = gw_lane_err(g, c, rec + f * kRec);
                LaneEntry le;
                le.G = G0 + cnt;
                le.p0 = p0;
                le.p1 = p1;
                le.p2 = p2;
                le.pad = nb;
                ent[f] = le;
                if (e != INT32_MAX && le.G + e < s.total_blocks) bad = true;
                cnt += nb;
                p0 = wadd(p0, d[0]);
                p1 = wadd(p1, d[1]);
                p2 = wadd(p2, d[2]);
                if (ii == K - 1 && m + 1 < nint) {
                    const uint64_t ex = c.m == -1 ? Y[f] : X[f];
                    const int64_t em = RS[m] >> 3, p = st_pos(ex);
                    if (st_b(ex) != 0 || p < em * 8 - 7 || p > em * 8) bad = true;
                    if (dri_end_kind(U + s.uoff, s.ulen, s.errpos, em, m, RS[m]) != kDriExact) bad = true;
                }
            }
            if (m + 1 < nint ? cnt != iblk : cnt < s.total_blocks - G0) bad = true;
            if (bad) atomicOr(&s_bad, 1);
        }
        __syncthreads();
        if (threadIdx.x == 0) {
            s.tail_n = 0;
            if (s_bad) dri_gw_fallback(s);
        }
        return;
    }
    if (s.err & kSpecGiveUp) {
        if (threadIdx.x == 0) { s.mode = 2; desc[i].mapped = 0; }
        return;
    }
    if (threadIdx.x == 0) s_bad = 0;
    __syncthreads();
    const int64_t base = (int64_t)s.wg_base * kLanes;
    int64_t G = 0;
    int32_t P0 = 0, P1 = 0, P2 = 0;
    for (int64_t j0 = 0; j0 < s.nsub; j0 += blockDim.x) {
        const int64_t j = j0 + threadIdx.x;
        const bool live = j < s.nsub;
        int32_t cnt = 0, d[3] = {0, 0, 0}, e = INT32_MAX;
        if (live) {
            const GwOut g = gwo[base + j];
            const GcRec c = crec[base + j];
            cnt = gw_lane_total(g, c, rec + (base + j) * kRec, d);
            e = gw_lane_err(g, c, rec + (base + j) * kRec);
        }
        const int ec = block_exclusive_scan(cnt, sh);
        const int e0 = block_exclusive_scan(d[0], sh);
        const int e1 = block_exclusive_scan(d[1], sh);
        const int e2 = block_exclusive_scan(d[2], sh);
        if (live) {
            LaneEntry le;
            le.G = G + ec;
            le.p0 = wadd(P0, e0);
            le.p1 = wadd(P1, e1);
            le.p2 = wadd(P2, e2);
            le.pad = cnt;
            ent[base + j] = le;
            if (e != INT32_MAX && le.G + e < s.total_blocks) atomicOr(&s_bad, 1);
        }
        if (threadIdx.x == blockDim.x - 1) {
            s_cnt = ec + cnt;
            s_d0 = wadd(e0, d[0]);
            s_d1 = wadd(e1, d[1]);
            s_d2 = wadd(e2, d[2]);
        }
        __syncthreads();
        G += s_cnt;
        P0 = wadd(P0, s_d0);
        P1 = wadd(P1, s_d1);
        P2 = wadd(P2, s_d2);
        __syncthreads();
    }
    if (threadIdx.x == 0) {
        s.tail_n = 0;
        if (s_bad) {
            s.err |= kSpecSyntax;
        } else if (G < s.total_blocks) {
            s.tail_G = G;
            s.tail_n = s.total_blocks - G;
            s.tail_p[0] = P0;
            s.tail_p[1] = P1;
            s.tail_p[2] = P2;
        }
    }
}

__global__ __launch_bounds__(64) void k_gw_tail(int n, Desc* __restrict__ desc, SpecImg* __restrict__ spec,
                                                const StepSet* __restrict__ steps, const uint8_t* __restrict__ U,
                                                const uint64_t* __restrict__ X, const uint64_t* __restrict__ Y,
                                                const GcRec* __restrict__ crec, int16_t* __restrict__ ac,
                                                int32_t* __restrict__ dcv, int32_t* __restrict__ chunk_next,
                                                unsigned long long* __restrict__ pool_next, int64_t pool_cap,
                                                uint2* __restrict__ map) {
    const int i = blockIdx.x;
    if (i >= n || threadIdx.x != 0) return;
    SpecImg& s = spec[i];
    if (s.mode != 1 || s.tail_n == 0 || (s.err & kSpecSyntax)) return;
    Desc& d = desc[i];
    const int64_t last = (int64_t)s.wg_base * kLanes + s.nsub - 1;
    const uint64_t entry = crec[last].m == -1 ? Y[last] : X[last];
    const Sel S = make_sel(d);
    ChainSink sink{ac, dcv, chunk_next, pool_next, pool_cap, -1, -1, 0};
    int32_t ds[3], err;
    const int32_t got = gw_tail(U + s.uoff, s.ulen, steps[i].write, d.huff, S, entry, s.tail_n,
                                s.errpos == INT64_MAX ? INT64_MAX : s.errpos * 8, sink, ds, &err);
    if (got < 0) { s.mode = 2; d.mapped = 0; return; }
    if (err != INT32_MAX) { s.err |= kSpecSyntax; return; }
    GwSlots ts{0, 0, -1, 0};
    for (int32_t t = 0; t < got; ++t) {
        const int64_t nb = s.tail_G + t;
        const int ci = S.comp((int)(nb % d.bpm));
        map[d.acbase + nb] = make_uint2((uint32_t)ts.addr(t, sink.chunk0, chunk_next), (uint32_t)s.tail_p[ci]);
    }
}

__global__ __launch_bounds__(256) void k_gw_map(int n, const Desc* __restrict__ desc, const SpecImg* __restrict__ spec,
                                                const int32_t* __restrict__ wpre, const int32_t* __restrict__ totals,
                                                const GwOut* __restrict__ gwo, const GcRec* __restrict__ crec,
                                                const RecState* __restrict__ rec, const LaneEntry* __restrict__ ent,
                                                const int32_t* __restrict__ chunk_next, uint2* __restrict__ map) {
    const int lane = threadIdx.x & 63, wave = __builtin_amdgcn_readfirstlane((int)(threadIdx.x >> 6));
    const int64_t nchunks = (int64_t)totals[1] * (kLanes / 64);
    for (int64_t C = (int64_t)blockIdx.x * 4 + wave; C < nchunks; C += (int64_t)gridDim.x * 4) {
        const int grp = (int)(C / (kLanes / 64));
        const int i = find_image(wpre, n, grp);
        const SpecImg& s = spec[i];
        if (s.mode != 1 || (s.err & kSpecSyntax)) continue;
        const int64_t j0 = (int64_t)(grp - wpre[i]) * kLanes + (C % (kLanes / 64)) * 64;
        if (j0 >= s.nsub) continue;
        const Desc& d = desc[i];
        const Sel S = make_sel(d);
        const int32_t Sst = s.gw_S;
        const int64_t j = j0 + lane;
        const bool live = j < s.nsub;
        const int64_t f = (int64_t)s.wg_base * kLanes + (live ? j : j0);
        const GwOut g = gwo[f];
        const GcRec c = crec[f];
        const LaneEntry le = ent[f];
        int32_t P0 = le.p0, P1 = le.p1, P2 = le.p2, Q0 = P0, Q1 = P1, Q2 = P2, m0 = 0;
        if (c.m >= 0) {
            const RecState e = rec[f * kRec + c.m];
            m0 = e.cnt;
            Q0 = wadd(P0, wsub(c.cds[0], e.ds[0]));
            Q1 = wadd(P1, wsub(c.cds[1], e.ds[1]));
            Q2 = wadd(P2, wsub(c.cds[2], e.ds[2]));
        }
        const int32_t cc = c.m != -2 ? c.c : 0;
        const int64_t nb = live ? min<int64_t>(le.pad, s.total_blocks - le.G) : 0;
        const int nl = (int)min<int64_t>(64, s.nsub - j0);
        for (int q = 0; q < nl; ++q) {
            const int64_t G = __shfl(le.G, q), nbq = __shfl(nb, q);
            const int32_t ccq = __shfl(cc, q), m0q = __shfl(m0, q), c0q = __shfl(c.chunk0, q), g0q = __shfl(g.chunk0, q);
            const int32_t p0 = __shfl(P0, q), p1 = __shfl(P1, q), p2 = __shfl(P2, q);
            const int32_t q0 = __shfl(Q0, q), q1 = __shfl(Q1, q), q2 = __shfl(Q2, q);
            const int64_t sbase = d.acbase + (j0 + q) * Sst;
            GwSlots gs{sbase, Sst, -1, 0}, cs{0, 0, -1, 0};
            for (int64_t t = lane; t < nbq; t += 64) {
                const int ci = S.comp((int)((G + t) % d.bpm));
                uint2 e;
                if (t < ccq) {
                    e.x = (uint32_t)cs.addr((int32_t)t, c0q, chunk_next);
                    e.y = (uint32_t)(ci == 0 ? p0 : (ci == 1 ? p1 : p2));
                } else {
                    e.x = (uint32_t)gs.addr((int32_t)(t - ccq + m0q), g0q, chunk_next);
                    e.y = (uint32_t)(ci == 0 ? q0 : (ci == 1 ? q1 : q2));
                }
                map[d.acbase + G + t] = e;
            }
        }
    }
}

__global__ void k_spec_finish(int n, Desc* __restrict__ desc, SpecImg* __restrict__ spec,
                              int32_t* __restrict__ stats) {
    const int i = blockIdx.x * blockDim.x + threadIdx.x;
    if (i >= n) return;
    SpecImg& s = spec[i];
    if (s.mode == 4 || s.mode == 5) return;
    if (s.mode == 3 && s.dri_first != INT32_MAX)
        s.err |= (s.dri_first & 1) ? kSpecGiveUp : kSpecSyntax;
    if (s.mode == 3 && (s.err & kSpecGiveUp)) s.mode = 2;
    if (s.mode != 1) desc[i].mapped = 0;
    if (s.mode == 1 || s.mode == 3) desc[i].status = (s.err & kSpecSyntax) ? kSyntaxError : kOk;
    if (s.mode == 1 || s.mode == 3) atomicAdd(&stats[0], 1);
    else if (s.mode == 2) atomicAdd(&stats[1], 1);
    else if (desc[i].status == kPending) atomicAdd(&stats[2], 1);
    s.mode = 5;
}

void launch_spec_entropy(const GroupWs& ws, int n, const uint8_t* d_data, const uint64_t* d_off, hipStream_t st,
                         StageHook* hook, int part) {
    const int rounds = [] {
        const char* e = std::getenv("ICX_ROUNDS");
        return e ? std::max(1, std::min(8, std::atoi(e))) : kMaxRounds;
    }();
    if (part == kFrontFirst) {
        launch_spec_round(ws, n, d_data, d_off, st, hook, 0, rounds == 1, kRoundHead);
        return;
    }
    if (part == kFrontRest) {
        const bool known = hipEventSynchronize(ws.ev_defer) == hipSuccess;
        launch_spec_round(ws, n, d_data, d_off, st, hook, 0, rounds == 1,
                          !known || ws.h_defer[1] != 0 ? kRoundTail : ws.h_defer[2] != 0 ? kRoundTailGw : kRoundTailNoDri);
        if (!known) return;
    }
    for (int r = part == kFrontRest ? 1 : 0; r < rounds; ++r) {
        if (part == kFrontRest) {
            if (hipEventSynchronize(ws.ev_defer) != hipSuccess || ws.h_defer[0] == 0) break;
        }
        launch_spec_round(ws, n, d_data, d_off, st, hook, r, r + 1 == rounds, kRoundAll);
    }
}

void launch_spec_round(const GroupWs& ws, int n, const uint8_t* d_data, const uint64_t* d_off, hipStream_t st,
                       StageHook* hook, int round, int last, int piece) {
    auto B = [&](Stage s) { if (hook) hook->begin(s, st); };
    auto E = [&](Stage s) { if (hook) hook->end(s, st); };
    static const int g0 = std::getenv("ICX_EGRID") ? std::max(1, std::atoi(std::getenv("ICX_EGRID"))) : 2048;
    const int g = round == 0 ? g0 : std::max(32, g0 / 32);
    static const int lead = std::getenv("ICX_GUESS_LEAD") ? std::max(0, std::atoi(std::getenv("ICX_GUESS_LEAD"))) : -1;
    static const int sub_env = std::getenv("ICX_SUB_BYTES") ? std::max(kSubBytesSmall, std::atoi(std::getenv("ICX_SUB_BYTES"))) & ~15
                               : std::getenv("ICX_SUB_MAX") ? -(std::max(kSubBytesSmall, std::atoi(std::getenv("ICX_SUB_MAX"))) & ~15) : 0;
    const char* gw_env = std::getenv("ICX_GW");
    const int gw = gw_env ? (std::atoi(gw_env) != 0) : ((int64_t)ws.max_w * ws.max_h > kGwMinPixels ? 1 : 0);
    const bool big = !gw && (std::getenv("ICX_BIG_WG") ? std::atoi(std::getenv("ICX_BIG_WG")) != 0 : true);
    const char* dri_env = std::getenv("ICX_DRI_GW");
    const int dri_min = dri_env ? (std::atoi(dri_env) != 0 ? kSubBytesSmall : 0) : kDriGwMin;
    if (piece == kRoundAll || piece == kRoundHead) {
        B(kStUnstuff);
        hipLaunchKernelGGL(k_spec_plan, dim3(1), dim3(1024), 0, st, n, d_data, d_off, ws.desc, ws.spec, ws.tilepre, ws.wgpre, ws.wg2pre,
                           ws.totals, ws.upool, ws.lanes_cap, sub_env, ws.pool_cap, ws.pool_next, gw, round, last, ws.h_defer,
                           dri_min);
        (void)hipEventRecord(ws.ev_defer, st);
        if (round == 0)
            hipLaunchKernelGGL(k_step_tabs, dim3(n), dim3(256), 0, st, n, ws.desc, ws.steps);
        const char* one_env = std::getenv("ICX_USTF1");
        if (one_env && std::atoi(one_env) != 0) {
            uint64_t* ts = reinterpret_cast<uint64_t*>(ws.tiles);
            (void)hipMemsetAsync(ts, 0, sizeof(uint64_t) * (size_t)(ws.tiles_cap + 2), st);
            hipLaunchKernelGGL(k_ustf_one, dim3(g), dim3(256), 0, st, n, d_data, d_off, ws.desc, ws.spec, ws.tilepre, ws.totals,
                               ts, ws.U, ws.rst, ws.rst_cap);
        } else {
            hipLaunchKernelGGL(k_ustf_count, dim3(g), dim3(256), 0, st, n, d_data, d_off, ws.desc, ws.spec, ws.tilepre,
                               ws.totals, ws.tiles);
            hipLaunchKernelGGL(k_ustf_scan, dim3(n), dim3(256), 0, st, n, ws.spec, ws.tiles, ws.tile_obase, ws.tile_rbase,
                               ws.U);
            hipLaunchKernelGGL(k_ustf_write, dim3(g), dim3(256), 0, st, n, d_data, d_off, ws.desc, ws.spec, ws.tilepre,
                               ws.totals, ws.tiles, ws.tile_obase, ws.tile_rbase, ws.U, ws.rst, ws.rst_cap);
        }
        E(kStUnstuff);
        if (gw) {
            B(kStWrite);
            hipLaunchKernelGGL((k_gw_lane<kWriteLanesBig, false>), dim3(g), dim3(kWriteLanesBig), 0, st, n, ws.desc, ws.spec,
                               ws.wg2pre, ws.totals, ws.steps, ws.U, ws.ac, ws.dc, ws.chunk_next, ws.pool_next, ws.pool_cap,
                               ws.X, ws.gw, ws.rec, lead, ws.rst, ws.rst_cap);
            hipLaunchKernelGGL((k_gw_lane<kWriteLanesBig, true>), dim3(std::min(g, 128)), dim3(kWriteLanesBig), 0, st, n,
                               ws.desc, ws.spec,
                               ws.wg2pre, ws.totals, ws.steps, ws.U, ws.ac, ws.dc, ws.chunk_next, ws.pool_next, ws.pool_cap,
                               ws.X, ws.gw, ws.rec, lead, ws.rst, ws.rst_cap);
            E(kStWrite);
            B(kStEntropy);
            hipLaunchKernelGGL(k_gw_check, dim3(g), dim3(kLanes), 0, st, n, ws.spec, ws.wgpre, ws.totals, ws.X, ws.gw, ws.crec,
                               ws.clist, ws.rst, ws.rst_cap);
            hipLaunchKernelGGL(k_gw_count, dim3(n), dim3(512), 0, st, n, ws.desc, ws.spec, ws.steps, ws.U, ws.X, ws.gw, ws.rec,
                               ws.ac, ws.dc, ws.chunk_next, ws.pool_next, ws.pool_cap, ws.crec, ws.Y, ws.clist, ws.repair,
                               ws.rst, ws.rst_cap);
            hipLaunchKernelGGL(k_gw_repair, dim3(n), dim3(64), 0, st, n, ws.desc, ws.spec, ws.steps, ws.U, ws.X, ws.Y, ws.gw,
                               ws.rec, ws.ac, ws.dc, ws.chunk_next, ws.pool_next, ws.pool_cap, ws.crec, ws.repair, ws.rst,
                               ws.rst_cap);
            hipLaunchKernelGGL(k_gw_scan, dim3(n), dim3(256), 0, st, n, ws.desc, ws.spec, ws.gw, ws.crec, ws.rec, ws.ent, ws.X,
                               ws.Y, ws.U, ws.rst, ws.rst_cap);
            hipLaunchKernelGGL(k_gw_tail, dim3(n), dim3(64), 0, st, n, ws.desc, ws.spec, ws.steps, ws.U, ws.X, ws.Y, ws.crec,
                               ws.ac, ws.dc, ws.chunk_next, ws.pool_next, ws.pool_cap, ws.map);
            hipLaunchKernelGGL(k_gw_map, dim3(g), dim3(kLanes), 0, st, n, ws.desc, ws.spec, ws.wgpre, ws.totals, ws.gw, ws.crec,
                               ws.rec, ws.ent, ws.chunk_next, ws.map);
            E(kStEntropy);
        } else {
        B(kStEntropy);
        if (big) {
            hipLaunchKernelGGL(k_spec_guess<kWriteLanesBig>, dim3(g), dim3(kWriteLanesBig), 0, st, n, ws.desc, ws.spec, ws.wg2pre,
                               ws.totals, 2, ws.steps, ws.U, ws.X, ws.rec, ws.nrec, ws.guess_cnt, lead);
            hipLaunchKernelGGL(k_spec_count<kWriteLanesBig>, dim3(g), dim3(kWriteLanesBig), 0, st, n, ws.desc, ws.spec, ws.wg2pre,
                               ws.totals, 2, ws.steps, ws.U, ws.X, ws.Y, ws.rec, ws.nrec, ws.guess_cnt, ws.sub, ws.repair);
        } else {
            hipLaunchKernelGGL(k_spec_guess<kLanes>, dim3(g), dim3(kLanes), 0, st, n, ws.desc, ws.spec, ws.wgpre,
                               ws.totals, 1, ws.steps, ws.U, ws.X, ws.rec, ws.nrec, ws.guess_cnt, lead);
            hipLaunchKernelGGL(k_spec_count<kLanes>, dim3(g), dim3(kLanes), 0, st, n, ws.desc, ws.spec, ws.wgpre,
                               ws.totals, 1, ws.steps, ws.U, ws.X, ws.Y, ws.rec, ws.nrec, ws.guess_cnt, ws.sub, ws.repair);
        }
        hipLaunchKernelGGL(k_spec_repair, dim3(n), dim3(64), 0, st, n, ws.desc, ws.spec, ws.steps, ws.U, ws.X, ws.Y,
                           ws.rec, ws.nrec, ws.guess_cnt, ws.sub, ws.repair);
        hipLaunchKernelGGL(k_spec_scan, dim3(n), dim3(256), 0, st, n, ws.spec, ws.sub, ws.ent);
        E(kStEntropy);
        B(kStWrite);
        if (big) {
            hipLaunchKernelGGL(k_spec_write<kWriteLanesBig>, dim3(g), dim3(kWriteLanesBig), 0, st, 1, n, ws.desc, ws.spec,
                               ws.wg2pre, ws.totals, ws.steps, ws.U, ws.X, ws.ent, ws.ac, ws.dc, ws.rst, ws.rst_cap);
        } else {
            hipLaunchKernelGGL(k_spec_write<kLanes>, dim3(g), dim3(kLanes), 0, st, 0, n, ws.desc, ws.spec, ws.wgpre,
                               ws.totals, ws.steps, ws.U, ws.X, ws.ent, ws.ac, ws.dc, ws.rst, ws.rst_cap);
        }
        E(kStWrite);
        }
    }
    if (piece == kRoundHead) return;
    if ((gw || big) && piece != kRoundTailNoDri) {
        B(kStWrite);
        hipLaunchKernelGGL(k_spec_write<kLanes>, dim3(piece == kRoundTailGw ? std::min(g, 128) : g), dim3(kLanes), 0, st, 3,
                           n, ws.desc, ws.spec, ws.wgpre,
                           ws.totals, ws.steps, ws.U, ws.X, ws.ent, ws.ac, ws.dc, ws.rst, ws.rst_cap);
        E(kStWrite);
    }
    hipLaunchKernelGGL(k_spec_finish, dim3((n + 63) / 64), dim3(64), 0, st, n, ws.desc, ws.spec, ws.stats);
}

}
```

include/icx.h:

```cpp
#ifndef ICX_H
#define ICX_H
#include <stddef.h>
#include <stdint.h>

#ifdef __cplusplus
extern "C" {
#endif

enum icx_result {
    ICX_OK = 0,
    ICX_NO_JPEG = 1,
    ICX_UNSUPPORTED = 2,
    ICX_OUT_OF_MEM = 3,
    ICX_INTERNAL_ERR = 4,
    ICX_SYNTAX_ERROR = 5
};

typedef struct icx_ctx icx_ctx;

icx_ctx* icx_create(int device);
void icx_destroy(icx_ctx* ctx);
const char* icx_last_error(const icx_ctx* ctx);
const char* icx_version(void);

int icx_jpeg_probe(const uint8_t* jpeg, size_t size, int* width, int* height, int* ncomp);

void icx_nj_init(icx_ctx* ctx);
void icx_nj_done(icx_ctx* ctx);
int icx_nj_decode(icx_ctx* ctx, const void* jpeg, int size);
int icx_nj_get_width(const icx_ctx* ctx);
int icx_nj_get_height(const icx_ctx* ctx);
int icx_nj_is_color(const icx_ctx* ctx);
unsigned char* icx_nj_get_image(icx_ctx* ctx);
int icx_nj_get_image_size(const icx_ctx* ctx);

int icx_jpeg_decode(icx_ctx* ctx, const uint8_t* jpeg, size_t size, uint8_t** out, int* width,
                    int* height, int* ncomp);
void icx_free(void* p);

typedef struct icx_batch icx_batch;

icx_batch* icx_batch_create(icx_ctx* ctx, int max_images, int max_width, int max_height, int group);
void icx_batch_destroy(icx_batch* b);

int icx_jpeg_batch_decode(icx_batch* b, int n, const uint8_t* d_data, const uint64_t* d_offsets,
                          const uint64_t* d_sizes, uint8_t* d_out, uint64_t out_stride,
                          int32_t* d_status, int32_t* d_dims, void* stream);

int icx_jpeg_batch_decode_host(icx_batch* b, int n, const uint8_t* const* jpegs, const size_t* sizes,
                               uint8_t* const* outs, uint64_t out_stride, int32_t* status, int32_t* dims);

int icx_batch_group(const icx_batch* b);
int icx_batch_groups(const icx_batch* b, int n);

int icx_batch_stage_times(const icx_batch* b, const char** names, float* ms, int cap);

int icx_batch_path_stats(const icx_batch* b, int32_t* parallel, int32_t* fallback, int32_t* sequential);

typedef struct icx_record {
    int32_t status, width, height, ncomp;
    uint64_t checksum;
} icx_record;

int icx_jpeg_records(icx_ctx* ctx, int n, const uint8_t* d_out, uint64_t out_stride, const int32_t* d_status,
                     const int32_t* d_dims, int max_width, int max_height, icx_record* d_records, void* stream);
uint64_t icx_checksum64(const uint8_t* data, size_t size);
int icx_ctx_device(const icx_ctx* ctx);
void* icx_ctx_stream(const icx_ctx* ctx);

typedef struct icx_multi icx_multi;
icx_multi* icx_multi_create(const int* devices, int ndev, int max_width, int max_height);
void icx_multi_destroy(icx_multi* m);
int icx_multi_decode_host(icx_multi* m, int n, const uint8_t* const* jpegs, const size_t* sizes,
                          uint8_t* const* outs, uint64_t out_stride, icx_record* records, int32_t* shard_of);
const char* icx_multi_last_error(const icx_multi* m);
const char* icx_multi_gather(const icx_multi* m);
int icx_multi_shard(const size_t* sizes, int n, int ndev, int32_t* shard_of);

typedef void icx_write_func(void* context, void* data, int size);

int icx_tje_encode_with_func(icx_ctx* ctx, icx_write_func* func, void* context, int quality,
                             int width, int height, int num_components, const unsigned char* src);
int icx_tje_encode_to_file_at_quality(icx_ctx* ctx, const char* dest_path, int quality, int width,
                                      int height, int num_components, const unsigned char* src);
int icx_tje_encode_to_file(icx_ctx* ctx, const char* dest_path, int width, int height,
                           int num_components, const unsigned char* src);

int icx_jpeg_encode_with_func(icx_ctx* ctx, icx_write_func* func, void* context, int quality,
                              int subsampling, int width, int height, int num_components,
                              const unsigned char* src);

typedef struct icx_encoder icx_encoder;
icx_encoder* icx_encoder_create(icx_ctx* ctx);
void icx_encoder_destroy(icx_encoder* enc);
int icx_jpeg_encode_device(icx_encoder* enc, int quality, int subsampling, int width, int height,
                           int num_components, const uint8_t* d_src, uint8_t* d_out, uint64_t out_cap,
                           uint64_t* out_size, void* hip_stream);
int icx_jpeg_encode_device_batch(icx_encoder* enc, int n, int quality, int subsampling, int width, int height,
                                 int num_components, const uint8_t* const* d_srcs, uint8_t* d_out,
                                 uint64_t out_stride, uint64_t* out_sizes, int32_t* status, void* hip_stream);
int icx_encoder_stage_times(icx_encoder* enc, const char** names, float* ms, int cap);

int icx_png_encode_with_func(icx_ctx* ctx, icx_write_func* func, void* context, const unsigned char* pixels,
                             int width, int height, int d);
int icx_png_save_to_file(icx_ctx* ctx, const char* path, const unsigned char* pixels, int width, int height,
                         int d);

typedef struct icx_png_encoder icx_png_encoder;
icx_png_encoder* icx_png_encoder_create(icx_ctx* ctx);
void icx_png_encoder_destroy(icx_png_encoder* enc);
int icx_png_encode_device(icx_png_encoder* enc, int width, int height, int d, const uint8_t* d_src,
                          uint8_t* d_out, uint64_t out_cap, uint64_t* out_size, void* hip_stream);
int icx_png_encode_device_batch(icx_png_encoder* enc, int n, int width, int height, int d,
                                const uint8_t* const* d_srcs, uint8_t* d_out, uint64_t out_stride,
                                uint64_t* out_sizes, int32_t* status, void* hip_stream);
int icx_png_encoder_stage_times(icx_png_encoder* enc, const char** names, float* ms, int cap);

enum icx_hdr_result {
    ICX_HDR_OK = 0,
    ICX_HDR_NOT_RADIANCE = 1,
    ICX_HDR_BAD_HEADER = 2,
    ICX_HDR_MALFORMED = 3,
    ICX_HDR_TRUNCATED = 4,
    ICX_HDR_TOO_LARGE = 5,
    ICX_HDR_INTERNAL_ERR = -1
};
int icx_hdr_probe(const uint8_t* data, size_t size, int* width, int* height);
int icx_hdr_decode(icx_ctx* ctx, const uint8_t* data, size_t size, float** out, int* width, int* height,
                   int* rows);
typedef struct icx_hdr_batch icx_hdr_batch;
icx_hdr_batch* icx_hdr_batch_create(icx_ctx* ctx, int max_images, int max_width, int max_height);
void icx_hdr_batch_destroy(icx_hdr_batch* b);
int icx_hdr_batch_decode(icx_hdr_batch* b, int n, const uint8_t* d_data, const uint64_t* d_offsets,
                         const uint64_t* d_sizes, float* d_out, uint64_t out_stride, int32_t* d_status,
                         int32_t* d_dims, void* hip_stream);
int icx_hdr_batch_stage_times(const icx_hdr_batch* b, const char** names, float* ms, int cap);

enum icx_exr_result {
    ICX_EXR_SUCCESS = 0,
    ICX_EXR_INVALID_MAGIC_NUMBER = -1,
    ICX_EXR_INVALID_EXR_VERSION = -2,
    ICX_EXR_INVALID_ARGUMENT = -3,
    ICX_EXR_INVALID_DATA = -4,
    ICX_EXR_UNSUPPORTED_FORMAT = -8,
    ICX_EXR_INVALID_HEADER = -9,
    ICX_EXR_UNSUPPORTED_FEATURE = -10,
    ICX_EXR_INTERNAL_ERR = -100
};
int icx_exr_probe(const uint8_t* data, size_t size, int* width, int* height);
int icx_exr_decode(icx_ctx* ctx, const uint8_t* data, size_t size, float** out_rgba, int* width, int* height);
int icx_exr_decode_device(icx_ctx* ctx, const uint8_t* data, const uint8_t* d_data, size_t size, float* d_out,
                          size_t out_floats, int* width, int* height);
int icx_exr_decode_device_batch(icx_ctx* ctx, int n, const uint8_t* const* data, const uint8_t* const* d_data,
                                const size_t* sizes, float* const* d_out, const size_t* out_floats, int32_t* codes,
                                int32_t* widths, int32_t* heights);

#ifdef __cplusplus
}
#endif
#endif
```

Baseline: 262,100.

## Overlap step tables and edge convert on side stream, skip redundant launches

Adds a non-blocking side stream per group, with fork/join events, so k_step_tabs runs alongside the unstuff stage and k_convert_edge runs alongside the main convert kernels. The luma border columns are now written by the chroma IDCT kernel instead of the stream-convert kernel, and the k_convert_stream<3> launch is dropped for common fuse modes. A host-visible flag set by the scan kernel lets the checking gw-lane kernel be skipped when no mode-1 error was seen. This cuts launch count and serial dependencies, at the cost of extra stream and event overhead, a host synchronization on a new scan event, and more complex correctness conditions.

Result: no change. 262,900 (median of 6 runs) (+0.3%).

```diff
diff --git a/imagecodecs_amd/__init__.py b/imagecodecs_amd/__init__.py
--- a/imagecodecs_amd/__init__.py
+++ b/imagecodecs_amd/__init__.py
@@ -55,6 +55,7 @@
     "icx_batch_group": (_i32, [_vp]),
     "icx_batch_groups": (_i32, [_vp, _i32]),
     "icx_batch_path_stats": (_i32, [_vp, C.POINTER(_i32), C.POINTER(_i32), C.POINTER(_i32)]),
+    "icx_batch_launch_stats": (_i32, [_vp, C.POINTER(_i32)]),
     "icx_tje_encode_with_func": (_i32, [_vp, _vp, _vp, _i32, _i32, _i32, _i32, _vp]),
     "icx_tje_encode_to_file_at_quality": (_i32, [_vp, C.c_char_p, _i32, _i32, _i32, _i32, _vp]),
     "icx_tje_encode_to_file": (_i32, [_vp, C.c_char_p, _i32, _i32, _i32, _vp]),
@@ -504,6 +505,12 @@
         lib().icx_batch_path_stats(self._p, C.byref(a), C.byref(b), C.byref(c))
         return {"parallel": a.value, "fallback": b.value, "sequential": c.value}
 
+    def launch_stats(self) -> dict:
+        v = (_i32 * 4)()
+        if lib().icx_batch_launch_stats(self._p, v) != OK:
+            raise ICXError("icx_batch_launch_stats failed")
+        return {"chk": v[0], "convert_stream3": v[1], "edge_side": v[2], "step_tabs_side": v[3]}
+
     @property
     def group(self) -> int:
         return int(lib().icx_batch_group(self._p))
diff --git a/imagecodecs_amd/csrc/icx_api.cpp b/imagecodecs_amd/csrc/icx_api.cpp
--- a/imagecodecs_amd/csrc/icx_api.cpp
+++ b/imagecodecs_amd/csrc/icx_api.cpp
@@ -193,6 +193,11 @@
     if (ws.h_defer) (void)hipHostFree(ws.h_defer);
     if (ws.h_layout) (void)hipHostFree(ws.h_layout);
     if (ws.ev_defer) (void)hipEventDestroy(ws.ev_defer);
+    if (ws.ev_scan) (void)hipEventDestroy(ws.ev_scan);
+    if (ws.side) (void)hipStreamDestroy(ws.side);
+    if (ws.ev_fork) (void)hipEventDestroy(ws.ev_fork);
+    if (ws.ev_join) (void)hipEventDestroy(ws.ev_join);
+    delete[] ws.launches;
     ws = GroupWs{};
 }
 
@@ -248,11 +253,16 @@
     ICX_HIP(ctx, hipMalloc(&ws.gw, sizeof(GwOut) * ws.lanes_cap), false);
     ICX_HIP(ctx, hipMalloc(&ws.crec, sizeof(GcRec) * ws.lanes_cap), false);
     ICX_HIP(ctx, hipMalloc(&ws.clist, sizeof(int2) * ws.lanes_cap), false);
-    ICX_HIP(ctx, hipHostMalloc(&ws.h_defer, 3 * sizeof(int32_t), hipHostMallocDefault), false);
-    ws.h_defer[0] = ws.h_defer[1] = ws.h_defer[2] = 0;
+    ICX_HIP(ctx, hipHostMalloc(&ws.h_defer, 4 * sizeof(int32_t), hipHostMallocDefault), false);
+    ws.h_defer[0] = ws.h_defer[1] = ws.h_defer[2] = ws.h_defer[kHChk] = 0;
     ICX_HIP(ctx, hipHostMalloc(&ws.h_layout, sizeof(int32_t), hipHostMallocDefault), false);
     *ws.h_layout = 1;
     ICX_HIP(ctx, hipEventCreateWithFlags(&ws.ev_defer, hipEventDisableTiming), false);
+    ICX_HIP(ctx, hipEventCreateWithFlags(&ws.ev_scan, hipEventDisableTiming), false);
+    ICX_HIP(ctx, hipStreamCreateWithFlags(&ws.side, hipStreamNonBlocking), false);
+    ICX_HIP(ctx, hipEventCreateWithFlags(&ws.ev_fork, hipEventDisableTiming), false);
+    ICX_HIP(ctx, hipEventCreateWithFlags(&ws.ev_join, hipEventDisableTiming), false);
+    ws.launches = new int32_t[4]();
     return true;
 }
 
@@ -344,8 +354,10 @@
     hipStream_t st = stream ? (hipStream_t)stream : ctx->stream;
     const RoctxRange range("icx_jpeg_batch_decode");
     b->hook->reset();
-    for (int p = 0; p < b->pipes; ++p)
+    for (int p = 0; p < b->pipes; ++p) {
         ICX_HIP(ctx, hipMemsetAsync(b->ws[p].stats, 0, sizeof(int32_t) * 4, st), ICX_INTERNAL_ERR);
+        std::fill(b->ws[p].launches, b->ws[p].launches + 4, 0);
+    }
     int per = 0;
     const int ng = batch_split(b, n, &per);
     const int used = std::min(b->pipes, ng);
@@ -412,6 +424,14 @@
     if (parallel) *parallel = h[0];
     if (fallback) *fallback = h[1];
     if (sequential) *sequential = h[2];
+    return ICX_OK;
+}
+
+int icx_batch_launch_stats(const icx_batch* b, int32_t out[4]) {
+    if (!b || !out) return ICX_INTERNAL_ERR;
+    for (int k = 0; k < 4; ++k) out[k] = 0;
+    for (int p = 0; p < b->pipes; ++p)
+        for (int k = 0; k < 4; ++k) out[k] += b->ws[p].launches[k];
     return ICX_OK;
 }
 
diff --git a/imagecodecs_amd/csrc/icx_decode.hip b/imagecodecs_amd/csrc/icx_decode.hip
--- a/imagecodecs_amd/csrc/icx_decode.hip
+++ b/imagecodecs_amd/csrc/icx_decode.hip
@@ -1513,6 +1513,25 @@
     }
 #endif
 }
+__device__ __forceinline__ void border_units(const Desc& d, const int16_t* ac, const int32_t* dcv, const uint2* map,
+                                             const uint32_t (&qw)[16], uint8_t* P, int stride, uint32_t mbw, uint32_t nby,
+                                             uint32_t b0, uint32_t ncol, uint32_t wid, uint32_t nw) {
+    const uint32_t lane = threadIdx.x & 63;
+    const uint32_t urows = (nby + 63) >> 6, nunits = ncol * urows;
+    for (uint32_t u = wid; u < nunits; u += nw) {
+        const uint32_t col = u / urows, ur = u - col * urows;
+        const uint32_t bx = col == 0 ? 0u : b0 + col - 1, by = min((ur << 6) + lane, nby - 1);
+        const BlkLoc l = blk_loc(d, map, (int64_t)(((by >> 1) * mbw + (bx >> 1)) * 6 + ((by & 1) << 1) + (bx & 1)));
+        int4 c[8];
+        load_block8(ac, l.blk, c);
+        uint32_t rowd[16];
+        block_idct(c, qw, dcv, l, rowd);
+        uint8_t* const bp = P + (int64_t)by * 8 * stride + (int64_t)bx * 8;
+#pragma unroll
+        for (int r = 0; r < 8; ++r)
+            *reinterpret_cast<uint2*>(bp + (int64_t)r * stride) = make_uint2(rowd[2 * r], rowd[2 * r + 1]);
+    }
+}
 __global__ __launch_bounds__(256, ICX_IDCT1_MINW) void k_idct420s(const Desc* __restrict__ desc, const int16_t* __restrict__ ac,
                                                                    const int32_t* __restrict__ dcv, const uint2* __restrict__ map,
                                                                    uint8_t* __restrict__ planes, int64_t plane_cap, int luma) {
@@ -1524,7 +1543,20 @@
     const uint32_t wid = chunk0 * 4 + wave, nw = gridDim.x * 4;
     const uint32_t mbw = (uint32_t)d.mbw, mbh = (uint32_t)d.mbh;
     uint8_t* const slot = planes + (int64_t)img * plane_cap;
-    const uint32_t ynbx = 2 * mbw, yunits = luma ? ((ynbx + 63) >> 6) * (2 * mbh) : 0u;
+    const uint32_t ynbx = 2 * mbw;
+    uint32_t yunits = ((ynbx + 63) >> 6) * (2 * mbh);
+    uint32_t b0 = 0, bcols = 0;
+    if (!luma) {
+        const CPl c1{slot + comp_plane_off(d, 1), d.c[1].w, d.c[1].h, d.c[1].stride};
+        const CPl c2{slot + comp_plane_off(d, 2), d.c[2].w, d.c[2].h, d.c[2].stride};
+        const int nl = (d.W + 3) >> 2, ef = edge_from(c1, c2, d.W);
+        if (ef > 1) {
+            yunits = 0;
+            b0 = (uint32_t)ef >> 1;
+            const uint32_t b1 = min(ynbx - 1, (uint32_t)(nl - 1) >> 1);
+            bcols = 1 + (ef < nl && b1 >= b0 ? b1 - b0 + 1 : 0u);
+        }
+    }
     const uint32_t cnbx = mbw, cunits = ((cnbx + 63) >> 6) * mbh;
     auto first = [&](uint32_t base) { return wid >= base ? wid - base : (base - wid + nw - 1) / nw * nw + wid - base; };
     uint32_t qw[16];
@@ -1547,6 +1579,13 @@
         uniform_q();
         plane_units(d, ac, dcv, map, qw, slot + comp_plane_off(d, 1 + cc), d.c[1 + cc].stride, cnbx, mbh, f, nw,
                     [&](uint32_t bx, uint32_t by) { return (int64_t)((by * mbw + bx) * 6 + 4 + cc); });
+    }
+    if (bcols) {
+        const uint32_t f = first(2 * cunits);
+        if (f >= bcols * ((2 * mbh + 63) >> 6)) return;
+        load_qw_g(d.q[d.c[0].tq], qw);
+        uniform_q();
+        border_units(d, ac, dcv, map, qw, slot, d.c[0].stride, mbw, 2 * mbh, b0, bcols, f, nw);
     }
 }
 
@@ -1672,8 +1711,6 @@
     uint8_t* o = out + (int64_t)img * out_stride;
     const StreamOut so{o, W, ((reinterpret_cast<uintptr_t>(o) & 3) == 0) && (W & 3) == 0};
     const int nsx = (mbw + 15) >> 4, nsy = (mbh + kFB5 - 1) / kFB5, nstrip = nsx * nsy;
-    uint8_t* const P0 = const_cast<uint8_t*>(pslot);
-    const int s0 = d.c[0].stride;
     const int ef = edge_from(c1, c2, W);
     const bool conv = ef > 1;
     const uint32_t chunk0 = (gridDim.x & 7) ? blockIdx.x : (blockIdx.x & 7) * (gridDim.x >> 3) + (blockIdx.x >> 3);
@@ -1682,7 +1719,6 @@
         const int mx0 = sx << 4, mb0 = sy * kFB5, mb1 = min(mbh, mb0 + kFB5);
         const int M = 64 * sx + lane, x0 = 4 * M;
         const bool live = M >= 1 && M < ef;
-        const bool border = x0 < W && !live;
         const int Mc = min(max(M, 1), max(ef - 1, 1));
         const int nb = live ? min(4, W - x0) * 3 : 0;
         const int mxl = min(mx0 + mq, mbw - 1);
@@ -1735,10 +1771,6 @@
 #endif
             asm volatile("" ::: "memory");
             const int Y0 = 16 * mby, Y1 = min(H, Y0 + 16);
-            if (border) {
-                for (int y = Y0; y < Y1; ++y)
-                    *reinterpret_cast<uint32_t*>(P0 + (int64_t)y * s0 + x0) = Yl[y - Y0][lane];
-            }
             if (conv) {
                 auto luma = [&](int y) { return Yl[y - Y0][lane]; };
                 auto emit = [&](int y, uint32_t yv, uint32_t cb, uint32_t cr) {
@@ -2007,6 +2039,14 @@
         hipLaunchKernelGGL(k_idct420s, dim3(std::max(sgx, 8), n), dim3(256), 0, st, ws.desc, ws.ac, ws.dc, ws.map,
                            ws.planes, ws.plane_cap, fuse == 4 ? 1 : 0);
     }
+    const int64_t egw = (4 * ((ws.max_h + kSHE - 1) / kSHE) + 255) / 256;
+    const int egx = (int)std::max<int64_t>(1, std::min<int64_t>(egw, 16384 / n));
+    const bool edge_side = fuse == 5 && side_fork(ws, st, kSideEdge);
+    if (edge_side) {
+        hipLaunchKernelGGL(k_convert_edge<3>, dim3(egx, n), dim3(256), 0, ws.side, ws.desc, ws.planes, ws.plane_cap, d_out,
+                           out_stride, fuse);
+        ++ws.launches[kLsEdgeSide];
+    }
     if (fuse == 1 || fuse == 2) {
         const int cgx = (int)std::max<int64_t>(1, std::min<int64_t>((maxblk / 6 / 16 + 31) / 32, 16384 / n)) & ~7;
         hipLaunchKernelGGL(k_idct420c, dim3(std::max(cgx, 8), n), dim3(256), 0, st, ws.desc, ws.ac, ws.dc, ws.map,
@@ -2053,8 +2093,11 @@
     const int64_t sxw = ((int64_t)(ws.max_w + 255) / 256) * ((ws.max_h + kSH - 1) / kSH) / 4 + 1;
     const int sxg = (int)std::max<int64_t>(1, std::min<int64_t>(sxw, 16384 / n));
     const int sxo = (int)std::max<int64_t>(1, std::min<int64_t>(sxw, gwg / n));
-    hipLaunchKernelGGL(k_convert_stream<3>, dim3(sxg, n), dim3(256), 0, st, ws.desc, ws.planes, ws.plane_cap, d_out,
-                       out_stride, fuse);
+    if (other || !(fuse == 1 || fuse == 3 || fuse == 5)) {
+        hipLaunchKernelGGL(k_convert_stream<3>, dim3(sxg, n), dim3(256), 0, st, ws.desc, ws.planes, ws.plane_cap, d_out,
+                           out_stride, fuse);
+        ++ws.launches[kLsStream3];
+    }
     if (other) {
         hipLaunchKernelGGL(k_convert_stream<0>, dim3(sxo, n), dim3(256), 0, st, ws.desc, ws.planes, ws.plane_cap, d_out,
                            out_stride, fuse);
@@ -2065,11 +2108,10 @@
         hipLaunchKernelGGL(k_convert_stream<4>, dim3(sxo, n), dim3(256), 0, st, ws.desc, ws.planes, ws.plane_cap, d_out,
                            out_stride, fuse);
     }
-    const int64_t egw = (4 * ((ws.max_h + kSHE - 1) / kSHE) + 255) / 256;
-    const int egx = (int)std::max<int64_t>(1, std::min<int64_t>(egw, 16384 / n));
     const int ego = (int)std::max<int64_t>(1, std::min<int64_t>(egw, gwg / n));
-    hipLaunchKernelGGL(k_convert_edge<3>, dim3(egx, n), dim3(256), 0, st, ws.desc, ws.planes, ws.plane_cap, d_out,
-                       out_stride, fuse);
+    if (!edge_side)
+        hipLaunchKernelGGL(k_convert_edge<3>, dim3(egx, n), dim3(256), 0, st, ws.desc, ws.planes, ws.plane_cap, d_out,
+                           out_stride, fuse);
     if (other) {
         hipLaunchKernelGGL(k_convert_edge<1>, dim3(ego, n), dim3(256), 0, st, ws.desc, ws.planes, ws.plane_cap, d_out,
                            out_stride, fuse);
@@ -2078,6 +2120,7 @@
         hipLaunchKernelGGL(k_convert, dim3(cx, n), dim3(256), 0, st, ws.desc, ws.planes, ws.tmp, ws.plane_cap,
                            ws.tmp_cap, d_out, out_stride);
     }
+    if (edge_side) side_join(ws, st);
     hipLaunchKernelGGL(k_finalize, dim3(nb), dim3(tb), 0, st, n, ws.desc, d_status, d_dims);
     E(kStConvert);
 }
diff --git a/imagecodecs_amd/csrc/icx_internal.h b/imagecodecs_amd/csrc/icx_internal.h
--- a/imagecodecs_amd/csrc/icx_internal.h
+++ b/imagecodecs_amd/csrc/icx_internal.h
@@ -1,6 +1,8 @@
 #pragma once
 #include <hip/hip_runtime.h>
 #include <stdint.h>
+
+#include <cstdlib>
 
 #include <string>
 #include <vector>
@@ -123,7 +125,25 @@
     int32_t* h_defer = nullptr;
     int32_t* h_layout = nullptr;
     hipEvent_t ev_defer = nullptr;
-};
+    hipEvent_t ev_scan = nullptr;
+    hipStream_t side = nullptr;
+    hipEvent_t ev_fork = nullptr, ev_join = nullptr;
+    int32_t* launches = nullptr;
+};
+enum { kHChk = 3 };
+enum { kLsChk = 0, kLsStream3 = 1, kLsEdgeSide = 2, kLsTabsSide = 3 };
+enum { kSideTabs = 1, kSideEdge = 2, kSideDefault = kSideTabs | kSideEdge };
+inline bool side_fork(const GroupWs& ws, hipStream_t st, int which) {
+    const char* e = std::getenv("ICX_SIDE");
+    if (!((e ? std::atoi(e) : kSideDefault) & which)) return false;
+    hipStreamCaptureStatus cap = hipStreamCaptureStatusNone;
+    if (!ws.side || hipStreamIsCapturing(st, &cap) != hipSuccess || cap != hipStreamCaptureStatusNone) return false;
+    return hipEventRecord(ws.ev_fork, st) == hipSuccess && hipStreamWaitEvent(ws.side, ws.ev_fork, 0) == hipSuccess;
+}
+inline void side_join(const GroupWs& ws, hipStream_t st) {
+    (void)hipEventRecord(ws.ev_join, ws.side);
+    (void)hipStreamWaitEvent(st, ws.ev_join, 0);
+}
 
 struct BlkLoc {
     int64_t blk;
@@ -183,7 +203,7 @@
                          StageHook* hook, int part = kFrontAll);
 enum { kRoundAll = 0, kRoundHead = 1, kRoundTail = 2, kRoundTailNoDri = 3, kRoundTailGw = 4 };
 void launch_spec_round(const GroupWs& ws, int n, const uint8_t* d_data, const uint64_t* d_off, hipStream_t st,
-                       StageHook* hook, int round, int last, int piece = kRoundAll);
+                       StageHook* hook, int round, int last, int piece = kRoundAll, bool chk = true);
 
 struct Record {
     int32_t status, w, h, c;
diff --git a/imagecodecs_amd/csrc/icx_spec.hip b/imagecodecs_amd/csrc/icx_spec.hip
--- a/imagecodecs_amd/csrc/icx_spec.hip
+++ b/imagecodecs_amd/csrc/icx_spec.hip
@@ -320,7 +320,7 @@
 
 __global__ __launch_bounds__(256) void k_ustf_scan(int n, SpecImg* __restrict__ spec, TileRec* __restrict__ tiles,
                                                    int32_t* __restrict__ tile_obase, int32_t* __restrict__ tile_rbase,
-                                                   uint8_t* __restrict__ U) {
+                                                   uint8_t* __restrict__ U, int32_t* __restrict__ h_chk) {
     __shared__ int sh[256];
     __shared__ int s_first_end;
     const int i = blockIdx.x;
@@ -361,6 +361,7 @@
         s.ulen = carry;
         s.nrst = rcarry;
         s.errpos = (fe != INT32_MAX && tiles[s.tile_base + fe].end_err) ? carry : INT64_MAX;
+        if (s.mode == 1 && s.errpos != INT64_MAX) *h_chk = 1;
         const int64_t nsub = carry > 0 ? (carry + s.sub_bytes - 1) / s.sub_bytes : 1;
         s.nsub = s.mode == 3 ? s.nint : (s.kint > 0 ? s.nint * s.kint : (int32_t)nsub);
     }
@@ -1685,6 +1686,11 @@
     s.mode = 5;
 }
 
+static int spec_gw(const GroupWs& ws) {
+    const char* gw_env = std::getenv("ICX_GW");
+    return gw_env ? (std::atoi(gw_env) != 0) : ((int64_t)ws.max_w * ws.max_h > kGwMinPixels ? 1 : 0);
+}
+
 void launch_spec_entropy(const GroupWs& ws, int n, const uint8_t* d_data, const uint64_t* d_off, hipStream_t st,
                          StageHook* hook, int part) {
     const int rounds = [] {
@@ -1692,13 +1698,15 @@
         return e ? std::max(1, std::min(8, std::atoi(e))) : kMaxRounds;
     }();
     if (part == kFrontFirst) {
+        ws.h_defer[kHChk] = 0;
         launch_spec_round(ws, n, d_data, d_off, st, hook, 0, rounds == 1, kRoundHead);
         return;
     }
     if (part == kFrontRest) {
-        const bool known = hipEventSynchronize(ws.ev_defer) == hipSuccess;
+        const bool known = hipEventSynchronize(spec_gw(ws) ? ws.ev_scan : ws.ev_defer) == hipSuccess;
         launch_spec_round(ws, n, d_data, d_off, st, hook, 0, rounds == 1,
-                          !known || ws.h_defer[1] != 0 ? kRoundTail : ws.h_defer[2] != 0 ? kRoundTailGw : kRoundTailNoDri);
+                          !known || ws.h_defer[1] != 0 ? kRoundTail : ws.h_defer[2] != 0 ? kRoundTailGw : kRoundTailNoDri,
+                          !known || ws.h_defer[kHChk] != 0);
         if (!known) return;
     }
     for (int r = part == kFrontRest ? 1 : 0; r < rounds; ++r) {
@@ -1710,7 +1718,7 @@
 }
 
 void launch_spec_round(const GroupWs& ws, int n, const uint8_t* d_data, const uint64_t* d_off, hipStream_t st,
-                       StageHook* hook, int round, int last, int piece) {
+                       StageHook* hook, int round, int last, int piece, bool chk) {
     auto B = [&](Stage s) { if (hook) hook->begin(s, st); };
     auto E = [&](Stage s) { if (hook) hook->end(s, st); };
     static const int g0 = std::getenv("ICX_EGRID") ? std::max(1, std::atoi(std::getenv("ICX_EGRID"))) : 2048;
@@ -1718,21 +1726,38 @@
     static const int lead = std::getenv("ICX_GUESS_LEAD") ? std::max(0, std::atoi(std::getenv("ICX_GUESS_LEAD"))) : -1;
     static const int sub_env = std::getenv("ICX_SUB_BYTES") ? std::max(kSubBytesSmall, std::atoi(std::getenv("ICX_SUB_BYTES"))) & ~15
                                : std::getenv("ICX_SUB_MAX") ? -(std::max(kSubBytesSmall, std::atoi(std::getenv("ICX_SUB_MAX"))) & ~15) : 0;
-    const char* gw_env = std::getenv("ICX_GW");
-    const int gw = gw_env ? (std::atoi(gw_env) != 0) : ((int64_t)ws.max_w * ws.max_h > kGwMinPixels ? 1 : 0);
+    const int gw = spec_gw(ws);
     const bool big = !gw && (std::getenv("ICX_BIG_WG") ? std::atoi(std::getenv("ICX_BIG_WG")) != 0 : true);
     const char* dri_env = std::getenv("ICX_DRI_GW");
     const int dri_min = dri_env ? (std::atoi(dri_env) != 0 ? kSubBytesSmall : 0) : kDriGwMin;
+    bool tabs_side = false;
+    auto launch_lane_a = [&]() {
+        hipLaunchKernelGGL((k_gw_lane<kWriteLanesBig, false>), dim3(g), dim3(kWriteLanesBig), 0, st, n, ws.desc, ws.spec,
+                           ws.wg2pre, ws.totals, ws.steps, ws.U, ws.ac, ws.dc, ws.chunk_next, ws.pool_next, ws.pool_cap,
+                           ws.X, ws.gw, ws.rec, lead, ws.rst, ws.rst_cap);
+    };
+    auto launch_lane_chk = [&]() {
+        hipLaunchKernelGGL((k_gw_lane<kWriteLanesBig, true>), dim3(std::min(g, 128)), dim3(kWriteLanesBig), 0, st, n,
+                           ws.desc, ws.spec,
+                           ws.wg2pre, ws.totals, ws.steps, ws.U, ws.ac, ws.dc, ws.chunk_next, ws.pool_next, ws.pool_cap,
+                           ws.X, ws.gw, ws.rec, lead, ws.rst, ws.rst_cap);
+        ++ws.launches[kLsChk];
+    };
+    const char* one_env = std::getenv("ICX_USTF1");
+    const bool ustf_one = one_env && std::atoi(one_env) != 0;
+    if (ustf_one) chk = true;
     if (piece == kRoundAll || piece == kRoundHead) {
+        if (round == 0) {
+            tabs_side = side_fork(ws, st, kSideTabs);
+            hipLaunchKernelGGL(k_step_tabs, dim3(n), dim3(256), 0, tabs_side ? ws.side : st, n, ws.desc, ws.steps);
+            if (tabs_side) ++ws.launches[kLsTabsSide];
+        }
         B(kStUnstuff);
         hipLaunchKernelGGL(k_spec_plan, dim3(1), dim3(1024), 0, st, n, d_data, d_off, ws.desc, ws.spec, ws.tilepre, ws.wgpre, ws.wg2pre,
                            ws.totals, ws.upool, ws.lanes_cap, sub_env, ws.pool_cap, ws.pool_next, gw, round, last, ws.h_defer,
                            dri_min);
         (void)hipEventRecord(ws.ev_defer, st);
-        if (round == 0)
-            hipLaunchKernelGGL(k_step_tabs, dim3(n), dim3(256), 0, st, n, ws.desc, ws.steps);
-        const char* one_env = std::getenv("ICX_USTF1");
-        if (one_env && std::atoi(one_env) != 0) {
+        if (ustf_one) {
             uint64_t* ts = reinterpret_cast<uint64_t*>(ws.tiles);
             (void)hipMemsetAsync(ts, 0, sizeof(uint64_t) * (size_t)(ws.tiles_cap + 2), st);
             hipLaunchKernelGGL(k_ustf_one, dim3(g), dim3(256), 0, st, n, d_data, d_off, ws.desc, ws.spec, ws.tilepre, ws.totals,
@@ -1741,21 +1766,29 @@
             hipLaunchKernelGGL(k_ustf_count, dim3(g), dim3(256), 0, st, n, d_data, d_off, ws.desc, ws.spec, ws.tilepre,
                                ws.totals, ws.tiles);
             hipLaunchKernelGGL(k_ustf_scan, dim3(n), dim3(256), 0, st, n, ws.spec, ws.tiles, ws.tile_obase, ws.tile_rbase,
-                               ws.U);
+                               ws.U, &ws.h_defer[kHChk]);
+            if (round == 0) (void)hipEventRecord(ws.ev_scan, st);
             hipLaunchKernelGGL(k_ustf_write, dim3(g), dim3(256), 0, st, n, d_data, d_off, ws.desc, ws.spec, ws.tilepre,
                                ws.totals, ws.tiles, ws.tile_obase, ws.tile_rbase, ws.U, ws.rst, ws.rst_cap);
         }
+        if (ustf_one && round == 0) (void)hipEventRecord(ws.ev_scan, st);
         E(kStUnstuff);
+        if (tabs_side) side_join(ws, st);
         if (gw) {
             B(kStWrite);
-            hipLaunchKernelGGL((k_gw_lane<kWriteLanesBig, false>), dim3(g), dim3(kWriteLanesBig), 0, st, n, ws.desc, ws.spec,
-                               ws.wg2pre, ws.totals, ws.steps, ws.U, ws.ac, ws.dc, ws.chunk_next, ws.pool_next, ws.pool_cap,
-                               ws.X, ws.gw, ws.rec, lead, ws.rst, ws.rst_cap);
-            hipLaunchKernelGGL((k_gw_lane<kWriteLanesBig, true>), dim3(std::min(g, 128)), dim3(kWriteLanesBig), 0, st, n,
-                               ws.desc, ws.spec,
-                               ws.wg2pre, ws.totals, ws.steps, ws.U, ws.ac, ws.dc, ws.chunk_next, ws.pool_next, ws.pool_cap,
-                               ws.X, ws.gw, ws.rec, lead, ws.rst, ws.rst_cap);
+            launch_lane_a();
+            if (piece == kRoundAll) launch_lane_chk();
             E(kStWrite);
+        }
+    }
+    if (gw && piece == kRoundHead) return;
+    if (piece == kRoundAll || piece == kRoundHead || gw) {
+        if (gw) {
+            if (piece != kRoundAll && chk) {
+                B(kStWrite);
+                launch_lane_chk();
+                E(kStWrite);
+            }
             B(kStEntropy);
             hipLaunchKernelGGL(k_gw_check, dim3(g), dim3(kLanes), 0, st, n, ws.spec, ws.wgpre, ws.totals, ws.X, ws.gw, ws.crec,
                                ws.clist, ws.rst, ws.rst_cap);
diff --git a/include/icx.h b/include/icx.h
--- a/include/icx.h
+++ b/include/icx.h
@@ -56,6 +56,8 @@
 int icx_batch_stage_times(const icx_batch* b, const char** names, float* ms, int cap);
 
 int icx_batch_path_stats(const icx_batch* b, int32_t* parallel, int32_t* fallback, int32_t* sequential);
+
+int icx_batch_launch_stats(const icx_batch* b, int32_t out[4]);
 
 typedef struct icx_record {
     int32_t status, width, height, ncomp;
```
